# mhpi/hydrodl2

Measured on AMD Instinct MI355X. Metric: basin-ensemble-timesteps/sec fwd+bwd, higher is better.
Workload: dtype f32

## Files before the change

### __graft_entry__.py

```python
from __future__ import annotations

import os
import subprocess
import sys

ROOT = os.path.dirname(os.path.abspath(__file__))
CSRC = os.path.join(ROOT, "hydrodl2_amd", "csrc")
HIP_LIB = os.path.join(CSRC, "libhbvx.so")
ORACLE_DIR = os.path.join(ROOT, "oracle")
ORACLE_LIB = os.path.join(ORACLE_DIR, "liboracle_hbv.so")

HIPCC_FLAGS = ["--offload-arch=gfx950", "-O3", "-std=c++17", "-ffp-contract=off", "-fno-slp-vectorize", "-fPIC"]


def _newer(target: str, *sources: str) -> bool:
    if not os.path.exists(target):
        return False
    t = os.path.getmtime(target)
    return all(os.path.getmtime(s) <= t for s in sources)


def _hipcc() -> str:
    hipcc = os.environ.get("HIPCC", "/opt/rocm/bin/hipcc")
    return hipcc if os.path.exists(hipcc) else "hipcc"


def build_hip(force: bool = False, tag: str = "", flags=()) -> str:
    from concurrent.futures import ThreadPoolExecutor
    units = [os.path.join(CSRC, f) for f in sorted(os.listdir(CSRC)) if f.endswith(".hip")]
    headers = [os.path.join(CSRC, f) for f in sorted(os.listdir(CSRC)) if f.endswith(".h")] + [
        os.path.join(ROOT, "include", "hbvx.h"), os.path.join(ROOT, "include", "hbvx_lstm.h"),
        os.path.join(ROOT, "include", "hbvx_gage_pop.h"), os.path.join(ROOT, "include", "hbvx_route_rows.h"),
        os.path.join(ROOT, "include", "hbvx_pop_fdc.h"), os.path.join(ROOT, "include", "hbvx_gage_events.h"),
        os.path.join(ROOT, "include", "hbvx_pop_events.h"), os.path.join(ROOT, "include", "hbvx_gage_fdc.h")]
    objdir = os.path.join(CSRC, "build_" + tag if tag else "build")
    os.makedirs(objdir, exist_ok=True)
    extra = os.environ.get("HBVX_EXTRA_HIPCC_FLAGS", "").split() + list(flags)
    lib = os.path.join(CSRC, f"libhbvx_{tag}.so") if tag else HIP_LIB

    def compile_one(src):
        obj = os.path.join(objdir, os.path.basename(src)[:-4] + ".o")
        if force or not _newer(obj, src, *headers):
            subprocess.check_call([_hipcc()] + HIPCC_FLAGS + extra + ["-c", src, "-o", obj], cwd=CSRC)
            return obj, True
        return obj, False

    with ThreadPoolExecutor(max_workers=min(len(units), os.cpu_count() or 1)) as pool:
        done = list(pool.map(compile_one, units))
    objs = [o for o, _ in done]
    if force or any(r for _, r in done) or not _newer(lib, *objs):
        subprocess.check_call([_hipcc(), "--offload-arch=gfx950", "-shared", "-fPIC", "-o", lib] + objs, cwd=CSRC)
    return lib


def build_oracle() -> str:
    subprocess.check_call(["make", "-C", ORACLE_DIR], stdout=subprocess.DEVNULL)
    return ORACLE_LIB


def build() -> None:
    build_hip()
    build_oracle()
    if ROOT not in sys.path:
        sys.path.insert(0, ROOT)
    import hydrodl2_amd
    from hydrodl2_amd._abi import Library
    lib = Library(HIP_LIB)
    assert lib.is_device
    assert set(hydrodl2_amd.available_models()["hbv"]) >= {"hbv", "hbv_1_1p", "hbv_2"}


def smoke() -> None:
    if ROOT not in sys.path:
        sys.path.insert(0, ROOT)
    import torch
    assert torch.cuda.is_available(), "smoke() needs a GPU"
    if not os.path.exists(HIP_LIB):
        build_hip()
    if not os.path.exists(ORACLE_LIB):
        build_oracle()
    from tests.abi_util import assert_close, compare_runs, make_problem, run_problem
    prob = make_problem(model="Hbv", T=120, B=9, M=16, dyn=("parBETA", "parBETAET"), seed=3)
    got = run_problem(prob, None, device="cuda:0", x_grad=True)
    want = run_problem(prob, ORACLE_LIB, device="cpu", x_grad=True)
    compare_runs(prob, got, want, keys=("flux", "routed", "state_out", "g_params", "g_x"))
    from tests import seam
    from hydrodl2_amd.lstm import SeqLSTM
    torch.manual_seed(0)
    net = SeqLSTM(5, 64, check=True)
    xs = torch.randn(30, 9, 5)
    outs = []
    for dev, lib in (("cuda:0", None), ("cpu", ORACLE_LIB)):
        seam.use_library(lib)
        m = net.to(dev)
        xd = xs.to(dev).requires_grad_(True)
        o, _ = m(xd)
        o.square().sum().backward()
        outs.append((o.detach().cpu(), xd.grad.cpu(), m.weight_hh_l0.grad.cpu().clone()))
        m.zero_grad()
    seam.use_library(None)
    for name, g, w in zip(("lstm h", "lstm grad_x", "lstm grad_w_hh"), outs[0], outs[1]):
        assert_close(name, g.numpy(), w.numpy())
    print("smoke ok: HIP path matches the CPU oracle "
          f"(flux {got['flux'].shape}, grad {got['g_params'].shape}, lstm {tuple(outs[0][0].shape)})")


if __name__ == "__main__":
    if len(sys.argv) > 2 and sys.argv[1] == "variant":
        print(build_hip(tag=sys.argv[2], flags=sys.argv[3:]))
        sys.exit(0)
    build()
    if len(sys.argv) > 1 and sys.argv[1] == "smoke":
        smoke()
```

### hydrodl2_amd/_abi.py

```python
from __future__ import annotations

import ctypes as C
import os
from typing import NamedTuple, Optional

ABI_VERSION = 10
MAX_PARAM = 20
GAGE_MAXLEN = 72
NSTATE = 5
MAX_FLUX = 12
UH_MAXLEN = 15

MODEL_HBV10, MODEL_HBV11P, MODEL_HBV20, MODEL_HBVADJ, MODEL_HOURLY = 0, 1, 2, 3, 4

TRAJ_ROWS, TRAJ_PACKED, TRAJ_CKPT = 0, 1, 2

(F_QSIM, F_Q0, F_Q1, F_Q2, F_AET, F_SWE, F_RECHARGE, F_EXCS, F_EVAPFACTOR, F_TOSOIL, F_PERC,
 F_CAPILLARY) = range(12)

PARAM_SLOTS = ["parBETA", "parFC", "parK0", "parK1", "parK2", "parLP", "parPERC", "parUZL",
               "parTT", "parCFMAX", "parCFR", "parCWH", "parBETAET", "parC", "parRT", "parAC",
               "parF0", "parFMIN", "parALPHA"]

_fp = C.c_void_p
# ... 153 lines not shown

SIGNATURES = [
    ("hbvx_zero", True, _int, [_vp, _u64, _vp], None),
    ("hbvx_zero_except", True, _int, [_vp, _i64, _i32, _i64, _i64, _i32, C.c_uint32, _vp], None),
    ("hbvx_preferred_traj_layout", True, _int, [_P(Desc)], None),
    ("hbvx_lstm_workspace_bytes", True, _u64, [_P(LstmDesc)], None),
    ("hbvx_lstm_forward", True, _int, [_P(LstmDesc), _fp, _fp, _fp, _fp, _fp, _vp, _u64, _vp], None),
    ("hbvx_lstm_backward", True, _int, [_P(LstmDesc), _fp, _fp, _fp, _fp, _fp, _vp, _u64, _vp], None),
    ("hbvx_lstm_check", True, _int, [_P(LstmDesc), _vp, _vp], None),
    ("hbvx_version", True, _int, [], None),
    ("hbvx_last_error", True, _str, [], None),
    ("hbvx_backend", True, _str, [], None),
    ("hbvx_sizeof", True, _u64, [_int], None),
    ("hbvx_forward", True, _int, [_P(Desc), _P(FwdOut), _vp], None),
    ("hbvx_backward", True, _int, [_P(Desc), _P(BwdIO), _vp], None),
    ("hbvx_backward_workspace_bytes", True, _u64, [_P(Desc)], None),
    ("hbvx_ckpt_workspace_bytes", True, _u64, [_P(Desc), _i32], None),
    ("hbvx_route_forward", True, _int, [_P(RouteDesc), _fp, _fp, _fp, _vp], None),
    ("hbvx_route_workspace_bytes", True, _u64, [_P(RouteDesc)], None),
    ("hbvx_route_backward", True, _int, [_P(RouteDesc), _fp, _fp, _fp, _fp, _fp, _fp, _fp, _u64, _vp], None),
    ("hbvx_adj_forward", True, _int, [_P(Desc), _P(FwdOut), _vp], None),
    ("hbvx_adj_backward", True, _int, [_P(Desc), _P(BwdIO), _vp], None),
    ("hbvx_bfi", True, _int, [_i32, _i32, _fp, _fp, C.c_float, _fp, _vp], None),
    ("hbvx_gage_route_forward", True, _int, [_P(GageDesc), _fp, _fp, _fp, _vp, _u64, _vp], None),
    ("hbvx_gage_route_backward", True, _int, [_P(GageDesc), _fp, _fp, _fp, _fp, _fp, _vp, _u64, _vp], None),
    ("hbvx_gage_route_workspace_bytes", True, _u64, [_P(GageDesc)], None),
    ("hbvx_zero_in_launch", True, _int, [], None),
    ("hbvx_zero_rest", True, _int, [_vp, _u64, _vp, _vp], None),
    ("hbvx_last_dispatch", True, _str, [_int], None),
    ("hbvx_lstm_forward_hx", False, _int, [_P(LstmDesc), _fp, _fp, _fp, _fp, _fp, _fp, _fp, _vp, _u64, _vp], None),
    ("hbvx_lstm_backward_hx", False, _int, [_P(LstmDesc), _fp, _fp, _fp, _fp, _fp, _fp, _fp, _fp, _vp, _u64, _vp], None),
    ("hbvx_forward_tangent", False, _int, [_P(Desc), _P(TanIO), _vp], (7, TanIO)),
    ("hbvx_route_tangent", False, _int, [_P(RouteDesc), _fp, _fp, _fp, _fp, _fp, _fp, _vp], None),
    ("hbvx_bfi_tangent", False, _int, [_i32, _i32, _fp, _fp, _fp, _fp, C.c_float, _fp, _vp], None),
    ("hbvx_lstm_tangent", False, _int,
     [_P(LstmDesc), _fp, _fp, _fp, _fp, _fp, _fp, _fp, _fp, _fp, _vp, _u64, _vp], None),
    ("hbvx_forward_tangent_batch", False, _int, [_P(Desc), _P(TanBatch), _vp], (8, TanBatch)),
    ("hbvx_route_tangent_batch", False, _int,
     [_P(RouteDesc), _i32, _fp, _fp, _fp, _i64, _fp, _fp, _i64, _fp, _vp], None),
    ("hbvx_bfi_tangent_batch", False, _int, [_i32, _i32, _i32, _fp, _fp, _fp, _fp, _i64, C.c_float, _fp, _vp], None),
    ("hbvx_lstm_tangent_batch", False, _int,
     [_P(LstmDesc), _i32, _fp, _fp, _fp, _fp, _fp, _fp, _fp, _fp, _fp, _vp, _u64, _vp], None),
    ("hbvx_lstm_tangent_batch_workspace_bytes", False, _u64, [_P(LstmDesc), _i32], None),
    ("hbvx_hourly_tangent_batch", False, _int, [_P(Desc), _P(TanBatch), _vp], (8, TanBatch)),
    ("hbvx_gage_route_tangent_batch", False, _int,
     [_P(GageDesc), _i32, _fp, _fp, _fp, _i64, _fp, _i64, _fp, _vp, _u64, _vp], None),
    ("hbvx_gage_route_tangent_workspace_bytes", False, _u64, [_P(GageDesc), _i32], None),
    ("hbvx_adj_tangent_batch", False, _int, [_P(Desc), _P(TanBatch), _fp, _vp], (8, TanBatch)),
    ("hbvx_gram", False, _int, [_P(GramDesc), _fp, _fp, _fp, _fp, _fp, _fp, _vp, _u64, _vp], (9, GramDesc)),
    ("hbvx_gram_workspace_bytes", False, _u64, [_P(GramDesc)], None),
    ("hbvx_quadform", False, _int, [_P(GramDesc), _fp, _fp, _fp, _vp, _u64, _vp], (9, GramDesc)),
    ("hbvx_quadform_workspace_bytes", False, _u64, [_P(GramDesc)], None),
] + [(_name, False, _int, [_P(Desc), _P(_e.struct), _vp], (_POP_SIZEOF[_e.struct], _e.struct))
     for _name, _e in POPULATION.items()]

EXPORTS = [row[0] for row in SIGNATURES if row[1]]
OPTIONAL_EXPORTS = [row[0] for row in SIGNATURES if not row[1]]

GAGE_POP_ABI_VERSION = 1


class PopRunoff(C.Structure):
    _fields_ = [("abi_version", C.c_int32), ("n_cand", C.c_int32), ("p", PopSrc * MAX_PARAM), ("runoff", _fp)]


class GagePop(C.Structure):
    _fields_ = [("abi_version", C.c_int32), ("n_cand", C.c_int32), ("runoff", _fp), ("runoff_c_stride", C.c_int64),
                ("dp", _fp), ("uh", _fp), ("transform", C.c_int32), ("n_periods", C.c_int32),
                ("period_end", C.c_void_p),
                ("target", _fp), ("w", _fp), ("shift", _fp), ("eps", _fp),
                ("sse", _fp), ("s1", _fp), ("s2", _fp), ("s3", _fp), ("sim", _fp), ("series", _fp)]


GAGE_POP_SIGNATURES = [
    ("hbvx_gage_pop_sizeof", False, _u64, [_int], None),
    ("hbvx_hourly_population_runoff", False, _int, [_P(Desc), _P(PopRunoff), _vp], (0, PopRunoff)),
    ("hbvx_gage_population_workspace_bytes", False, _u64, [_P(GageDesc), _P(GagePop)], (1, GagePop)),
    ("hbvx_gage_population_stats", False, _int, [_P(GageDesc), _P(GagePop), _vp, _u64, _vp], (1, GagePop)),
]


GAGE_EVENTS_ABI_VERSION = 1


class GageEvents(C.Structure):
    _fields_ = [("abi_version", C.c_int32), ("n_cand", C.c_int32), ("T", C.c_int32), ("G", C.c_int32),
                ("n_events", C.c_int32), ("series", _fp),
                ("start", C.c_void_p), ("end", C.c_void_p),
                ("peak", _fp), ("peak_hour", C.c_void_p), ("volume", _fp)]


GAGE_EVENTS_SIGNATURES = [
    ("hbvx_gage_events_sizeof", False, _u64, [_int], None),
    ("hbvx_gage_population_events", False, _int, [_P(GageEvents), _vp], (0, GageEvents)),
]


POP_FDC_ABI_VERSION = 1
POP_FDC_MAX_THR = 32

GAGE_FDC_ABI_VERSION = 1
GAGE_QUANT_MAX_T = 16384


class GageFdc(C.Structure):
    _fields_ = [("abi_version", C.c_int32), ("n_cand", C.c_int32), ("T", C.c_int32), ("G", C.c_int32),
                ("n_lev", C.c_int32), ("series", _fp),
                ("scored", C.c_void_p),
                ("thr", _fp), ("count", C.c_void_p), ("volume", _fp),
                ("rank", C.c_void_p), ("quantile", _fp)]


GAGE_FDC_SIGNATURES = [
    ("hbvx_gage_fdc_sizeof", False, _u64, [_int], None),
    ("hbvx_gage_population_fdc", False, _int, [_P(GageFdc), _vp], (0, GageFdc)),
    ("hbvx_gage_quantiles_workspace_bytes", False, _u64, [C.c_int32, C.c_int32, C.c_int32], None),
    ("hbvx_gage_population_quantiles", False, _int, [_P(GageFdc), _fp, _u64, _vp], (0, GageFdc)),
]


class PopFdc(C.Structure):
    _fields_ = [("abi_version", C.c_int32), ("n_thr", C.c_int32), ("flow", PopStats), ("thr", _fp),
                ("count", C.c_void_p),
                ("volume", _fp)]


POP_FDC_SIGNATURES = [
    ("hbvx_pop_fdc_sizeof", False, _u64, [_int], None),
    ("hbvx_population_fdc", False, _int, [_P(Desc), _P(PopFdc), _vp], (0, PopFdc)),
]
POP_FDC_ENTRY = PopEntry(PopFdc, False, None)


POP_EVENTS_ABI_VERSION = 1


class PopEvents(C.Structure):
    _fields_ = [("abi_version", C.c_int32), ("n_events", C.c_int32), ("flow", PopStats),
                ("start", C.c_void_p), ("end", C.c_void_p),
                ("peak", _fp), ("peak_day", C.c_void_p), ("volume", _fp)]


POP_EVENTS_SIGNATURES = [
    ("hbvx_pop_events_sizeof", False, _u64, [_int], None),
    ("hbvx_population_events", False, _int, [_P(Desc), _P(PopEvents), _vp], (0, PopEvents)),
]
POP_EVENTS_ENTRY = PopEntry(PopEvents, False, None)


ROUTE_ROWS_SIGNATURES = [
    ("hbvx_route_backward_rows", False, _int, [_P(RouteDesc), _fp, _fp, _fp, _fp, _i32, _fp, _fp, _fp, _u64, _vp], None),
]


class HbvxError(RuntimeError):
    pass


class Library:

    def __init__(self, path: str):
        if not os.path.exists(path):
            raise FileNotFoundError(path)
        self.path = path
        self.dll = C.CDLL(path)
        d = self.dll
        for name in EXPORTS:
            if not hasattr(d, name):
                raise HbvxError(f"{path}: missing export {name}")
        self.missing = [name for name in OPTIONAL_EXPORTS +
                        [row[0] for row in GAGE_POP_SIGNATURES + ROUTE_ROWS_SIGNATURES + POP_FDC_SIGNATURES +
                         GAGE_EVENTS_SIGNATURES + POP_EVENTS_SIGNATURES + GAGE_FDC_SIGNATURES]
                        if not hasattr(d, name)]
        checked = set()
        for name, _, restype, argtypes, layout, sizeof in [row + ("hbvx_sizeof",) for row in SIGNATURES] + \
                [row + ("hbvx_gage_pop_sizeof",) for row in GAGE_POP_SIGNATURES] + \
                [row + ("hbvx_sizeof",) for row in ROUTE_ROWS_SIGNATURES] + \
                [row + ("hbvx_pop_fdc_sizeof",) for row in POP_FDC_SIGNATURES] + \
                [row + ("hbvx_gage_events_sizeof",) for row in GAGE_EVENTS_SIGNATURES] + \
                [row + ("hbvx_pop_events_sizeof",) for row in POP_EVENTS_SIGNATURES] + \
                [row + ("hbvx_gage_fdc_sizeof",) for row in GAGE_FDC_SIGNATURES]:
            if name in self.missing:
                continue
            fn = getattr(d, name)
            fn.restype, fn.argtypes = restype, argtypes
            if layout is not None and (sizeof, layout[0]) not in checked and sizeof not in self.missing:
                checked.add((sizeof, layout[0]))
                which, st = layout
                got = getattr(d, sizeof)(which)
                if got != C.sizeof(st):
                    raise HbvxError(f"{path}: layout mismatch for {st.__name__}: {got} != {C.sizeof(st)}")
        if d.hbvx_version() != ABI_VERSION:
            raise HbvxError(f"{path}: ABI version {d.hbvx_version()} != {ABI_VERSION}")
        for which, st in enumerate([Desc, FwdOut, BwdIO, RouteDesc, ParamSrc, ParamGrad, GageDesc]):
            if d.hbvx_sizeof(which) != C.sizeof(st):
                raise HbvxError(f"{path}: layout mismatch for {st.__name__}: "
                                f"{d.hbvx_sizeof(which)} != {C.sizeof(st)}")
        self.backend = d.hbvx_backend().decode()
        self.saves_pow = "+savepow" in self.backend

    @property
    def is_device(self) -> bool:
        return self.backend.startswith("hip")

    def _check(self, rc: int, what: str):
        if rc != 0:
            msg = self.dll.hbvx_last_error().decode(errors="replace")
            raise HbvxError(f"{what} failed ({rc}): {msg}")

    def forward(self, desc: Desc, out: FwdOut, stream: int):
        self._check(self.dll.hbvx_forward(C.byref(desc), C.byref(out), C.c_void_p(stream)),
                    "hbvx_forward")

    def backward(self, desc: Desc, io: BwdIO, stream: int):
        self._check(self.dll.hbvx_backward(C.byref(desc), C.byref(io), C.c_void_p(stream)),
                    "hbvx_backward")

    def zero_rest(self, ptr: int, nbytes: int, state_ptr: int, stream: int):
        self._check(self.dll.hbvx_zero_rest(C.c_void_p(ptr), nbytes, C.c_void_p(state_ptr), C.c_void_p(stream)), "hbvx_zero_rest")

    def zero_in_launch(self) -> bool:
        return bool(self.dll.hbvx_zero_in_launch())

    def last_dispatch(self, direction: int) -> str:
        return self.dll.hbvx_last_dispatch(direction).decode()

    def preferred_traj_layout(self, desc: Desc) -> int:
        return int(self.dll.hbvx_preferred_traj_layout(C.byref(desc)))

    def ckpt_workspace_bytes(self, desc: Desc, K: int) -> int:
        return int(self.dll.hbvx_ckpt_workspace_bytes(C.byref(desc), K))

    def backward_workspace_bytes(self, desc: Desc) -> int:
        return int(self.dll.hbvx_backward_workspace_bytes(C.byref(desc)))

    def adj_forward(self, desc: Desc, out: FwdOut, stream: int):
        self._check(self.dll.hbvx_adj_forward(C.byref(desc), C.byref(out), C.c_void_p(stream)),
                    "hbvx_adj_forward")

    def adj_backward(self, desc: Desc, io: BwdIO, stream: int):
        self._check(self.dll.hbvx_adj_backward(C.byref(desc), C.byref(io), C.c_void_p(stream)),
                    "hbvx_adj_backward")

    def gage_route_workspace_bytes(self, r: GageDesc) -> int:
        return int(self.dll.hbvx_gage_route_workspace_bytes(C.byref(r)))

    def gage_route_forward(self, r: GageDesc, qs: int, uh: int, out: int, ws, ws_bytes: int, stream: int):
        self._check(self.dll.hbvx_gage_route_forward(C.byref(r), qs, uh, out, ws, C.c_uint64(ws_bytes),
                                                     C.c_void_p(stream)), "hbvx_gage_route_forward")

    def gage_route_backward(self, r: GageDesc, qs: int, uh: int, go: int, gqs: int, gdp: int, ws,
                            ws_bytes: int, stream: int):
        self._check(self.dll.hbvx_gage_route_backward(C.byref(r), qs, uh, go, gqs, gdp, ws,
                                                      C.c_uint64(ws_bytes), C.c_void_p(stream)),
                    "hbvx_gage_route_backward")

    def zero(self, ptr: int, nbytes: int, stream: int):
        self._check(self.dll.hbvx_zero(ptr, C.c_uint64(nbytes), C.c_void_p(stream)), "hbvx_zero")

    def zero_except(self, ptr: int, rows: int, width: int, r0: int, r1: int, group_w: int, keep: int,
                    stream: int):
        self._check(self.dll.hbvx_zero_except(ptr, rows, width, r0, r1, group_w, C.c_uint32(keep),
                                              C.c_void_p(stream)), "hbvx_zero_except")

    def lstm_workspace_bytes(self, r: LstmDesc) -> int:
        return int(self.dll.hbvx_lstm_workspace_bytes(C.byref(r)))

    def lstm_forward(self, r: LstmDesc, w_hh: int, gx: int, gates: int, c_all: int, h_all: int, ws,
                     ws_bytes: int, stream: int):
        self._check(self.dll.hbvx_lstm_forward(C.byref(r), w_hh, gx, gates, c_all, h_all, ws,
                                               C.c_uint64(ws_bytes), C.c_void_p(stream)), "hbvx_lstm_forward")

    def lstm_backward(self, r: LstmDesc, w_hh: int, gates: int, c_all: int, gh: int, gg: int, ws,
                      ws_bytes: int, stream: int):
        self._check(self.dll.hbvx_lstm_backward(C.byref(r), w_hh, gates, c_all, gh, gg, ws,
                                                C.c_uint64(ws_bytes), C.c_void_p(stream)), "hbvx_lstm_backward")

    def require(self, name: str):
        if name in self.missing:
            raise HbvxError(f"{self.path}: missing export {name} (backend {self.backend!r})")

    def lstm_forward_hx(self, r: LstmDesc, w_hh: int, gx: int, h0, c0, gates: int, c_all: int, h_all: int, ws,
                        ws_bytes: int, stream: int):
        self.require("hbvx_lstm_forward_hx")
        self._check(self.dll.hbvx_lstm_forward_hx(C.byref(r), w_hh, gx, h0, c0, gates, c_all, h_all, ws,
                                                  C.c_uint64(ws_bytes), C.c_void_p(stream)), "hbvx_lstm_forward_hx")

    def lstm_backward_hx(self, r: LstmDesc, w_hh: int, gates: int, c0, c_all: int, gh: int, gc_last, gg: int, gc0,
                         ws, ws_bytes: int, stream: int):
        self.require("hbvx_lstm_backward_hx")
        self._check(self.dll.hbvx_lstm_backward_hx(C.byref(r), w_hh, gates, c0, c_all, gh, gc_last, gg, gc0, ws,
                                                   C.c_uint64(ws_bytes), C.c_void_p(stream)), "hbvx_lstm_backward_hx")

    def lstm_tangent(self, r: LstmDesc, w_hh: int, gates: int, c0, c_all: int, gx_t: int, h0_t, c0_t, h_t: int,
                     c_t_last, ws, ws_bytes: int, stream: int):
        self.require("hbvx_lstm_tangent")
        self._check(self.dll.hbvx_lstm_tangent(C.byref(r), w_hh, gates, c0, c_all, gx_t, h0_t, c0_t, h_t, c_t_last, ws,
                                               C.c_uint64(ws_bytes), C.c_void_p(stream)), "hbvx_lstm_tangent")

    def lstm_tangent_batch_workspace_bytes(self, r: LstmDesc, n_dir: int) -> int:
        self.require("hbvx_lstm_tangent_batch_workspace_bytes")
        return int(self.dll.hbvx_lstm_tangent_batch_workspace_bytes(C.byref(r), n_dir))

    def lstm_tangent_batch(self, r: LstmDesc, n_dir: int, w_hh: int, gates: int, c0, c_all: int, gx_t: int, h0_t,
                           c0_t, h_t: int, c_t_last, ws, ws_bytes: int, stream: int):
        self.require("hbvx_lstm_tangent_batch")
        self._check(self.dll.hbvx_lstm_tangent_batch(C.byref(r), n_dir, w_hh, gates, c0, c_all, gx_t, h0_t, c0_t, h_t,
                                                     c_t_last, ws, C.c_uint64(ws_bytes), C.c_void_p(stream)),
                    "hbvx_lstm_tangent_batch")

    def forward_tangent(self, desc: Desc, io: TanIO, stream: int):
        self.require("hbvx_forward_tangent")
        self._check(self.dll.hbvx_forward_tangent(C.byref(desc), C.byref(io), C.c_void_p(stream)), "hbvx_forward_tangent")

    def route_tangent(self, r: RouteDesc, q: int, uh: int, q_dot, ra_dot, rb_dot, q_rout_dot: int, stream: int):
        self.require("hbvx_route_tangent")
        self._check(self.dll.hbvx_route_tangent(C.byref(r), q, uh, q_dot, ra_dot, rb_dot, q_rout_dot,
                                                C.c_void_p(stream)), "hbvx_route_tangent")

    def bfi_tangent(self, T: int, B: int, qs: int, q2: int, qs_dot, q2_dot, nearzero: float, out: int, stream: int):
        self.require("hbvx_bfi_tangent")
        self._check(self.dll.hbvx_bfi_tangent(T, B, qs, q2, qs_dot, q2_dot, C.c_float(nearzero), out,
                                              C.c_void_p(stream)), "hbvx_bfi_tangent")

    def forward_tangent_batch(self, desc: Desc, tb: TanBatch, stream: int):
        self.require("hbvx_forward_tangent_batch")
        self._check(self.dll.hbvx_forward_tangent_batch(C.byref(desc), C.byref(tb), C.c_void_p(stream)),
                    "hbvx_forward_tangent_batch")

    def route_tangent_batch(self, r: RouteDesc, n_dir: int, q: int, uh: int, q_dot, q_dot_ds: int, ra_dot, rb_dot,
                            r_ds: int, q_rout_dot: int, stream: int):
        self.require("hbvx_route_tangent_batch")
        self._check(self.dll.hbvx_route_tangent_batch(C.byref(r), n_dir, q, uh, q_dot, q_dot_ds, ra_dot, rb_dot, r_ds,
                                                      q_rout_dot, C.c_void_p(stream)), "hbvx_route_tangent_batch")

    def bfi_tangent_batch(self, T: int, B: int, n_dir: int, qs: int, q2: int, qs_dot, q2_dot, dot_ds: int,
                          nearzero: float, out: int, stream: int):
        self.require("hbvx_bfi_tangent_batch")
        self._check(self.dll.hbvx_bfi_tangent_batch(T, B, n_dir, qs, q2, qs_dot, q2_dot, dot_ds, C.c_float(nearzero),
                                                    out, C.c_void_p(stream)), "hbvx_bfi_tangent_batch")

    def hourly_tangent_batch(self, desc: Desc, tb: TanBatch, stream: int):
        self.require("hbvx_hourly_tangent_batch")
        self._check(self.dll.hbvx_hourly_tangent_batch(C.byref(desc), C.byref(tb), C.c_void_p(stream)),
                    "hbvx_hourly_tangent_batch")

    def adj_tangent_batch(self, desc: Desc, tb: TanBatch, traj, stream: int):
        self.require("hbvx_adj_tangent_batch")
        self._check(self.dll.hbvx_adj_tangent_batch(C.byref(desc), C.byref(tb), traj, C.c_void_p(stream)),
                    "hbvx_adj_tangent_batch")

    def gram_workspace_bytes(self, g: GramDesc) -> int:
        self.require("hbvx_gram_workspace_bytes")
        return int(self.dll.hbvx_gram_workspace_bytes(C.byref(g)))

    def gram(self, g: GramDesc, s: int, w, r, gram: int, rhs, cost, ws, ws_bytes: int, stream: int):
        self.require("hbvx_gram")
        self._check(self.dll.hbvx_gram(C.byref(g), s, w, r, gram, rhs, cost, ws, C.c_uint64(ws_bytes),
                                       C.c_void_p(stream)), "hbvx_gram")

    def quadform_workspace_bytes(self, g: GramDesc) -> int:
        self.require("hbvx_quadform_workspace_bytes")
        return int(self.dll.hbvx_quadform_workspace_bytes(C.byref(g)))

    def quadform(self, g: GramDesc, s: int, m: int, q: int, ws, ws_bytes: int, stream: int):
        self.require("hbvx_quadform")
        self._check(self.dll.hbvx_quadform(C.byref(g), s, m, q, ws, C.c_uint64(ws_bytes), C.c_void_p(stream)),
                    "hbvx_quadform")

    def gage_route_tangent_workspace_bytes(self, r: GageDesc, n_dir: int) -> int:
# ... 92 lines not shown
```

### hydrodl2_amd/csrc/hbv_chunked.h

```cpp
#pragma once

#include <hip/hip_runtime.h>

#include "../../include/hbvx.h"
#include "hbv_step.h"
#include "hbv_lane.h"
#include "hbv_onepass_compose.h"

namespace hbvx {

struct ChunkArgs {
    hbvx_desc d;
    hbvx_bwd_io io;
    int lgMp;
    int C;
    int nchunk;
    float *phi;
    float *abnd;
    float *gpart;
    int nd;
    int dslot[3];
    int per_xcd;
    int group;
};

struct ChunkBlock {
    int bx, chunk;
};
__host__ __device__ inline int chunk_per_xcd(int B, int lgMp)
{
    const int bpw = 64 >> lgMp;
    return ((B + bpw - 1) / bpw + 7) / 8;
}
__device__ __forceinline__ bool chunk_block(const hbvx_desc &d, int lgMp, int per_xcd, ChunkBlock &b)
{
    const int i = blockIdx.x;
#if defined(HBVX_CHUNK_XCD) && HBVX_CHUNK_XCD == 0
    b.chunk = i / (8 * per_xcd);
    b.bx = i - b.chunk * (8 * per_xcd);
#else
    const int c = i & 7, k = i >> 3;
    b.chunk = k / per_xcd;
    b.bx = c * per_xcd + (k - b.chunk * per_xcd);
#endif
    return b.bx * (64 >> lgMp) < d.B;
}

#define CHUNK_FEW 3

template <int NP>
__device__ __forceinline__ void slot_set(float *p, int slot, float v)
{
#pragma unroll
    for (int i = 0; i < NP; i++)
        if (slot == i) p[i] = v;
}
template <int NP>
__device__ __forceinline__ float slot_get(const float *p, int slot)
{
    float v = 0.0f;
#pragma unroll
    for (int i = 0; i < NP; i++)
        if (slot == i) v = p[i];
    return v;
}

template <int MODEL, bool BETAET>
struct ChunkNP {
    static constexpr int value = MODEL == MODEL_HBV10 ? (BETAET ? 13 : 12)
                               : MODEL == MODEL_HBV11P ? 14 : (MODEL == MODEL_HOURLY ? 19 : 16);
};

template <int NP>
struct ChunkRaw {
    float f[3];
    float st[5];
    float sw0, ef0;
    float gf[HBVX_MAX_FLUX];
    float g4[4];
    float dv[NP];
    float mu;
};

template <int MODEL, bool BETAET, int NP>
struct ChunkDay {
    Step<MODEL, BETAET> s;
    float p[NPARAM_MAX];
    float ud[NP];
    FluxGrad g;
    float gq;
};

template <int NP>
__device__ __forceinline__ void chunk_dma_dyn(const hbvx_desc &d, const LaneId &L, int t, float *lds)
{
#if defined(__HIP_DEVICE_COMPILE__)
    const hbvx_param_src &ps = d.p[0];
    const float *src = ps.dyn + (int64_t)t * ps.dyn_t_stride + (int64_t)L.b * ps.dyn_b_stride + L.j;
    const int M = d.M;
#pragma unroll
    for (int i = 0; i < NP; i++) {
        __builtin_amdgcn_global_load_lds((const __attribute__((address_space(1))) void *)src,
                                         (__attribute__((address_space(3))) void *)(lds + i * 64), 4, 0, 0);
        src += M;
    }
#endif
}
template <int NP>
__device__ __forceinline__ void chunk_pull_dyn(ChunkRaw<NP> &R, const float *lds)
{
#pragma unroll
    for (int i = 0; i < NP; i++) R.dv[i] = lds[i * 64 + (threadIdx.x & 63)];
}

template <int NP, int DYN, bool GFULL, bool LDSDV = false, bool MU = false>
__device__ __forceinline__ void chunk_issue(const hbvx_desc &d, const hbvx_bwd_io &io,
                                            const LaneId &L, int t, int nf, ChunkRaw<NP> &R,
                                            int nd, const int *dslot)
{
    const int T = d.T;
    const int64_t N = (int64_t)d.B * d.M;
    const float *xr = d.x + (int64_t)t * d.x_t_stride + (int64_t)L.b * d.x_b_stride;
    R.f[0] = xr[d.ch_prcp]; R.f[1] = xr[d.ch_tmean]; R.f[2] = xr[d.ch_pet];
    const float *tp = io.traj + (int64_t)t * N + L.n;
    const int64_t ks = (int64_t)(T + 1) * N;
#pragma unroll
    for (int k = 0; k < 5; k++) R.st[k] = tp[k * ks];
    if (SAVE_POW) {
        const float *ap = io.aux + (int64_t)t * N + L.n;
        R.sw0 = ap[0];
        R.ef0 = ap[(int64_t)T * N];
    } else {
        R.sw0 = R.ef0 = 0.0f;
    }
    const int64_t fs = (int64_t)T * d.B, go = (int64_t)t * d.B + L.b;
#pragma unroll
    for (int k = 0; k < HBVX_MAX_FLUX; k++) {
        R.gf[k] = 0.0f;
        if (GFULL && k < nf) R.gf[k] = io.grad_flux[k * fs + go];
        if (k < 4) R.g4[k] = io.grad_flux4 ? io.grad_flux4[k * fs + go] : 0.0f;
    }
    R.mu = 0.0f;
    if (DYN == 1) {
#pragma unroll
        for (int k = 0; k < CHUNK_FEW; k++)
            if (k < nd) {
                const hbvx_param_src &ps = d.p[dslot[k]];
                R.dv[k] = ps.dyn[(int64_t)t * ps.dyn_t_stride + (int64_t)L.b * ps.dyn_b_stride + L.j];
            }
    }
    if (DYN == 3 && !LDSDV) {
        const hbvx_param_src &ps = d.p[0];
        const float *src = ps.dyn + (int64_t)t * ps.dyn_t_stride + (int64_t)L.b * ps.dyn_b_stride + L.j;
#pragma unroll
        for (int i = 0; i < NP; i++) R.dv[i] = src[i * d.M];
    }
    if (DYN == 2) {
#pragma unroll
        for (int i = 0; i < NP; i++) {
            const hbvx_param_src &ps = d.p[i];
            const bool dy = ps.dyn != nullptr;
            const float *base = dy ? ps.dyn : ps.sta;
            const int64_t ts = dy ? ps.dyn_t_stride : 0, bs = dy ? ps.dyn_b_stride : ps.sta_b_stride;
            R.dv[i] = base[(int64_t)t * ts + (int64_t)L.b * bs + L.j];
        }
    }
    if ((MU || DYN == 2) && d.muwts) R.mu = d.muwts[(int64_t)t * d.mu_t_stride + (int64_t)L.b * d.mu_b_stride + L.j];
}

template <int MODEL, bool BETAET, int NP, int DYN, bool GFULL, bool MU = false>
__device__ __forceinline__ void chunk_finish(const hbvx_desc &d, const ChunkRaw<NP> &R, bool raw, float nz,
                                             float ac, float elev, const float *usta, const float *psta,
                                             const bool *use_dyn, int nf, float invM,
                                             ChunkDay<MODEL, BETAET, NP> &D, int nd, const int *dslot, bool has4)
{
    float gf[HBVX_MAX_FLUX];
#pragma unroll
    for (int k = 0; k < HBVX_MAX_FLUX; k++) {
        gf[k] = R.gf[k];
        if (k < 4 && has4) gf[k] += R.g4[k];
    }
    D.s.P = R.f[0]; D.s.Tf = R.f[1]; D.s.PET = R.f[2];
    D.s.SP = R.st[0]; D.s.MW = R.st[1]; D.s.SM = R.st[2]; D.s.SUZ = R.st[3]; D.s.SLZ = R.st[4];
    if (DYN == 1) {
#pragma unroll
        for (int i = 0; i < NP; i++) D.p[i] = psta[i];
#pragma unroll
        for (int k = 0; k < CHUNK_FEW; k++)
            if (k < nd) {
                const hbvx_param_src &ps = d.p[dslot[k]];
                const float v = raw ? sigmoid_dyn_(R.dv[k]) : R.dv[k];
                D.ud[k] = v;
                const float pv = descale_(v, ps.lo, ps.hi);
                const float cur = slot_get<NP>(D.p, dslot[k]);
                slot_set<NP>(D.p, dslot[k], use_dyn[k] ? pv : cur);
            }
    }
    if (DYN == 3) {
#pragma unroll
        for (int i = 0; i < NP; i++) {
            D.ud[i] = raw ? sigmoid_dyn_(R.dv[i]) : R.dv[i];
            D.p[i] = descale_(D.ud[i], d.p[i].lo, d.p[i].hi);
        }
    }
#pragma unroll
    for (int i = 0; i < NP; i++) {
        if (DYN == 1 || DYN == 3) break;
        D.ud[i] = usta[i];
        D.p[i] = psta[i];
        if (DYN == 2) {
            const float v = raw ? sigmoid_dyn_(R.dv[i]) : R.dv[i];
            D.ud[i] = use_dyn[i] ? v : usta[i];
            D.p[i] = use_dyn[i] ? descale_(v, d.p[i].lo, d.p[i].hi) : psta[i];
        }
    }
#pragma unroll
    for (int i = NP; i < NPARAM_MAX; i++) D.p[i] = 0.0f;
    D.s.template fwd<SAVE_POW>(D.p, nz, ac, elev, R.sw0, R.ef0);
    D.gq = gf[HBVX_F_QSIM];
    const float wq = ((MU || DYN == 2) && d.muwts) ? R.mu : invM;
    D.g.gQ = D.gq * wq;
    D.g.gQ0 = gf[HBVX_F_Q0] * invM;
    D.g.gQ1 = gf[HBVX_F_Q1] * invM;
    D.g.gQ2 = gf[HBVX_F_Q2] * invM;
    D.g.gET = GFULL ? gf[HBVX_F_AET] * invM : 0.0f;
    D.g.gSWE = GFULL ? gf[HBVX_F_SWE] * invM : 0.0f;
    D.g.grech = GFULL ? gf[HBVX_F_RECHARGE] * invM : 0.0f;
    D.g.gexc = GFULL ? gf[HBVX_F_EXCS] * invM : 0.0f;
    D.g.gef = GFULL ? gf[HBVX_F_EVAPFACTOR] * invM : 0.0f;
    D.g.gtosoil = GFULL ? gf[HBVX_F_TOSOIL] * invM : 0.0f;
    D.g.gPERC = GFULL ? gf[HBVX_F_PERC] * invM : 0.0f;
    D.g.gcap = (GFULL && nf > HBVX_F_CAPILLARY) ? gf[HBVX_F_CAPILLARY] * invM : 0.0f;
}

template <int NP, int DYN>
__device__ __forceinline__ void chunk_static(const hbvx_desc &d, const LaneId &L, bool raw,
                                             float *usta, float *psta, bool *use_dyn, int nd,
                                             const int *dslot)
{
#pragma unroll
    for (int i = 0; i < NP; i++) {
        if (DYN == 3) {
            usta[i] = psta[i] = 0.0f;
            use_dyn[i] = true;
            continue;
        }
        const hbvx_param_src &s = d.p[i];
        float v = s.sta[(int64_t)L.b * s.sta_b_stride + L.j];
        usta[i] = raw ? sigmoid_(v) : v;
        psta[i] = descale_(usta[i], s.lo, s.hi);
        use_dyn[i] = DYN == 2 && s.dyn && !(s.drop && s.drop[L.b]);
    }
    if (DYN == 1) {
#pragma unroll
        for (int k = 0; k < CHUNK_FEW; k++) {
            use_dyn[k] = false;
            if (k < nd) {
                const hbvx_param_src &s = d.p[dslot[k]];
                use_dyn[k] = !(s.drop && s.drop[L.b]);
            }
        }
    }
}

template <int SC>
struct SlotCombo {
    static constexpr int nd = SC == 1 ? 2 : (SC == 2 ? 3 : 0);
    static constexpr int s0 = P_BETA, s1 = SC == 1 ? P_BETAET : P_K0, s2 = P_BETAET;
};
#define CHUNK_SLOTS(A)                                                                             \
    const int nd_ = SC ? SlotCombo<SC>::nd : (A).nd;                                               \
    const int ds_[3] = {SC ? SlotCombo<SC>::s0 : (A).dslot[0], SC ? SlotCombo<SC>::s1 : (A).dslot[1], \
                        SC ? SlotCombo<SC>::s2 : (A).dslot[2]}

template <int MODEL, bool BETAET, int DYN, bool GFULL, int SC = 0, bool MU = false>
__global__ void __launch_bounds__(64) k_bwd_chunk_phi(const ChunkArgs A)
{
    CHUNK_SLOTS(A);
    constexpr int NP = ChunkNP<MODEL, BETAET>::value;
    const hbvx_desc &d = A.d;
    const hbvx_bwd_io &io = A.io;
    ChunkBlock blk;
    if (!chunk_block(d, A.lgMp, A.per_xcd, blk)) return;
    const LaneId L = lane_id(d, A.lgMp, blk.bx);
    const int chunk = blk.chunk;
    const int t0 = chunk * A.C, t1 = min(d.T, t0 + A.C);
    const int64_t N = (int64_t)d.B * d.M;
    const bool raw = d.raw_sigmoid != 0;
    const float nz = d.nearzero, invM = 1.0f / (float)d.M;
    const float ac = (MODEL == MODEL_HBV20 || MODEL == MODEL_HOURLY) ? d.ac[L.b] : 0.0f;
    const float elev = (MODEL == MODEL_HBV20 || MODEL == MODEL_HOURLY) ? d.elev[L.b] : 0.0f;
    float usta[NP], psta[NP];
    bool use_dyn[NP];
    chunk_static<NP, DYN>(d, L, raw, usta, psta, use_dyn, nd_, ds_);

    float Phi[5][5], phi[5];
#pragma unroll
    for (int k = 0; k < 5; k++) {
        phi[k] = 0.0f;
#pragma unroll
        for (int i = 0; i < 5; i++) Phi[k][i] = (i == k) ? 1.0f : 0.0f;
    }
    FluxGrad g0;
    g0.gQ = g0.gQ0 = g0.gQ1 = g0.gQ2 = g0.gET = g0.gSWE = g0.grech = g0.gexc = g0.gef = g0.gtosoil =
        g0.gPERC = g0.gcap = 0.0f;
    constexpr bool LDSDV = DYN == 3;
    __shared__ float dvbuf[LDSDV ? NP * 64 : 1];
    ChunkRaw<NP> Rn;
    if (LDSDV) chunk_dma_dyn<NP>(d, L, t1 - 1, dvbuf);
    chunk_issue<NP, DYN, GFULL, LDSDV, MU>(d, io, L, t1 - 1, io.n_flux, Rn, nd_, ds_);
    for (int t = t1 - 1; t >= t0; t--) {
        ChunkRaw<NP> Rc = Rn;
        if (LDSDV) {
            asm volatile("s_waitcnt vmcnt(0)" ::: "memory");
            chunk_pull_dyn<NP>(Rc, dvbuf);
            asm volatile("s_waitcnt lgkmcnt(0)" ::: "memory");
        }
        if (t > t0) {
            if (LDSDV) chunk_dma_dyn<NP>(d, L, t - 1, dvbuf);
            chunk_issue<NP, DYN, GFULL, LDSDV, MU>(d, io, L, t - 1, io.n_flux, Rn, nd_, ds_);
        }
        ChunkDay<MODEL, BETAET, NP> D;
        chunk_finish<MODEL, BETAET, NP, DYN, GFULL, MU>(d, Rc, raw, nz, ac, elev, usta, psta, use_dyn,
                                                    io.n_flux, invM, D, nd_, ds_, io.grad_flux4 != nullptr);
        float gp[NPARAM_MAX], gx[3];
#pragma unroll
        for (int i = 0; i < NPARAM_MAX; i++) gp[i] = 0.0f;
        if constexpr (MODEL == MODEL_HBV10) {
            typedef Step<MODEL, BETAET> S;
            const typename S::JT c = D.s.jt_coef(D.p, nz);
            S::template jt_unit<0>(c, Phi[0]);
            S::template jt_unit<0>(c, Phi[1]);
            S::template jt_unit<1>(c, Phi[2]);
            S::template jt_unit<2>(c, Phi[3]);
            S::template jt_unit<2>(c, Phi[4]);
            if constexpr (!GFULL) {
                S::jt_affine(c, phi, D.g.gQ0 + D.g.gQ, D.g.gQ1 + D.g.gQ, D.g.gQ2 + D.g.gQ);
                continue;
            }
        } else if constexpr (MODEL == MODEL_HBV11P || MODEL == MODEL_HBV20) {
            typedef Step<MODEL, BETAET> S;
            const typename S::JTC c = D.s.jt_coef_cap(D.p, nz);
            S::template jt_unit<0>(c, Phi[0]);
            S::template jt_unit<0>(c, Phi[1]);
#pragma unroll
            for (int k = 2; k < 5; k++) S::jt_cap(c, Phi[k], 0.0f, 0.0f, 0.0f);
            if constexpr (!GFULL) {
                S::jt_cap(c, phi, D.g.gQ0 + D.g.gQ, D.g.gQ1 + D.g.gQ, D.g.gQ2 + D.g.gQ);
                continue;
            }
        } else {
#pragma unroll
            for (int k = 0; k < 5; k++) D.s.bwd(D.p, nz, g0, Phi[k], gp, gx);
        }
        D.s.bwd(D.p, nz, D.g, phi, gp, gx);
    }
    if (L.active) {
        float *dst = A.phi + ((int64_t)chunk * 30) * N + L.n;
#pragma unroll
        for (int k = 0; k < 5; k++)
#pragma unroll
            for (int i = 0; i < 5; i++) dst[(int64_t)(k * 5 + i) * N] = Phi[k][i];
#pragma unroll
        for (int i = 0; i < 5; i++) dst[(int64_t)(25 + i) * N] = phi[i];
    }
}

#define ONEPASS_GMAX 4
__host__ __device__ constexpr int onepass_slot_bytes(int NP) { return (30 + onepass_rows(NP)) * 64 * (int)sizeof(float); }

template <int NP>
struct OnepassSlot {
    float *s;
    __device__ __forceinline__ float Phi(int k, int j) const { return s[(k * 5 + j) * 64]; }
    __device__ __forceinline__ float phi(int j) const { return s[(25 + j) * 64]; }
    __device__ __forceinline__ float G(int k, int p) const { return s[(30 + onepass_row(p) + k - onepass_kmin(p)) * 64]; }
    __device__ __forceinline__ void Phi(int k, int i, float v) { s[(k * 5 + i) * 64] = v; }
    __device__ __forceinline__ void phi(int i, float v) { s[(25 + i) * 64] = v; }
    __device__ __forceinline__ void G(int k, int p, float v) { s[(30 + onepass_row(p) + k - onepass_kmin(p)) * 64] = v; }
};
template <int NP>
struct OnepassRows {
    float *m, *g;
    int64_t N;
    bool active;
    __device__ __forceinline__ void Phi(int k, int i, float v) { if (active) m[(int64_t)(k * 5 + i) * N] = v; }
    __device__ __forceinline__ void phi(int i, float v) { if (active) m[(int64_t)(25 + i) * N] = v; }
    __device__ __forceinline__ void G(int k, int p, float v)
    {
        if (active) g[(int64_t)(onepass_row(p) + k - onepass_kmin(p)) * N] = v;
    }
};

template <bool BETAET, bool GFULL>
__global__ void __launch_bounds__(64 * ONEPASS_GMAX) __attribute__((amdgpu_waves_per_eu(GFULL ? 2 : 3)))
k_bwd_chunk_onepass(const ChunkArgs A)
{
    extern __shared__ float onepass_slot[];
    constexpr int MODEL = MODEL_HBV10, DYN = 0;
    constexpr int NP = ChunkNP<MODEL, BETAET>::value;
    typedef Step<MODEL, BETAET> S;
    const int ds_[3] = {0, 0, 0};
    const hbvx_desc &d = A.d;
    const hbvx_bwd_io &io = A.io;
    ChunkBlock blk;
    if (!chunk_block(d, A.lgMp, A.per_xcd, blk)) return;
    const LaneId L = lane_id(d, A.lgMp, blk.bx);
    const int grp = blk.chunk;
    const int w = __builtin_amdgcn_readfirstlane((int)threadIdx.x >> 6);
    const int nw = min(min(A.group, ONEPASS_GMAX), A.nchunk - grp * A.group);
    const int chunk = grp * A.group + w;
    const int t0 = chunk * A.C, t1 = min(d.T, t0 + A.C);
    const int64_t N = (int64_t)d.B * d.M;
    const bool raw = d.raw_sigmoid != 0;
    const float nz = d.nearzero, invM = 1.0f / (float)d.M;
    float usta[NP], psta[NP];
    bool use_dyn[NP];
    chunk_static<NP, DYN>(d, L, raw, usta, psta, use_dyn, 0, ds_);

    float Phi[5][5], phi[5];
    float G[6][NPARAM_MAX];
#pragma unroll
    for (int k = 0; k < 5; k++) {
        phi[k] = 0.0f;
#pragma unroll
        for (int i = 0; i < 5; i++) Phi[k][i] = (i == k) ? 1.0f : 0.0f;
    }
#pragma unroll
    for (int k = 0; k < 6; k++)
#pragma unroll
        for (int i = 0; i < NPARAM_MAX; i++) G[k][i] = 0.0f;
    if (w < nw) {
    ChunkRaw<NP> Rn;
    chunk_issue<NP, DYN, GFULL>(d, io, L, t1 - 1, io.n_flux, Rn, 0, ds_);
    for (int t = t1 - 1; t >= t0; t--) {
        ChunkRaw<NP> Rc = Rn;
        if (t > t0) chunk_issue<NP, DYN, GFULL>(d, io, L, t - 1, io.n_flux, Rn, 0, ds_);
        ChunkDay<MODEL, BETAET, NP> D;
        chunk_finish<MODEL, BETAET, NP, DYN, GFULL>(d, Rc, raw, nz, 0.0f, 0.0f, usta, psta, use_dyn, io.n_flux, invM,
                                                    D, 0, ds_, io.grad_flux4 != nullptr);
        const typename S::JT c = D.s.jt_coef(D.p, nz);
        const typename S::JG k = D.s.jg_coef(D.p, nz);
        S::template jt_gp<0>(c, k, Phi[0], G[0]);
        S::template jt_gp<0>(c, k, Phi[1], G[1]);
        S::template jt_gp<1>(c, k, Phi[2], G[2]);
        S::template jt_gp<2>(c, k, Phi[3], G[3]);
        S::template jt_gp<2>(c, k, Phi[4], G[4]);
        if constexpr (!GFULL) {
            S::template jt_gp<2, true>(c, k, phi, G[5], D.g.gQ0 + D.g.gQ, D.g.gQ1 + D.g.gQ, D.g.gQ2 + D.g.gQ);
        } else {
            float gx[3];
            D.s.bwd(D.p, nz, D.g, phi, G[5], gx);
        }
    }
    }
    OnepassRows<NP> rows{A.phi + ((int64_t)grp * 30) * N + L.n, A.gpart + ((int64_t)grp * onepass_rows(NP)) * N + L.n, N,
                         L.active};
    if (A.group == 1) {
        onepass_put<float, NP>(Phi, phi, G, rows);
        return;
    }
    OnepassSlot<NP> slot{onepass_slot + (threadIdx.x & 63)};
    if (w == nw - 1 && w > 0) onepass_put<float, NP>(Phi, phi, G, slot);
    static_assert(ONEPASS_GMAX == 4, "one stage per wave above wave 0");
    if (nw > 1) {
        if (nw > 2) {
            if (nw > 3) __syncthreads();
            if (w == 2 && nw > 3) onepass_compose<float, NP, false>(slot, Phi, phi, G, slot);
            __syncthreads();
        }
        if (w == 1 && nw > 2) onepass_compose<float, NP, false>(slot, Phi, phi, G, slot);
        __syncthreads();
    }
    if (w == 0) {
        if (nw == 1) onepass_put<float, NP>(Phi, phi, G, rows);
        else onepass_compose<float, NP, true>(slot, Phi, phi, G, rows);
    }
}

#ifndef HBVX_CHUNK_NO_SHARED_KERNELS
__global__ void __launch_bounds__(64) k_bwd_chunk_scan(const ChunkArgs A)
{
    const hbvx_desc &d = A.d;
    const int64_t N = (int64_t)d.B * d.M;
    const int64_t n = (int64_t)blockIdx.x * 64 + threadIdx.x;
    if (n >= N) return;
    float a[5];
#pragma unroll
    for (int k = 0; k < 5; k++) a[k] = A.io.grad_state_out ? A.io.grad_state_out[k * N + n] : 0.0f;
    constexpr int SCAN_DEPTH = 4;
    float buf[SCAN_DEPTH][30];
    auto fetch = [&](int c, float *dst) __attribute__((always_inline)) {
        const float *src = A.phi + ((int64_t)c * 30) * N + n;
#pragma unroll
        for (int i = 0; i < 30; i++) dst[i] = src[(int64_t)i * N];
    };
#pragma unroll
    for (int j = 0; j < SCAN_DEPTH; j++)
        if (A.nchunk - 1 - j >= 0) fetch(A.nchunk - 1 - j, buf[j]);
    for (int c0 = A.nchunk - 1; c0 >= 0; c0 -= SCAN_DEPTH) {
#pragma unroll
        for (int j = 0; j < SCAN_DEPTH; j++) {
            const int c = c0 - j;
            if (c < 0) break;
            float cur[30];
#pragma unroll
            for (int i = 0; i < 30; i++) cur[i] = buf[j][i];
            if (c - SCAN_DEPTH >= 0) fetch(c - SCAN_DEPTH, buf[j]);
#pragma unroll
            for (int k = 0; k < 5; k++) A.abnd[((int64_t)c * 5 + k) * N + n] = a[k];
            float an[5];
#pragma unroll
            for (int i = 0; i < 5; i++) {
                float v = cur[25 + i];
#pragma unroll
                for (int k = 0; k < 5; k++) v += a[k] * cur[k * 5 + i];
                an[i] = v;
            }
#pragma unroll
            for (int i = 0; i < 5; i++) a[i] = an[i];
        }
    }
    if (A.io.grad_state_in) {
#pragma unroll
        for (int k = 0; k < 5; k++) A.io.grad_state_in[k * N + n] = a[k];
    }
}

#endif

template <int MODEL, bool BETAET, int DYN, bool GFULL, int SC = 0, bool ROWST = false, bool MU = false>
__global__ void __launch_bounds__(64) k_bwd_chunk_sweep(const ChunkArgs A)
{
    CHUNK_SLOTS(A);
    constexpr int NP = ChunkNP<MODEL, BETAET>::value;
    __shared__ float rowbuf[ROWST ? 64 * NP : 1];
    const hbvx_desc &d = A.d;
    const hbvx_bwd_io &io = A.io;
    ChunkBlock blk;
    if (!chunk_block(d, A.lgMp, A.per_xcd, blk)) return;
    const LaneId L = lane_id(d, A.lgMp, blk.bx);
    const int chunk = blk.chunk;
    const int t0 = chunk * A.C, t1 = min(d.T, t0 + A.C);
    const int64_t N = (int64_t)d.B * d.M;
    const bool raw = d.raw_sigmoid != 0;
    const float nz = d.nearzero, invM = 1.0f / (float)d.M;
    const float ac = (MODEL == MODEL_HBV20 || MODEL == MODEL_HOURLY) ? d.ac[L.b] : 0.0f;
    const float elev = (MODEL == MODEL_HBV20 || MODEL == MODEL_HOURLY) ? d.elev[L.b] : 0.0f;
    float usta[NP], psta[NP], gsta[NP];
    bool use_dyn[NP];
    chunk_static<NP, DYN>(d, L, raw, usta, psta, use_dyn, nd_, ds_);
#pragma unroll
    for (int i = 0; i < NP; i++) gsta[i] = 0.0f;
    float gused[CHUNK_FEW] = {0.0f, 0.0f, 0.0f};
    float a[5];
#pragma unroll
    for (int k = 0; k < 5; k++) a[k] = A.abnd[((int64_t)chunk * 5 + k) * N + L.n];

    constexpr bool LDSDV = DYN == 3;
    __shared__ float dvbuf[LDSDV ? NP * 64 : 1];
    ChunkRaw<NP> Rn;
    if (LDSDV) chunk_dma_dyn<NP>(d, L, t1 - 1, dvbuf);
    chunk_issue<NP, DYN, GFULL, LDSDV, MU>(d, io, L, t1 - 1, io.n_flux, Rn, nd_, ds_);
    for (int t = t1 - 1; t >= t0; t--) {
        ChunkRaw<NP> Rc = Rn;
        if (LDSDV) {
            asm volatile("s_waitcnt vmcnt(0)" ::: "memory");
            chunk_pull_dyn<NP>(Rc, dvbuf);
            asm volatile("s_waitcnt lgkmcnt(0)" ::: "memory");
        }
        if (t > t0) {
            if (LDSDV) chunk_dma_dyn<NP>(d, L, t - 1, dvbuf);
            chunk_issue<NP, DYN, GFULL, LDSDV, MU>(d, io, L, t - 1, io.n_flux, Rn, nd_, ds_);
        }
        ChunkDay<MODEL, BETAET, NP> D;
        chunk_finish<MODEL, BETAET, NP, DYN, GFULL, MU>(d, Rc, raw, nz, ac, elev, usta, psta, use_dyn,
                                                    io.n_flux, invM, D, nd_, ds_, io.grad_flux4 != nullptr);
        if ((MU || DYN == 2) && io.grad_muwts && L.active) io.grad_muwts[((int64_t)t * d.B + L.b) * d.M + L.j] = D.gq * D.s.Q;
        float gp[NPARAM_MAX], gx[3];
#pragma unroll
        for (int i = 0; i < NPARAM_MAX; i++) gp[i] = 0.0f;
        D.s.bwd(D.p, nz, D.g, a, gp, gx);
        if (DYN == 1) {
#pragma unroll
            for (int i = 0; i < NP; i++) gsta[i] += gp[i] * (d.p[i].hi - d.p[i].lo);
#pragma unroll
            for (int k = 0; k < CHUNK_FEW; k++)
                if (k < nd_) {
                    const int sl = ds_[k];
                    const float gu = slot_get<NP>(gp, sl) * (d.p[sl].hi - d.p[sl].lo);
                    const float gr = raw ? gu * (D.ud[k] * (1.0f - D.ud[k])) : gu;
                    if (io.g[sl].dyn && L.active)
                        io.g[sl].dyn[(int64_t)t * io.g[sl].dyn_t_stride + (int64_t)L.b * io.g[sl].dyn_b_stride + L.j] =
                            use_dyn[k] ? gr : 0.0f;
                    gused[k] += use_dyn[k] ? gu : 0.0f;
                }
        }
        if (DYN == 3 && !ROWST) {
#pragma unroll
            for (int i = 0; i < NP; i++) {
                const float gu = gp[i] * (d.p[i].hi - d.p[i].lo);
                const float gr = raw ? gu * (D.ud[i] * (1.0f - D.ud[i])) : gu;
                if (io.g[i].dyn && L.active)
                    io.g[i].dyn[(int64_t)t * io.g[i].dyn_t_stride + (int64_t)L.b * io.g[i].dyn_b_stride + L.j] = gr;
            }
        }
        if (DYN == 3 && ROWST) {
            const int M = d.M, rowf = NP * M, bl = (threadIdx.x & 63) >> A.lgMp;
            if (L.jm < M) {
#pragma unroll
                for (int i = 0; i < NP; i++) {
                    const float gu = gp[i] * (d.p[i].hi - d.p[i].lo);
                    rowbuf[bl * rowf + i * M + L.jm] = raw ? gu * (D.ud[i] * (1.0f - D.ud[i])) : gu;
                }
            }
            const int b0 = blk.bx * (64 >> A.lgMp);
            const int nb = min(64 >> A.lgMp, d.B - b0);
            const int half = rowf >> 1, total2 = nb * half;
            float *gbase = io.g[0].dyn + (int64_t)t * io.g[0].dyn_t_stride + (int64_t)b0 * io.g[0].dyn_b_stride;
            for (int k = threadIdx.x & 63; k < total2; k += 64) {
                const int rb = k / half, w2 = k - rb * half;
                const float2 v = *reinterpret_cast<const float2 *>(&rowbuf[rb * rowf + 2 * w2]);
                *reinterpret_cast<float2 *>(gbase + (int64_t)rb * io.g[0].dyn_b_stride + 2 * w2) = v;
            }
        }
#pragma unroll
        for (int i = 0; i < NP; i++) {
            if (DYN == 1 || DYN == 3) break;
            const float gu = gp[i] * (d.p[i].hi - d.p[i].lo);
            if (DYN == 2) {
// ... 118 lines not shown
```

### hydrodl2_amd/csrc/hbv_pipe.h

```cpp
#pragma once

#include <hip/hip_runtime.h>

#include "../../include/hbvx.h"
#include "hbv_step.h"
#include "hbv_tiled.h"
#include "hbv_adj_step.h"

namespace hbvx {

#ifndef PIPE_KT
#define PIPE_KT 8
#endif
#ifndef PIPE_KT_STATIC
#define PIPE_KT_STATIC 10
#endif
#define PIPE_KT_MANY 4
#define PIPE_FEWDYN 3
#define PIPE_MAXDYN 18
#ifndef PIPE_REBALANCE
#define PIPE_REBALANCE 1
#endif
#ifndef PIPE_Q1
#define PIPE_Q1 2
#endif

#define PIPE_DAYS(nt, body)                                                                        \
    do {                                                                                           \
        if ((nt) == KT && !PIPE_NO_UNROLL) {                                                       \
            _Pragma("unroll") for (int tt_ = 0; tt_ < KT; tt_++) body(tt_, tt_ + 1 < KT);          \
        } else {                                                                                   \
            for (int tt_ = 0; tt_ < (nt); tt_++) body(tt_, tt_ + 1 < (nt));                        \
        }                                                                                          \
    } while (0)

struct PipeArgs {
    hbvx_desc d;
    hbvx_fwd_out o;
    int lgMp;
    int Kt;
    int ckptK;
    void *fill_ptr;
    unsigned *fill_state;
    unsigned long long fill_n16;
    int nwg;
    int fill_waves;
};

typedef float pipe_f4 __attribute__((ext_vector_type(4)));
constexpr unsigned PIPE_FILL_PIECE16 = HBVX_ZERO_PIECE / 16;

__device__ __forceinline__ void pipe_signal_done(const PipeArgs &A)
{
    if (A.fill_n16 && (threadIdx.x & 63) == 0)
        __hip_atomic_fetch_add(A.fill_state + 1, 1u, __ATOMIC_RELAXED, __HIP_MEMORY_SCOPE_AGENT);
}

__device__ __forceinline__ void pipe_fill_role(const PipeArgs &A)
{
    const unsigned lane = threadIdx.x & 63;
    if ((int)(threadIdx.x >> 6) >= A.fill_waves) return;
    const unsigned long long npiece = (A.fill_n16 + PIPE_FILL_PIECE16 - 1) / PIPE_FILL_PIECE16;
    pipe_f4 *base = static_cast<pipe_f4 *>(A.fill_ptr);
    const pipe_f4 z = {0.0f, 0.0f, 0.0f, 0.0f};
    for (;;) {
        unsigned done = 0, c = 0;
        if (lane == 0) done = __hip_atomic_load(A.fill_state + 1, __ATOMIC_RELAXED, __HIP_MEMORY_SCOPE_AGENT);
        if (__builtin_amdgcn_readfirstlane(done) >= (unsigned)A.nwg) return;
        if (lane == 0) c = __hip_atomic_fetch_add(A.fill_state, 1u, __ATOMIC_RELAXED, __HIP_MEMORY_SCOPE_AGENT);
        c = __builtin_amdgcn_readfirstlane(c);
        if (c >= npiece) return;
        const unsigned long long i0 = (unsigned long long)c * PIPE_FILL_PIECE16;
        const unsigned long long left = A.fill_n16 - i0;
        const unsigned n = left < PIPE_FILL_PIECE16 ? (unsigned)left : PIPE_FILL_PIECE16;
        pipe_f4 *p = base + i0;
#pragma unroll 4
        for (unsigned i = lane; i < n; i += 64) __builtin_nontemporal_store(z, p + i);
    }
}

struct PipeLds {
    int xin, ab, bc, oa, ob, oc, pin, total;
    __host__ __device__ explicit PipeLds(int Kt, int pd = 0, bool cap = false)
    {
        const int obr = cap ? 8 : 7;
        xin = 0;
        ab = xin + 4 * Kt * 256;
        bc = ab + 2 * Kt * 128;
        oa = bc + 2 * Kt * 128;
        ob = oa + 2 * Kt * 256;
        oc = ob + 2 * Kt * obr * 64;
        pin = oc + 2 * Kt * 448;
        total = pin + 5 * Kt * pd * 64;
    }
};

template <int NSER, int NFS, unsigned FMAP>
__device__ __forceinline__ void pipe_reduce_pass(const hbvx_desc &d, const hbvx_fwd_out &o, const float *buf,
                                                 int t0, int items, int pass, int lane, int lgMp, int b0, bool muq = false)
{
    const int T = d.T, B = d.B;
    const float invM = 1.0f / (float)d.M;
    __amdgpu_buffer_rsrc_t r = __builtin_amdgcn_make_buffer_rsrc(o.flux, 0, -1, 0x00020000);
    ens_reduce_pass<NSER, NFS>(buf, items, pass * 64, lane, d.M, lgMp, [&](int tt, int ks, int bl, float acc) {
        const int kk = (int)((FMAP >> (4 * ks)) & 0xFu);
        const unsigned off = b0 + bl < B ? (unsigned)(((kk * T + (t0 + tt)) * B + b0 + bl) * 4) : 0xFFFFFFFFu;
        const float v = (muq && kk == HBVX_F_QSIM) ? acc : acc * invM;
        __builtin_amdgcn_raw_buffer_store_b32(__builtin_bit_cast(unsigned, v), r, off, 0, 0);
    });
}

#ifdef PIPE_PROBE
__device__ unsigned long long g_pipe_probe[32];
__device__ unsigned long long g_pipe_blocks[4096];
#define PIPE_BARRIER()                                                                             \
    do {                                                                                           \
        unsigned long long t_a = __builtin_readcyclecounter();                                     \
        probe_busy += t_a - probe_t;                                                               \
        lds_barrier();                                                                             \
        probe_t = __builtin_readcyclecounter();                                                    \
        probe_wait += probe_t - t_a;                                                               \
    } while (0)
#else
#define PIPE_BARRIER() lds_barrier()
#endif

template <int SC>
__device__ __forceinline__ constexpr int pipe_sc_flag(int X)
{
    return SC == 0 ? -1 : ((X == P_BETA || X == P_BETAET || (SC == 2 && X == P_K0)) ? 1 : 0);
}
#define DY_DECL(X) const bool dy_##X = DYN && (pipe_sc_flag<SC>(X) >= 0 ? pipe_sc_flag<SC>(X) != 0 : (((dmask >> X) & 1u) != 0)); const int ix_##X = dy_##X ? dyn_index(dmask, X) * 64 : 0; float pn_##X = 0.0f
#define DY_LOAD(X, ptr) do { pn_##X = (ptr)[ix_##X]; } while (0)
#define DY_USE(X) do { p[X] = dy_##X ? pn_##X : p[X]; } while (0)

template <int MODEL, bool BETAET, int TRAJ, bool DYN, bool MANY = false, int SC = 0>
__global__ void __launch_bounds__(1024) k_fwd_pipe(const PipeArgs A)
{
    constexpr bool ADJ = MODEL == MODEL_HBVADJ;
    constexpr bool PIPE_NO_UNROLL = ADJ;
    constexpr bool CAP = MODEL != MODEL_HBV10 && !ADJ;
    constexpr int KT = MANY ? PIPE_KT_MANY : (DYN ? PIPE_KT : PIPE_KT_STATIC);
    constexpr int OBR = CAP ? 8 : 7, NFB = CAP ? 5 : 4;
#ifdef PIPE_PROBE
    unsigned long long probe_busy = 0, probe_wait = 0, probe_t = __builtin_readcyclecounter();
    struct ProbeFlush {
        unsigned long long &b, &w;
        __device__ ~ProbeFlush()
        {
            if ((threadIdx.x >> 6) == 1 && (threadIdx.x & 63) == 0 && blockIdx.x < 4096) g_pipe_blocks[blockIdx.x] = b + w;
            if (blockIdx.x == 5 && (threadIdx.x & 63) == 0) {
                g_pipe_probe[(threadIdx.x >> 6) * 2] = b;
                g_pipe_probe[(threadIdx.x >> 6) * 2 + 1] = w;
            }
        }
    } probe_flush{probe_busy, probe_wait};
#endif
    constexpr int NP = NParamT<MODEL, BETAET>::value;
    extern __shared__ __align__(16) float lds[];
    if (A.fill_n16 && (int)blockIdx.x >= A.nwg) {
        pipe_fill_role(A);
        return;
    }
    const hbvx_desc &d = A.d;
    const hbvx_fwd_out &o = A.o;
    const int wave = __builtin_amdgcn_readfirstlane(threadIdx.x >> 6);
    const LaneT L = lane_t(d, A.lgMp);
    const int lane = L.lane;
    const int T = d.T, Kt = A.Kt;
    const int nT = (T + Kt - 1) / Kt;
    const int nIt = nT + 3;
    const int64_t N = (int64_t)d.B * d.M;
    const bool raw = d.raw_sigmoid != 0;
    const unsigned row_bytes = (unsigned)(N * 4);
    const unsigned voff = L.active ? (unsigned)(L.n * 4) : 0xFFFFFFFFu;
    unsigned dmask = 0;
    if (DYN) {
#pragma unroll
        for (int i = 0; i < NP; i++) dmask |= d.p[i].dyn ? (1u << i) : 0u;
    }
    const bool has_mu = DYN && !ADJ && d.muwts != nullptr;
    const int mrow = __builtin_popcount(dmask);
    const int ix_mu = has_mu ? mrow * 64 : 0;
    const int PD = DYN ? (MANY ? mrow + (has_mu ? 1 : 0) : PIPE_FEWDYN) : 0;
    const PipeLds P(Kt, PD, CAP);
    const float nz = d.nearzero;
    const float ac = (MODEL == MODEL_HBV20 || MODEL == MODEL_HOURLY) ? d.ac[L.b] : 0.0f;
    const float elev = (MODEL == MODEL_HBV20 || MODEL == MODEL_HOURLY) ? d.elev[L.b] : 0.0f;
    auto pin_of = [&](int tile) { return lds + P.pin + (tile % 5) * Kt * PD * 64 + lane; };

    float p[NPARAM_MAX];
#pragma unroll
    for (int i = 0; i < NPARAM_MAX; i++) p[i] = 0.0f;
#pragma unroll
    for (int i = 0; i < NP; i++) {
        const hbvx_param_src &s = d.p[i];
        float v = s.sta[(int64_t)L.b * s.sta_b_stride + L.j];
        v = raw ? sigmoid_(v) : v;
        p[i] = descale_(v, s.lo, s.hi);
    }
    auto tile_nt = [&](int tile) { return min(Kt, T - tile * Kt); };

    constexpr bool DIRECT = TRAJ == 2 && !SAVE_POW;
    const int64_t SRt = (int64_t)(T + 1) * N;
    auto trj_rsrc = [&](int k, int tile) {
        return A.ckptK ? __builtin_amdgcn_make_buffer_rsrc(o.traj, 0, -1, 0x00020000)
                       : __builtin_amdgcn_make_buffer_rsrc(o.traj + k * SRt + (int64_t)tile * Kt * N, 0, (int)(row_bytes * KT),
                                                           0x00020000);
    };
    auto trj_put = [&](__amdgpu_buffer_rsrc_t r, int tile, int tt, int k, float v) __attribute__((always_inline)) {
        if (A.ckptK) {
            const int day = tile * Kt + tt;
            if (day % A.ckptK == 0)
                __builtin_amdgcn_raw_buffer_store_b32(__builtin_bit_cast(unsigned, v), r, voff,
                                                      (unsigned)(((int64_t)(day / A.ckptK) * 5 + k) * row_bytes), 0);
        } else {
            __builtin_amdgcn_raw_buffer_store_b32(__builtin_bit_cast(unsigned, v), r, voff, (unsigned)tt * row_bytes, 0);
        }
    };

    if (wave == 0) {
        __builtin_amdgcn_s_setprio(3);
        constexpr float S0 = ADJ ? 0.0f : 0.001f;
        float SP = d.state_in ? d.state_in[0 * N + L.n] : S0;
        float MW = d.state_in ? d.state_in[1 * N + L.n] : S0;
        PIPE_BARRIER();
        for (int it = 0; it < nIt; it++) {
            const int tile = it;
            if (tile < nT) {
                const int nt = tile_nt(tile);
                const float4 *in4 = reinterpret_cast<const float4 *>(lds + P.xin + (tile & 3) * Kt * 256);
                float *ab = lds + P.ab + (tile & 1) * Kt * 128 + lane;
                float *oa = lds + P.oa + (tile & 1) * Kt * 256 + lane;
                float4 fn = in4[lane];
                const float *pin = pin_of(tile);
                const auto rSP = trj_rsrc(0, tile), rMW = trj_rsrc(1, tile);
                DY_DECL(P_TT); DY_DECL(P_CFMAX); DY_DECL(P_CFR); DY_DECL(P_CWH);
                if (DYN) { DY_LOAD(P_TT, pin); DY_LOAD(P_CFMAX, pin); DY_LOAD(P_CFR, pin); DY_LOAD(P_CWH, pin); }
                auto day = [&](int tt, bool more) __attribute__((always_inline)) {
                    const float4 f = fn;
                    if (DYN) { DY_USE(P_TT); DY_USE(P_CFMAX); DY_USE(P_CFR); DY_USE(P_CWH); }
                    if (more) {
                        fn = in4[(tt + 1) * 64 + lane];
                        if (DYN) {
                            const float *pt = pin + (tt + 1) * PD * 64;
                            DY_LOAD(P_TT, pt); DY_LOAD(P_CFMAX, pt); DY_LOAD(P_CFR, pt); DY_LOAD(P_CWH, pt);
                        }
                    }
                    float *q = oa + tt * 256;
                    if constexpr (ADJ) {
                        float y0, y1, rfv, isn;
                        AdjStaged<BETAET>::snow(p, f.x, f.y, 1.0f, SP, MW, y0, y1, rfv, isn);
                        ab[tt * 128] = rfv;
                        ab[tt * 128 + 64] = isn;
                        if (TRAJ) {
                            if (DIRECT) { trj_put(rSP, tile, tt, 0, SP); trj_put(rMW, tile, tt, 1, MW); }
                            else { q[128] = SP; q[192] = MW; }
                        }
                        SP = y0; MW = y1;
                    } else {
                        Step<MODEL, BETAET> s;
                        s.P = f.x; s.Tf = f.y;
                        s.SP = SP; s.MW = MW;
                        s.fwd_snow(p, elev);
                        ab[tt * 128] = s.RAIN;
                        ab[tt * 128 + 64] = s.tosoil;
                        q[0] = s.SP3; q[64] = s.tosoil;
                        if (TRAJ) {
                            if (DIRECT) { trj_put(rSP, tile, tt, 0, SP); trj_put(rMW, tile, tt, 1, MW); }
                            else { q[128] = SP; q[192] = MW; }
                        }
                        SP = s.SP3; MW = s.MW3;
                    }
                };
                PIPE_DAYS(nt, day);
            }
            PIPE_BARRIER();
        }
        if (L.active) {
            o.state_out[0 * N + L.n] = SP;
            o.state_out[1 * N + L.n] = MW;
            if (TRAJ && !A.ckptK) {
                o.traj[((int64_t)0 * (T + 1) + T) * N + L.n] = SP;
                o.traj[((int64_t)1 * (T + 1) + T) * N + L.n] = MW;
            }
        }
    } else if (wave == 1) {
      if constexpr (CAP) {
        __builtin_amdgcn_s_setprio(3);
        float SM = d.state_in ? d.state_in[2 * N + L.n] : 0.001f;
        float SUZ = d.state_in ? d.state_in[3 * N + L.n] : 0.001f;
        float SLZ = d.state_in ? d.state_in[4 * N + L.n] : 0.001f;
        PIPE_BARRIER();
        for (int it = 0; it < nIt; it++) {
            const int tile = it - 1;
            if (tile >= 0 && tile < nT) {
// ... 456 lines not shown
```

### hydrodl2_amd/csrc/hbvx.hip

```cpp
#include "hbvx_host.h"
#include "../../include/hbvx_route_rows.h"
#include "hbv_step.h"
#include "hbv_lane.h"
#include "hbv_gage.h"
#include "hbv_pop.h"

using namespace hbvx;
using namespace hbvx_host;

static thread_local char g_err[512] = "";

int hbvx_host::fail(int code, const char *msg)
{
    snprintf(g_err, sizeof g_err, "%s", msg);
    return code;
}

int hbvx_host::hip_fail(hipError_t e, const char *what)
{
    snprintf(g_err, sizeof g_err, "%s: %s", what, hipGetErrorString(e));
    return HBVX_E_DEVICE;
}

static std::mutex g_disp_mu;
static char g_disp[2][48] = {"", ""};
void hbvx_host::note_dispatch(int dir, const char *family)
{
    std::lock_guard<std::mutex> lock(g_disp_mu);
    snprintf(g_disp[dir & 1], sizeof g_disp[0], "%s", family);
}
extern "C" int hbvx_zero_in_launch(void) { return hbvx_host::zero_taken() ? 1 : 0; }

extern "C" const char *hbvx_last_dispatch(int direction)
{
    static thread_local char out[48];
    std::lock_guard<std::mutex> lock(g_disp_mu);
    snprintf(out, sizeof out, "%s", g_disp[direction & 1]);
    return out;
}

extern "C" int hbvx_version(void) { return HBVX_ABI_VERSION; }
extern "C" const char *hbvx_last_error(void) { return g_err; }
extern "C" const char *hbvx_backend(void) { return hbvx::SAVE_POW ? "hip:gfx950+savepow" : "hip:gfx950"; }
extern "C" uint64_t hbvx_sizeof(int which)
{
    switch (which) {
    case 0: return sizeof(hbvx_desc);
    case 1: return sizeof(hbvx_fwd_out);
    case 2: return sizeof(hbvx_bwd_io);
    case 3: return sizeof(hbvx_route_desc);
    case 6: return sizeof(hbvx_gage_desc);
    case 4: return sizeof(hbvx_param_src);
    case 5: return sizeof(hbvx_param_grad);
    case 7: return sizeof(hbvx_tan_io);
    case 8: return sizeof(hbvx_tan_batch);
    case 9: return sizeof(hbvx_gram_desc);
    case 10: return sizeof(hbvx_pop);
    case 11: return sizeof(hbvx_pop_stats);
    case 12: return sizeof(hbvx_pop_joint);
    case 13: return sizeof(hbvx_pop_period);
    default: return 0;
    }
}

struct FwdArgs {
    hbvx_desc d;
    hbvx_fwd_out o;
    int lgMp;
};

template <int MODEL, bool BETAET>
__global__ void __launch_bounds__(64) k_fwd(const FwdArgs A)
{
    constexpr int NP = NParam<MODEL, BETAET>::value;
    const hbvx_desc &d = A.d;
    const hbvx_fwd_out &o = A.o;
    const int lgMp = A.lgMp;
    const LaneId L = lane_id(d, lgMp);
    const int T = d.T;
    const int64_t N = (int64_t)d.B * d.M;
    const bool raw = d.raw_sigmoid != 0;
    const float nz = d.nearzero;
    const float ac = (MODEL == MODEL_HBV20 || MODEL == MODEL_HOURLY) ? d.ac[L.b] : 0.0f;
    const float elev = (MODEL == MODEL_HBV20 || MODEL == MODEL_HOURLY) ? d.elev[L.b] : 0.0f;

    float p[NPARAM_MAX];
    const float *dynp[NP];
    bool use_dyn[NP];
    unsigned dmask = 0;
#pragma unroll
    for (int i = 0; i < NP; i++) {
        const hbvx_param_src &s = d.p[i];
        float v = s.sta[(int64_t)L.b * s.sta_b_stride + L.j];
        v = raw ? sigmoid_(v) : v;
        p[i] = descale_(v, s.lo, s.hi);
        dynp[i] = s.dyn ? s.dyn + (int64_t)L.b * s.dyn_b_stride + L.j : s.sta;
        use_dyn[i] = s.dyn && !(s.drop && s.drop[L.b]);
        if (s.dyn) dmask |= 1u << i;
    }
#pragma unroll
    for (int i = NP; i < NPARAM_MAX; i++) p[i] = 0.0f;

    float st[5];
#pragma unroll
    for (int k = 0; k < 5; k++) st[k] = d.state_in ? d.state_in[k * N + L.n] : 0.001f;

    const float *xb = d.x + (int64_t)L.b * d.x_b_stride;
    const float *mu = d.muwts ? d.muwts + (int64_t)L.b * d.mu_b_stride + L.j : nullptr;
    const float invM = 1.0f / (float)d.M;
    const int nf = o.n_flux;
    const int ckpt_k = (o.traj && HBVX_TRAJ_KIND(o.traj_layout) == HBVX_TRAJ_CKPT) ? HBVX_TRAJ_CKPT_DAYS(o.traj_layout) : 0;

    float nxf[3], nxd[NP];
    {
        const float *xr = xb;
        nxf[0] = T > 0 ? xr[d.ch_prcp] : 0.f;
        nxf[1] = T > 0 ? xr[d.ch_tmean] : 0.f;
        nxf[2] = T > 0 ? xr[d.ch_pet] : 0.f;
#pragma unroll
        for (int i = 0; i < NP; i++) nxd[i] = ((dmask >> i) & 1) && T > 0 ? dynp[i][0] : 0.f;
    }

    for (int t = 0; t < T; t++) {
        Step<MODEL, BETAET> s;
        s.P = nxf[0]; s.Tf = nxf[1]; s.PET = nxf[2];
        float cur[NP];
#pragma unroll
        for (int i = 0; i < NP; i++) cur[i] = nxd[i];
        {
            const int tn = t + 1 < T ? t + 1 : t;
            const float *xr = xb + (int64_t)tn * d.x_t_stride;
            nxf[0] = xr[d.ch_prcp]; nxf[1] = xr[d.ch_tmean]; nxf[2] = xr[d.ch_pet];
#pragma unroll
            for (int i = 0; i < NP; i++)
                if ((dmask >> i) & 1) nxd[i] = dynp[i][(int64_t)tn * d.p[i].dyn_t_stride];
        }
#pragma unroll
        for (int i = 0; i < NP; i++)
            if ((dmask >> i) & 1) {
                float v = raw ? sigmoid_dyn_(cur[i]) : cur[i];
                float pv = descale_(v, d.p[i].lo, d.p[i].hi);
                if (use_dyn[i]) p[i] = pv;
            }
        s.SP = st[0]; s.MW = st[1]; s.SM = st[2]; s.SUZ = st[3]; s.SLZ = st[4];
        s.template fwd<false, true>(p, nz, ac, elev, 0.f, 0.f);

        if (ckpt_k) {
            if (t % ckpt_k == 0 && L.active) {
#pragma unroll
                for (int k = 0; k < 5; k++) o.traj[((int64_t)(t / ckpt_k) * 5 + k) * N + L.n] = st[k];
            }
        } else if (o.traj && L.active) {
#pragma unroll
            for (int k = 0; k < 5; k++) o.traj[((int64_t)k * (T + 1) + t) * N + L.n] = st[k];
// ... 514 lines not shown
    else if (d->model == HBVX_MODEL_HBV20) ok = (d->n_param == 16);
    else if (d->model == HBVX_MODEL_HBVADJ) ok = (d->n_param == 12 || d->n_param == 13);
    else if (d->model == HBVX_MODEL_HOURLY) ok = (d->n_param == 19);
    else return fail(HBVX_E_UNSUPPORTED, "unknown model");
    if (!ok) return fail(HBVX_E_SHAPE, "n_param does not match model");
    if (!d->x && d->T > 0) return fail(HBVX_E_NULL, "forcing pointer is NULL");
    if (d->ch_prcp < 0 || d->ch_tmean < 0 || d->ch_pet < 0)
        return fail(HBVX_E_SHAPE, "negative forcing channel");
    if (!(d->nearzero >= 0.0f)) return fail(HBVX_E_SHAPE, "nearzero must be >= 0 (the storages' lower clamp, hbv.py:54)");
    if ((d->model == HBVX_MODEL_HBV20 || d->model == HBVX_MODEL_HOURLY) && (!d->ac || !d->elev))
        return fail(HBVX_E_NULL, "HBV 2.0 needs ac and elev");
    for (int i = 0; i < d->n_param; i++)
        if (!d->p[i].sta) return fail(HBVX_E_NULL, "static parameter pointer is NULL");
    if (d->model != HBVX_MODEL_HBVADJ) {
        if (!(d->p[P_LP].hi <= 1.0f && d->p[P_LP].lo <= 1.0f))
            return fail(HBVX_E_UNSUPPORTED, "parLP bounds above 1 are not supported (evaporation factor on an excess day, hbv.py:474-477)");
        if (!(d->p[P_BETA].lo > 0.0f && d->p[P_BETA].hi > 0.0f))
            return fail(HBVX_E_UNSUPPORTED, "parBETA bounds must be positive (soil wetness power, hbv.py:462)");
        if (d->n_param > P_BETAET && !(d->p[P_BETAET].lo > 0.0f && d->p[P_BETAET].hi > 0.0f))
            return fail(HBVX_E_UNSUPPORTED, "parBETAET bounds must be positive (evaporation factor power, hbv.py:476)");
        if (d->model == HBVX_MODEL_HOURLY && !(d->p[P_ALPHA].lo > 0.0f && d->p[P_ALPHA].hi > 0.0f))
            return fail(HBVX_E_UNSUPPORTED, "parALPHA bounds must be positive (infiltration power, hbv_2_hourly.py:590-600)");
    }
    return HBVX_OK;
}

int hbvx_host::lg_members(int M)
{
    int lg = 0;
    while ((1 << lg) < M) lg++;
    return lg;
}

int hbvx_host::env_int(const char *name, int dflt)
{
    const char *v = getenv(name);
    return (v && *v) ? atoi(v) : dflt;
}

bool hbvx_host::use_tiled(const hbvx_desc *d)
{
    const char *v = getenv("HBVX_KERNEL");
    if (v && !strcmp(v, "simple")) return false;
    return d->T > 0;
}

hipError_t hbvx_host::set_dynamic_lds(const void *kern, int lds)
{
    struct Entry { const void *k; int dev, lds; };
    static std::mutex mu;
    static Entry seen[256];
    static int n_seen = 0;
    int dev = 0;
    (void)hipGetDevice(&dev);
    std::lock_guard<std::mutex> lock(mu);
    Entry *e = nullptr;
    for (int i = 0; i < n_seen && !e; i++)
        if (seen[i].k == kern && seen[i].dev == dev) e = &seen[i];
    if (e && lds <= e->lds) return hipSuccess;
    const hipError_t rc = hipFuncSetAttribute(kern, hipFuncAttributeMaxDynamicSharedMemorySize, lds);
    if (rc != hipSuccess) return rc;
    if (e) e->lds = lds;
    else if (n_seen < 256) seen[n_seen++] = Entry{kern, dev, lds};
    return hipSuccess;
}

int hbvx_host::count_dyn(const hbvx_desc *d)
{
    int nd = 0;
    for (int i = 0; i < d->n_param; i++) nd += d->p[i].dyn ? 1 : 0;
    return nd;
}

int hbvx_host::device_cu_count()
{
    static int n_cu[64] = {0};
    int dev = 0;
    if (hipGetDevice(&dev) != hipSuccess || dev < 0 || dev >= 64) return 256;
    if (n_cu[dev] == 0) {
        int v = 0;
        if (hipDeviceGetAttribute(&v, hipDeviceAttributeMultiprocessorCount, dev) != hipSuccess || v <= 0) v = 256;
        n_cu[dev] = v;
    }
    return n_cu[dev];
}

bool &hbvx_host::zero_taken()
{
    static thread_local bool taken = false;
    return taken;
}

static int forward_dispatch(const hbvx_desc *d, const hbvx_fwd_out *out, void *stream);

extern "C" int hbvx_forward(const hbvx_desc *d, const hbvx_fwd_out *out, void *stream)
{
    zero_taken() = false;
    if (out && out->zero_ptr && !out->zero_state) return fail(HBVX_E_NULL, "zero_ptr needs zero_state");
    return forward_dispatch(d, out, stream);
}

static int forward_dispatch(const hbvx_desc *d, const hbvx_fwd_out *out, void *stream)
{
    int rc = check_desc(d);
    if (rc) return rc;
    if (d->model == HBVX_MODEL_HBVADJ) return fail(HBVX_E_UNSUPPORTED, "use hbvx_adj_forward for HBVADJ");
    if (!out || !out->state_out) return fail(HBVX_E_NULL, "state_out is NULL");
    const int want_nf = (d->model == HBVX_MODEL_HBV10) ? 11 : 12;
    if (out->flux && out->n_flux != want_nf) return fail(HBVX_E_SHAPE, "n_flux does not match model");
    if (out->traj && out->traj_layout != HBVX_TRAJ_ROWS) {
        const int kind = HBVX_TRAJ_KIND(out->traj_layout);
        if (kind == HBVX_TRAJ_CKPT) {
            const int K = HBVX_TRAJ_CKPT_DAYS(out->traj_layout);
            if (K != 4 && K != 8 && K != 16) return fail(HBVX_E_SHAPE, "checkpoint interval must be 4, 8 or 16");
            if (out->aux) return fail(HBVX_E_SHAPE, "checkpoints: aux must be NULL");
            if (try_fwd_stream(d, out, stream, &rc)) return rc;
            if (try_fwd_pipe(d, out, stream, &rc)) return rc;
            if (try_fwd_stream(d, out, stream, &rc, true)) return rc;
            FwdArgs ca;
            ca.d = *d;
            ca.o = *out;
            ca.lgMp = lg_members(d->M);
            const int bpw_c = 64 >> ca.lgMp;
            note_dispatch(0, "simple");
            const dim3 grid_c((d->B + bpw_c - 1) / bpw_c);
            hipError_t ec = with_model(d, [&](auto m, auto be) {
                hipLaunchKernelGGL((k_fwd<m, be>), grid_c, dim3(64), 0, (hipStream_t)stream, ca);
                return hipGetLastError();
            });
            return ec == hipSuccess ? HBVX_OK : hip_fail(ec, "hbvx_forward (checkpoints) launch");
        }
        if (out->traj_layout != HBVX_TRAJ_PACKED) return fail(HBVX_E_SHAPE, "unknown traj_layout");
        if (try_fwd_stream(d, out, stream, &rc, true)) return rc;
        return fail(HBVX_E_UNSUPPORTED, "packed trajectory: no forward kernel for this call");
    }
    if (try_fwd_stream(d, out, stream, &rc)) return rc;
    if (try_fwd_pipe(d, out, stream, &rc)) return rc;
    if (try_fwd_tiled(d, out, stream, &rc)) return rc;
    FwdArgs a;
    a.d = *d;
    a.o = *out;
    a.lgMp = lg_members(d->M);
    const int bpw = 64 >> a.lgMp;
    dim3 grid((d->B + bpw - 1) / bpw);
    note_dispatch(0, "simple");
    hipError_t e = with_model(d, [&](auto m, auto be) {
        hipLaunchKernelGGL((k_fwd<m, be>), grid, dim3(64), 0, (hipStream_t)stream, a);
        return hipGetLastError();
    });
    if (e != hipSuccess) return hip_fail(e, "hbvx_forward launch");
    return HBVX_OK;
}

extern "C" int hbvx_backward(const hbvx_desc *d, const hbvx_bwd_io *io, void *stream)
{
    int rc = check_desc(d);
    if (rc) return rc;
    if (d->model == HBVX_MODEL_HBVADJ) return fail(HBVX_E_UNSUPPORTED, "use hbvx_adj_backward for HBVADJ");
    if (!io || !io->traj) return fail(HBVX_E_NULL, "traj is NULL");
    if (SAVE_POW && !io->aux && HBVX_TRAJ_KIND(io->traj_layout) != HBVX_TRAJ_CKPT) return fail(HBVX_E_NULL, "aux is NULL");
    const int want_nf = (d->model == HBVX_MODEL_HBV10) ? 11 : 12;
    if (io->n_flux != want_nf) return fail(HBVX_E_SHAPE, "n_flux does not match model");
    if (d->T == 0) return HBVX_OK;
    if (io->traj_layout != HBVX_TRAJ_ROWS) {
        if (HBVX_TRAJ_KIND(io->traj_layout) == HBVX_TRAJ_CKPT) {
            if (try_bwd_stream_ckpt(d, io, stream, &rc)) return rc;
            if (try_bwd_ckpt(d, io, stream, &rc)) return rc;
            return fail(HBVX_E_UNSUPPORTED, "checkpoints: no adjoint kernel for this call");
        }
        if (io->traj_layout != HBVX_TRAJ_PACKED) return fail(HBVX_E_SHAPE, "unknown traj_layout");
        if (try_bwd_stream(d, io, stream, &rc)) return rc;
        return fail(HBVX_E_UNSUPPORTED, "packed trajectory: no adjoint kernel for this call");
    }
    if (try_bwd_stream(d, io, stream, &rc)) return rc;
    if (try_bwd_chunked(d, io, stream, &rc)) return rc;
    if (try_bwd_tiled(d, io, stream, &rc)) return rc;
    BwdArgs a;
    a.d = *d;
    a.io = *io;
    a.lgMp = lg_members(d->M);
    const int bpw = 64 >> a.lgMp;
    dim3 grid((d->B + bpw - 1) / bpw);
    store_gate(io, (hipStream_t)stream);
    note_dispatch(1, "simple");
    hipError_t e = with_model(d, [&](auto m, auto be) {
        hipLaunchKernelGGL((k_bwd<m, be>), grid, dim3(64), 0, (hipStream_t)stream, a);
        return hipGetLastError();
    });
    if (e != hipSuccess) return hip_fail(e, "hbvx_backward launch");
    return HBVX_OK;
}

static int check_route(const hbvx_route_desc *r)
{
    if (!r) return fail(HBVX_E_NULL, "route desc is NULL");
    if (r->abi_version != HBVX_ABI_VERSION) return fail(HBVX_E_ABI, "abi_version mismatch");
    if (r->T <= 0 || r->B <= 0 || r->S <= 0) return fail(HBVX_E_SHAPE, "bad T/B/S");
    const int L = r->T < HBVX_UH_MAXLEN ? r->T : HBVX_UH_MAXLEN;
    if (r->L != L) return fail(HBVX_E_SHAPE, "L must be min(T, 15)");
    if (!r->ra || !r->rb) return fail(HBVX_E_NULL, "routing parameter pointer is NULL");
    return HBVX_OK;
}

extern "C" int hbvx_route_forward(const hbvx_route_desc *r, const float *q, float *uh,
                                  float *q_rout, void *stream)
{
    int rc = check_route(r);
    if (rc) return rc;
    if (!q || !uh || !q_rout) return fail(HBVX_E_NULL, "route buffer is NULL");
    hipStream_t st = (hipStream_t)stream;
    hipLaunchKernelGGL(k_uh_gamma, dim3((r->B + UH_PB - 1) / UH_PB), dim3(16 * UH_PB), 0, st, *r, uh);
    const int64_t nblk = (int64_t)((r->B + 63) / 64) * ((r->T + ROUTE_FWD_TILE - 1) / ROUTE_FWD_TILE) * r->S;
    if (nblk > INT32_MAX - 8) return fail(HBVX_E_SHAPE, "routing: too many (basin, day, series) tiles for one launch");
    hipLaunchKernelGGL(k_route_fwd, dim3(xcd_grid(nblk)), dim3(256), 0, st, r->T, r->B, r->S, r->L, q, uh, q_rout);
    hipError_t e = hipGetLastError();
    if (e != hipSuccess) return hip_fail(e, "hbvx_route_forward launch");
    return HBVX_OK;
}

static int route_chunks(const hbvx_route_desc *r) { return (r->T + ROUTE_CHUNK_BWD - 1) / ROUTE_CHUNK_BWD; }

extern "C" uint64_t hbvx_route_workspace_bytes(const hbvx_route_desc *r)
{
    if (!r || r->T <= 0 || r->B <= 0) return 0;
    return (uint64_t)route_chunks(r) * (uint64_t)r->L * (uint64_t)r->B * sizeof(double);
}

static int launch_route_bwd(const hbvx_route_desc *r, const float *q, const float *uh, const float *grad_q_rout,
                            float *grad_q, int n_rows, float *grad_ra, float *grad_rb, void *workspace,
                            uint64_t workspace_bytes, void *stream, const char *what)
{
    int rc = check_route(r);
    if (rc) return rc;
    if (!q || !uh || !grad_q_rout || !grad_q) return fail(HBVX_E_NULL, "route buffer is NULL");
    if (n_rows < r->S) return fail(HBVX_E_SHAPE, "grad_q has fewer rows than series");
    hipStream_t st = (hipStream_t)stream;
    const bool want_p = grad_ra || grad_rb;
    if (want_p && (!workspace || workspace_bytes < hbvx_route_workspace_bytes(r)))
        return fail(HBVX_E_NULL, "route workspace missing or too small");
    const int nchunk = route_chunks(r);
    const int64_t nblk = (int64_t)((r->B + 63) / 64) * nchunk;
    if (nblk > INT32_MAX - 8) return fail(HBVX_E_SHAPE, "routing adjoint: too many (basin, chunk) tiles for one launch");
    hipLaunchKernelGGL(k_route_bwd, dim3(xcd_grid(nblk)), dim3(256), 0, st, r->T, r->B, r->S, r->L, n_rows, q, uh,
                       grad_q_rout, grad_q, want_p ? (double *)workspace : nullptr);
    if (want_p)
        hipLaunchKernelGGL(k_route_bwd_params, dim3((r->B + ROUTE_PB - 1) / ROUTE_PB), dim3(1024), 0, st, *r, nchunk,
                           uh, (const double *)workspace, grad_ra, grad_rb);
    hipError_t e = hipGetLastError();
    if (e != hipSuccess) return hip_fail(e, what);
    return HBVX_OK;
}

extern "C" int hbvx_route_backward(const hbvx_route_desc *r, const float *q, const float *uh,
                                   const float *grad_q_rout, float *grad_q, float *grad_ra,
                                   float *grad_rb, void *workspace, uint64_t workspace_bytes,
                                   void *stream)
{
    return launch_route_bwd(r, q, uh, grad_q_rout, grad_q, r ? r->S : 0, grad_ra, grad_rb, workspace, workspace_bytes,
                            stream, "hbvx_route_backward launch");
}

extern "C" int hbvx_route_backward_rows(const hbvx_route_desc *r, const float *q, const float *uh,
                                        const float *grad_q_rout, float *grad_q, int32_t grad_q_rows, float *grad_ra,
                                        float *grad_rb, void *workspace, uint64_t workspace_bytes, void *stream)
{
    return launch_route_bwd(r, q, uh, grad_q_rout, grad_q, grad_q_rows, grad_ra, grad_rb, workspace, workspace_bytes,
                            stream, "hbvx_route_backward_rows launch");
}

__global__ void k_selftest_pow(const float *x, const float *y, float *out, int n)
{
    int i = blockIdx.x * blockDim.x + threadIdx.x;
    if (i < n) out[i] = pow_pos_(x[i], y[i]);
}

extern "C" int hbvx_selftest_pow(const float *x, const float *y, float *out, int n, void *stream)
{
    if (!x || !y || !out || n <= 0) return fail(HBVX_E_NULL, "selftest_pow: bad arguments");
    hipLaunchKernelGGL(k_selftest_pow, dim3((n + 255) / 256), dim3(256), 0, (hipStream_t)stream, x, y,
                       out, n);
    hipError_t e = hipGetLastError();
    if (e != hipSuccess) return hip_fail(e, "selftest_pow launch");
    return HBVX_OK;
}

__global__ void k_selftest_div(const float *x, const float *y, float *out, int n)
{
    int i = blockIdx.x * blockDim.x + threadIdx.x;
    if (i < n) out[i] = div_(x[i], y[i]);
}

extern "C" int hbvx_selftest_div(const float *x, const float *y, float *out, int n, void *stream)
{
    if (!x || !y || !out || n <= 0) return fail(HBVX_E_NULL, "selftest_div: bad arguments");
    hipLaunchKernelGGL(k_selftest_div, dim3((n + 255) / 256), dim3(256), 0, (hipStream_t)stream, x, y,
                       out, n);
    hipError_t e = hipGetLastError();
    if (e != hipSuccess) return hip_fail(e, "selftest_div launch");
    return HBVX_OK;
}

#define BFI_ROWS 8
template <int PB, int NH>
__global__ void __launch_bounds__(PB * 64 * NH) k_bfi(int T, int B, const float *__restrict__ qs,
                                                      const float *__restrict__ q2, float nz,
                                                      float *__restrict__ bfi)
{
    constexpr int NC = 2 / NH, NR = BFI_ROWS / NC;
    __shared__ float r0[2][64][PB], r2[2][64][PB];
    const int bl = threadIdx.x % PB, sl = (threadIdx.x / PB) & 63, half = threadIdx.x / (PB * 64);
    const int b = xcd_block() * PB + bl;
    float a0[NC], a2[NC];
#pragma unroll
    for (int i = 0; i < NC; i++) a0[i] = a2[i] = 0.0f;
    if (b < B) {
        const int h0 = half * NC;
        int t = sl;
        for (; t + 64 * (h0 + NC - 1) + 128 * (NR - 1) < T; t += 128 * NR) {
            float v0[NC][NR], v2[NC][NR];
#pragma unroll
            for (int j = 0; j < NR; j++)
#pragma unroll
                for (int i = 0; i < NC; i++) {
                    v0[i][j] = qs[(int64_t)(t + 64 * (h0 + i) + 128 * j) * B + b];
                    v2[i][j] = q2[(int64_t)(t + 64 * (h0 + i) + 128 * j) * B + b];
                }
#pragma unroll
            for (int j = 0; j < NR; j++)
#pragma unroll
                for (int i = 0; i < NC; i++) {
                    a0[i] += v0[i][j];
                    a2[i] += v2[i][j];
                }
        }
#pragma unroll
        for (int i = 0; i < NC; i++)
            for (int tt = t + 64 * (h0 + i); tt < T; tt += 128) {
                a0[i] += qs[(int64_t)tt * B + b];
                a2[i] += q2[(int64_t)tt * B + b];
            }
    }
#pragma unroll
    for (int i = 0; i < NC; i++) {
// ... 400 lines not shown
```

### hydrodl2_amd/csrc/hbvx_host.h

```cpp
#pragma once

#include <hip/hip_runtime.h>

#include <cstdint>
#include <cstdio>
#include <cstdlib>
#include <cstring>
#include <mutex>
#include <type_traits>

#include "../../include/hbvx.h"
#include "hbv_step.h"

namespace hbvx_host {

int fail(int code, const char *msg);
int hip_fail(hipError_t e, const char *what);
void note_dispatch(int dir, const char *family);
int env_int(const char *name, int dflt);
int device_cu_count();
bool &zero_taken();
int lg_members(int M);
int count_dyn(const hbvx_desc *d);
bool use_tiled(const hbvx_desc *d);
int check_desc(const hbvx_desc *d);
inline bool aux_matches_traj(const hbvx_fwd_out *out) { return !hbvx::SAVE_POW || ((out->traj != nullptr) == (out->aux != nullptr)); }

static const int LDS_BUDGET = 160 * 1024 - 512;

template <typename F>
auto with_model(const hbvx_desc *d, F &&f)
{
    using namespace hbvx;
    switch (d->model) {
    case HBVX_MODEL_HBV10:
        if (d->n_param == 13) return f(std::integral_constant<int, MODEL_HBV10>{}, std::true_type{});
        return f(std::integral_constant<int, MODEL_HBV10>{}, std::false_type{});
    case HBVX_MODEL_HBV11P: return f(std::integral_constant<int, MODEL_HBV11P>{}, std::true_type{});
    case HBVX_MODEL_HOURLY: return f(std::integral_constant<int, MODEL_HOURLY>{}, std::true_type{});
    default: return f(std::integral_constant<int, MODEL_HBV20>{}, std::true_type{});
    }
}

template <typename F>
auto with_adj(const hbvx_desc *d, bool few, F &&f)
{
    if (d->n_param == 13) return few ? f(std::true_type{}, std::true_type{}) : f(std::true_type{}, std::false_type{});
    return few ? f(std::false_type{}, std::true_type{}) : f(std::false_type{}, std::false_type{});
}

inline int check_tan_params(const hbvx_desc *d, const hbvx_param_tan *p)
{
    for (int i = d->n_param; i < HBVX_MAX_PARAM; i++)
        if (p[i].dyn || p[i].sta) return fail(HBVX_E_SHAPE, "tangent for a parameter slot the model lacks");
    for (int i = 0; i < d->n_param; i++)
        if (p[i].dyn && !d->p[i].dyn) return fail(HBVX_E_SHAPE, "dynamic tangent for a static parameter");
    return HBVX_OK;
}
inline void zero_stride_tangents(hbvx_tan_batch &tb, int n_param)
{
    if (!tb.x_d_stride) tb.x = nullptr;
    if (!tb.mu_d_stride) tb.muwts = nullptr;
    if (!tb.state_d_stride) tb.state_in = nullptr;
    for (int i = 0; i < n_param; i++) {
        if (!tb.dyn_d_stride[i]) tb.p[i].dyn = nullptr;
        if (!tb.sta_d_stride[i]) tb.p[i].sta = nullptr;
    }
}

bool try_fwd_pipe(const hbvx_desc *d, const hbvx_fwd_out *out, void *stream, int *rc);
bool try_fwd_stream(const hbvx_desc *d, const hbvx_fwd_out *out, void *stream, int *rc, bool any_size = false);
hipError_t set_dynamic_lds(const void *kern, int lds);
template <typename Args, typename K>
hipError_t launch_tiled_one(K kern, const Args &a, dim3 grid, int threads, size_t lds, hipStream_t st)
{
    hipError_t e = set_dynamic_lds(reinterpret_cast<const void *>(kern), (int)lds);
    if (e != hipSuccess) return e;
    hipLaunchKernelGGL(kern, grid, dim3(threads), lds, st, a);
    return hipGetLastError();
}
inline void store_gate(const hbvx_bwd_io *io, hipStream_t st)
{
    if (io->store_gate) (void)hipStreamWaitEvent(st, (hipEvent_t)io->store_gate, 0);
}
bool try_bwd_stream(const hbvx_desc *d, const hbvx_bwd_io *io, void *stream, int *rc);
bool stream_ckpt_applicable(const hbvx_desc *d, int K);
bool try_bwd_stream_ckpt(const hbvx_desc *d, const hbvx_bwd_io *io, void *stream, int *rc);
bool try_fwd_tiled(const hbvx_desc *d, const hbvx_fwd_out *out, void *stream, int *rc);
bool try_bwd_tiled(const hbvx_desc *d, const hbvx_bwd_io *io, void *stream, int *rc);
bool chunked_applicable(const hbvx_desc *d);
int chunk_days();
bool try_bwd_chunked(const hbvx_desc *d, const hbvx_bwd_io *io, void *stream, int *rc);

bool try_bwd_ckpt(const hbvx_desc *d, const hbvx_bwd_io *io, void *stream, int *rc);

}
```

### hydrodl2_amd/csrc/launch_chunked.hip

```cpp
#include "hbvx_host.h"
#include "hbv_chunked.h"

#include <algorithm>
#include <atomic>

using namespace hbvx;
using namespace hbvx_host;

namespace hbvx_host {
void launch_chunk_scan(const hbvx::ChunkArgs &a, hipStream_t st)
{
    const int64_t N = (int64_t)a.d.B * a.d.M;
    hipLaunchKernelGGL(k_bwd_chunk_scan, dim3((unsigned)((N + 63) / 64)), dim3(64), 0, st, a);
}
void launch_chunk_reduce(const hbvx::ChunkArgs &a, int n_param, hipStream_t st)
{
    const int64_t N = (int64_t)a.d.B * a.d.M;
    hipLaunchKernelGGL(k_bwd_chunk_reduce, dim3((unsigned)((N + 255) / 256), n_param), dim3(256), 0, st, a, n_param);
}
}

int hbvx_host::chunk_days() { int c = env_int("HBVX_CHUNK", 64); return c < 2 ? 2 : c; }

bool hbvx_host::chunked_applicable(const hbvx_desc *d)
{
    const char *v = getenv("HBVX_BWD");
    if (v && !strcmp(v, "tiled")) return false;
    return d->T >= 2 * chunk_days();
}

static int np_of(const hbvx_desc *d) { return d->n_param; }

static bool onepass_admitted(const hbvx_desc *d)
{
    return d->model == HBVX_MODEL_HBV10 && (d->n_param == 12 || d->n_param == 13) && count_dyn(d) == 0;
}

static int gpart_rows(const hbvx_desc *d)
{
    const int np = np_of(d);
    return onepass_admitted(d) ? std::max(np, onepass_rows(np)) : np;
}

extern "C" uint64_t hbvx_backward_workspace_bytes(const hbvx_desc *d)
{
    if (!d || d->T <= 0 || d->B <= 0 || d->M <= 0 || !chunked_applicable(d)) return 0;
    const int C = chunk_days();
    const uint64_t nchunk = (uint64_t)(d->T + C - 1) / C;
    return nchunk * (uint64_t)d->B * (uint64_t)d->M * (uint64_t)(35 + gpart_rows(d)) * sizeof(float);
}

static std::atomic<int> g_chunk_form{0};
extern "C" int hbvx_chunk_form(void) { return g_chunk_form.load(); }

#define ONEPASS_GROUP_DEFAULT 4
static int onepass_group() { return std::min(std::max(env_int("HBVX_ONEPASS_GROUP", ONEPASS_GROUP_DEFAULT), 1), ONEPASS_GMAX); }
static std::atomic<int> g_onepass_group{0};
extern "C" int hbvx_onepass_group(void) { return g_onepass_group.load(); }
extern "C" int hbvx_onepass_slot_bytes(int n_param) { return onepass_slot_bytes(n_param); }

template <int MODEL, bool BETAET, int DYN, bool GFULL>
static hipError_t launch_chunked_t(const ChunkArgs &a, hipStream_t st, bool onepass)
{
    const hbvx_desc &d = a.d;
    const int bpw = 64 >> a.lgMp;
    const int64_t N = (int64_t)d.B * d.M;
    (void)bpw;
    dim3 g2((unsigned)(8 * a.per_xcd * a.nchunk));
    if constexpr (MODEL == MODEL_HBV10 && DYN == 0) {
        if (onepass) {
            constexpr int NP = ChunkNP<MODEL, BETAET>::value;
            g_chunk_form = 1;
            ChunkArgs o = a;
            o.group = onepass_group();
            g_onepass_group = o.group;
            const int ngrp = (a.nchunk + o.group - 1) / o.group;
            hipLaunchKernelGGL((k_bwd_chunk_onepass<BETAET, GFULL>), dim3((unsigned)(8 * a.per_xcd * ngrp)),
                               dim3(64 * o.group), o.group > 1 ? onepass_slot_bytes(NP) : 0, st, o);
            ChunkArgs s = a;
            s.nchunk = ngrp;
            hipLaunchKernelGGL(k_bwd_chunk_scan, dim3((unsigned)((N + 63) / 64)), dim3(64), 0, st, s);
            store_gate(&a.io, st);
            const int ngroup = (ngrp + ONEPASS_FOLD_GROUP - 1) / ONEPASS_FOLD_GROUP;
            hipLaunchKernelGGL((k_bwd_chunk_fold<NP>), dim3((unsigned)((N + 255) / 256), (unsigned)ngroup), dim3(256), 0,
                               st, s);
            ChunkArgs r = a;
            r.gpart = a.phi;
            r.nchunk = ngroup;
            hipLaunchKernelGGL(k_bwd_chunk_reduce, dim3((unsigned)((N + 255) / 256), d.n_param), dim3(256), 0, st,
                               r, d.n_param);
            return hipGetLastError();
        }
    }
    g_chunk_form = 2;
    int sc = 0;
    const bool mu = d.muwts != nullptr;
    if (!mu && DYN == 1 && MODEL == MODEL_HBV10 && BETAET && a.nd == 2 && a.dslot[0] == P_BETA && a.dslot[1] == P_BETAET) sc = 1;
    if (!mu && DYN == 1 && (MODEL == MODEL_HBV20 || MODEL == MODEL_HOURLY) && a.nd == 3 && a.dslot[0] == P_BETA &&
        a.dslot[1] == P_K0 && a.dslot[2] == P_BETAET)
        sc = 2;
    if constexpr (DYN == 1 && MODEL == MODEL_HBV10 && BETAET) {
        if (sc == 1) {
            hipLaunchKernelGGL((k_bwd_chunk_phi<MODEL, BETAET, DYN, GFULL, 1>), g2, dim3(64), 0, st, a);
            hipLaunchKernelGGL(k_bwd_chunk_scan, dim3((unsigned)((N + 63) / 64)), dim3(64), 0, st, a);
            store_gate(&a.io, st);
            hipLaunchKernelGGL((k_bwd_chunk_sweep<MODEL, BETAET, DYN, GFULL, 1>), g2, dim3(64), 0, st, a);
        }
    }
    if constexpr (DYN == 1 && (MODEL == MODEL_HBV20 || MODEL == MODEL_HOURLY)) {
        if (sc == 2) {
            hipLaunchKernelGGL((k_bwd_chunk_phi<MODEL, BETAET, DYN, GFULL, 2>), g2, dim3(64), 0, st, a);
            hipLaunchKernelGGL(k_bwd_chunk_scan, dim3((unsigned)((N + 63) / 64)), dim3(64), 0, st, a);
            store_gate(&a.io, st);
            hipLaunchKernelGGL((k_bwd_chunk_sweep<MODEL, BETAET, DYN, GFULL, 2>), g2, dim3(64), 0, st, a);
        }
    }
    if (sc != 0) {
        hipLaunchKernelGGL(k_bwd_chunk_reduce, dim3((unsigned)((N + 255) / 256), d.n_param), dim3(256), 0, st,
                           a, d.n_param);
        return hipGetLastError();
    }
    if constexpr (DYN == 0 || DYN == 1) {
        if (d.muwts) {
            hipLaunchKernelGGL((k_bwd_chunk_phi<MODEL, BETAET, DYN, GFULL, 0, true>), g2, dim3(64), 0, st, a);
            hipLaunchKernelGGL(k_bwd_chunk_scan, dim3((unsigned)((N + 63) / 64)), dim3(64), 0, st, a);
            store_gate(&a.io, st);
            hipLaunchKernelGGL((k_bwd_chunk_sweep<MODEL, BETAET, DYN, GFULL, 0, false, true>), g2, dim3(64), 0, st, a);
            hipLaunchKernelGGL(k_bwd_chunk_reduce, dim3((unsigned)((N + 255) / 256), d.n_param), dim3(256), 0, st,
                               a, d.n_param);
            return hipGetLastError();
        }
    }
    hipLaunchKernelGGL((k_bwd_chunk_phi<MODEL, BETAET, DYN, GFULL>), g2, dim3(64), 0, st, a);
    hipLaunchKernelGGL(k_bwd_chunk_scan, dim3((unsigned)((N + 63) / 64)), dim3(64), 0, st, a);
    store_gate(&a.io, st);
    if constexpr (DYN == 3) {
        const hbvx_param_grad &g0 = a.io.g[0];
        bool rows = g0.dyn && ((uintptr_t)g0.dyn & 7) == 0 &&
                    (g0.dyn_b_stride & 1) == 0 && (g0.dyn_t_stride & 1) == 0 && ((d.n_param * d.M) & 1) == 0;
        for (int i = 1; i < d.n_param && rows; i++)
            rows = a.io.g[i].dyn == g0.dyn + (int64_t)i * d.M && a.io.g[i].dyn_b_stride == g0.dyn_b_stride &&
                   a.io.g[i].dyn_t_stride == g0.dyn_t_stride;
        if (rows) hipLaunchKernelGGL((k_bwd_chunk_sweep<MODEL, BETAET, DYN, GFULL, 0, true>), g2, dim3(64), 0, st, a);
        else hipLaunchKernelGGL((k_bwd_chunk_sweep<MODEL, BETAET, DYN, GFULL>), g2, dim3(64), 0, st, a);
        return hipGetLastError();
    }
    hipLaunchKernelGGL((k_bwd_chunk_sweep<MODEL, BETAET, DYN, GFULL>), g2, dim3(64), 0, st, a);
    if (DYN == 3) return hipGetLastError();
    hipLaunchKernelGGL(k_bwd_chunk_reduce, dim3((unsigned)((N + 255) / 256), d.n_param), dim3(256), 0, st,
                       a, d.n_param);
    return hipGetLastError();
}

template <int DYN, bool GFULL>
static hipError_t launch_chunked_v(const hbvx_desc *d, const ChunkArgs &a, hipStream_t st, bool onepass = false)
{
    return with_model(d, [&](auto m, auto be) { return launch_chunked_t<m, be, DYN, GFULL>(a, st, onepass); });
}

static hipError_t launch_chunked(const hbvx_desc *d, const hbvx_bwd_io *io, hipStream_t st)
{
    ChunkArgs a;
    a.d = *d;
    a.io = *io;
    a.lgMp = lg_members(d->M);
    a.C = chunk_days();
    a.nchunk = (d->T + a.C - 1) / a.C;
    a.per_xcd = chunk_per_xcd(d->B, a.lgMp);
    a.group = 1;
    const int64_t N = (int64_t)d->B * d->M;
    a.phi = (float *)io->workspace;
    a.abnd = a.phi + (int64_t)a.nchunk * 30 * N;
    a.gpart = a.abnd + (int64_t)a.nchunk * 5 * N;
    const bool gfull = io->grad_flux != nullptr;
    a.nd = 0;
    a.dslot[0] = a.dslot[1] = a.dslot[2] = 0;
    const int ndyn = count_dyn(d);
    if (ndyn > 0 && ndyn <= CHUNK_FEW) {
        for (int i = 0; i < d->n_param; i++)
            if (d->p[i].dyn) a.dslot[a.nd++] = i;
        return gfull ? launch_chunked_v<1, true>(d, a, st) : launch_chunked_v<1, false>(d, a, st);
    }
    bool alldyn = ndyn == d->n_param && !d->muwts;
    for (int i = 0; i < d->n_param && alldyn; i++)
        alldyn = d->p[i].drop == nullptr && d->p[i].dyn == d->p[0].dyn + (int64_t)i * d->M &&
                 d->p[i].dyn_t_stride == d->p[0].dyn_t_stride && d->p[i].dyn_b_stride == d->p[0].dyn_b_stride;
    if (alldyn) return gfull ? launch_chunked_v<3, true>(d, a, st) : launch_chunked_v<3, false>(d, a, st);
    if (ndyn > 0) return gfull ? launch_chunked_v<2, true>(d, a, st) : launch_chunked_v<2, false>(d, a, st);
    const bool onepass = onepass_admitted(d) && !d->muwts && !io->grad_x && env_int("HBVX_CHUNK_ONEPASS", 1) != 0;
    return gfull ? launch_chunked_v<0, true>(d, a, st, onepass) : launch_chunked_v<0, false>(d, a, st, onepass);
}

bool hbvx_host::try_bwd_chunked(const hbvx_desc *d, const hbvx_bwd_io *io, void *stream, int *rc)
{
    if (io->workspace && chunked_applicable(d) && io->workspace_bytes >= hbvx_backward_workspace_bytes(d)) {
        hipError_t e = launch_chunked(d, io, (hipStream_t)stream);
        note_dispatch(1, "chunked");
        *rc = e != hipSuccess ? hip_fail(e, "hbvx_backward (chunked) launch") : HBVX_OK;
        return true;
    }
    return false;
}
```

### hydrodl2_amd/csrc/launch_pipe.hip

```cpp
#include "hbvx_host.h"
#include "hbv_pipe.h"

using namespace hbvx;
using namespace hbvx_host;

bool hbvx_host::try_fwd_pipe(const hbvx_desc *d, const hbvx_fwd_out *out, void *stream, int *rc)
{
        const char *fv = getenv("HBVX_FWD");
        const bool adj = d->model == HBVX_MODEL_HBVADJ;
        const bool mu = d->muwts != nullptr && !adj;
        const int nd = count_dyn(d) + (mu ? 1 : 0);
        const bool many = nd > PIPE_FEWDYN;
        const int Kt = many ? PIPE_KT_MANY : (nd > 0 ? PIPE_KT : PIPE_KT_STATIC);
        const bool cap = d->model != HBVX_MODEL_HBV10 && !adj;
        const int nfl = adj ? 1 : (cap ? 12 : 11);
        bool off32 = ((int64_t)d->B * d->x_b_stride + (int64_t)Kt * d->x_t_stride) * 4 < (int64_t)1 << 31;
        for (int i = 0; i < d->n_param; i++)
            if (d->p[i].dyn)
                off32 = off32 && ((int64_t)d->B * d->p[i].dyn_b_stride + (int64_t)Kt * d->p[i].dyn_t_stride) * 4 <
                                     (int64_t)1 << 31;
        if (mu) off32 = off32 && ((int64_t)d->B * d->mu_b_stride + (int64_t)Kt * d->mu_t_stride) * 4 < (int64_t)1 << 31 &&
                        d->mu_t_stride >= 0;
        const int chmax = std::max(d->ch_prcp, std::max(d->ch_tmean, d->ch_pet));
        bool day_outer = (int64_t)(d->B - 1) * d->x_b_stride + chmax + 1 <= d->x_t_stride;
        for (int i = 0; i < d->n_param; i++)
            if (d->p[i].dyn)
                day_outer = day_outer && (int64_t)(d->B - 1) * d->p[i].dyn_b_stride + d->M <= d->p[i].dyn_t_stride;
        if (mu) day_outer = day_outer && (int64_t)(d->B - 1) * d->mu_b_stride + d->M <= d->mu_t_stride;
        const int64_t wgs_p = ((int64_t)d->B + (64 >> lg_members(d->M)) - 1) / (64 >> lg_members(d->M));
        const bool pmodel = d->model == HBVX_MODEL_HBV10 || d->model == HBVX_MODEL_HBV11P ||
                            d->model == HBVX_MODEL_HBV20 || d->model == HBVX_MODEL_HOURLY ||
                            (adj && d->adj_stop == 2 && !many);
        const size_t lds = (size_t)PipeLds(Kt, nd > 0 ? (many ? nd : PIPE_FEWDYN) : 0, cap).total * 4;
        const int ckpt_k = (out->traj && HBVX_TRAJ_KIND(out->traj_layout) == HBVX_TRAJ_CKPT)
                               ? HBVX_TRAJ_CKPT_DAYS(out->traj_layout) : 0;
        const bool ckpt_fits = !ckpt_k || ((int64_t)((d->T + ckpt_k - 1) / ckpt_k) * 5 * d->B * d->M * 4 < (int64_t)1 << 32);
        if (ckpt_fits && use_tiled(d) && !(fv && !strcmp(fv, "tiled")) && pmodel && off32 && day_outer &&
            nd <= PIPE_MAXDYN && (int)lds <= LDS_BUDGET && wgs_p < 4096 && !(adj && d->muwts) && (out->flux || adj) && d->T >= 4 * Kt &&
            (adj ? !ckpt_k : (ckpt_k ? true : aux_matches_traj(out))) &&
            (int64_t)d->B * d->M * 4 * Kt < (int64_t)1 << 31 &&
            (int64_t)nfl * d->T * d->B * 4 < (int64_t)1 << 31) {
            PipeArgs pa;
            pa.d = *d;
            pa.o = *out;
            pa.lgMp = lg_members(d->M);
            pa.Kt = Kt;
            pa.ckptK = ckpt_k;
            const int bpw_p = 64 >> pa.lgMp;
            dim3 grid_p((d->B + bpw_p - 1) / bpw_p);
            pa.fill_ptr = nullptr;
            pa.fill_state = nullptr;
            pa.fill_n16 = 0;
            pa.nwg = (int)grid_p.x;
            pa.fill_waves = env_int("HBVX_PIPE_FILL_WAVES", 16);
            if (out->zero_ptr && out->zero_state && out->zero_bytes >= 16 && ((uintptr_t)out->zero_ptr & 15) == 0) {
                const int n_cu = device_cu_count();
                const int spare = n_cu - (int)grid_p.x;
                const int nfill = env_int("HBVX_PIPE_FILL_WGS", spare >= n_cu / 8 ? spare : 0);
                if (nfill > 0) {
                    pa.fill_ptr = out->zero_ptr;
                    pa.fill_state = (unsigned *)out->zero_state;
                    pa.fill_n16 = out->zero_bytes / 16;
                    grid_p.x += (unsigned)nfill;
                    zero_taken() = true;
                }
            }
            int pthreads = env_int("HBVX_PIPE_THREADS", 1024);
            pthreads = pthreads < 512 ? 512 : (pthreads > 1024 ? 1024 : (pthreads / 64) * 64);
            if (nd > 0) pthreads = 1024;
            const bool be = d->n_param == 13, tr = out->traj != nullptr, dy = nd > 0;
            const int dflag = env_int("HBVX_PIPE_DIRECT", -1);
            const bool direct = !SAVE_POW && (dflag >= 0 ? dflag != 0 : bpw_p >= 8);
            hipStream_t st = (hipStream_t)stream;
            unsigned dmask = 0;
            for (int i = 0; i < d->n_param; i++) dmask |= d->p[i].dyn ? (1u << i) : 0u;
            const int sc = dmask == ((1u << P_BETA) | (1u << P_BETAET)) ? 1
                         : dmask == ((1u << P_BETA) | (1u << P_K0) | (1u << P_BETAET)) ? 2 : 0;
            auto go = [&](auto m, auto be_c, auto trm) -> hipError_t {
                constexpr int MODEL = decltype(m)::value, TR = decltype(trm)::value;
                constexpr bool BE = decltype(be_c)::value;
                constexpr bool S1 = BE && (MODEL == MODEL_HBV10 || MODEL == MODEL_HBV11P);
                constexpr bool S2 = BE && (MODEL == MODEL_HBV10 || MODEL == MODEL_HBV20 || MODEL == MODEL_HOURLY);
                auto launch = [&](auto kern) { return launch_tiled_one(kern, pa, grid_p, pthreads, lds, st); };
                if constexpr (MODEL != MODEL_HBVADJ)
                    if (many) return launch(k_fwd_pipe<MODEL, BE, TR, true, true, 0>);
                if constexpr (S1)
                    if (dy && sc == 1) return launch(k_fwd_pipe<MODEL, BE, TR, true, false, 1>);
                if constexpr (S2)
                    if (dy && sc == 2) return launch(k_fwd_pipe<MODEL, BE, TR, true, false, 2>);
                if (dy) return launch(k_fwd_pipe<MODEL, BE, TR, true, false, 0>);
                return launch(k_fwd_pipe<MODEL, BE, TR, false, false, 0>);
            };
            constexpr std::integral_constant<int, 0> tr0{};
            constexpr std::integral_constant<int, 1> tr1{};
            constexpr std::integral_constant<int, 2> tr2{};
            hipError_t e;
            if (adj) {
                constexpr std::integral_constant<int, MODEL_HBVADJ> ma{};
                if (be) e = tr ? go(ma, std::true_type{}, tr1) : go(ma, std::true_type{}, tr0);
                else e = tr ? go(ma, std::false_type{}, tr1) : go(ma, std::false_type{}, tr0);
            } else {
                e = with_model(d, [&](auto m, auto be_c) {
                    return tr && direct ? go(m, be_c, tr2) : (tr ? go(m, be_c, tr1) : go(m, be_c, tr0));
                });
            }
            note_dispatch(0, "pipe");
            *rc = e != hipSuccess ? hip_fail(e, "hbvx_forward (pipelined) launch") : HBVX_OK;
            return true;
        }
    return false;
}

#ifdef PIPE_PROBE
extern "C" int hbvx_debug_pipe_blocks(unsigned long long *out, int n)
{
    hipError_t e = hipMemcpyFromSymbol(out, HIP_SYMBOL(hbvx::g_pipe_blocks), (size_t)(n > 4096 ? 4096 : n) * sizeof(unsigned long long));
    return e == hipSuccess ? 0 : -1;
}
extern "C" int hbvx_debug_pipe_probe(unsigned long long *out32)
{
    hipError_t e = hipMemcpyFromSymbol(out32, HIP_SYMBOL(hbvx::g_pipe_probe), 32 * sizeof(unsigned long long));
    return e == hipSuccess ? 0 : -1;
}
#endif
```

### hydrodl2_amd/csrc/launch_stream_bwd.hip

```cpp
#include "launch_stream_plan.h"
#include "hbv_stream2_ckpt.h"

using namespace hbvx;
using namespace hbvx_host;
using namespace hbvx_host::stream_plan;

namespace {

bool four_waves_pay(int64_t wgs)
{
    const int n_cu = device_cu_count();
    const int64_t s3 = (int64_t)n_cu * 4 * 3, s4 = (int64_t)n_cu * 4 * 4;
    return (wgs + s4 - 1) / s4 < (wgs + s3 - 1) / s3;
}

template <int MODEL, bool BE, int SC>
void go_bwd2(int trj, bool gfull, const StreamBwdArgs &sa, dim3 grid, hipStream_t st)
{
    if constexpr (SC != 4) {
        if (trj == 2 && !gfull && MODEL != MODEL_HOURLY && four_waves_pay((int64_t)sa.per_xcd * 8)) {
            hipLaunchKernelGGL((k_bwd_stream2<MODEL, BE, 2, SC, false, true, MODEL != MODEL_HOURLY>), grid, dim3(64), 0, st, sa);
            return;
        }
    }
    if (trj == 2) {
        if (gfull) hipLaunchKernelGGL((k_bwd_stream2<MODEL, BE, 2, SC, true, true>), grid, dim3(64), 0, st, sa);
        else hipLaunchKernelGGL((k_bwd_stream2<MODEL, BE, 2, SC, false, true>), grid, dim3(64), 0, st, sa);
    } else {
        if (gfull) hipLaunchKernelGGL((k_bwd_stream2<MODEL, BE, 1, SC, true, true>), grid, dim3(64), 0, st, sa);
        else hipLaunchKernelGGL((k_bwd_stream2<MODEL, BE, 1, SC, false, true>), grid, dim3(64), 0, st, sa);
    }
}

template <int MODEL, bool BE, int SC>
void go_bwd2c(bool gfull, int K, const StreamBwdArgs &sa, dim3 grid, hipStream_t st, hipError_t *err)
{
    constexpr int NP = NParamT<MODEL, BE>::value;
    if constexpr (SC == 4) {
        *err = hipErrorInvalidValue;
    } else {
        const int lds = s2c_lds_floats<NP, StreamDyn<SC>::nd>(K) * (int)sizeof(float);
        if (gfull) {
            *err = set_dynamic_lds((const void *)k_bwd_stream2_ckpt<MODEL, BE, SC, true>, lds);
            if (*err == hipSuccess) hipLaunchKernelGGL((k_bwd_stream2_ckpt<MODEL, BE, SC, true>), grid, dim3(64), lds, st, sa, K);
        } else {
            *err = set_dynamic_lds((const void *)k_bwd_stream2_ckpt<MODEL, BE, SC, false>, lds);
            if (*err == hipSuccess) hipLaunchKernelGGL((k_bwd_stream2_ckpt<MODEL, BE, SC, false>), grid, dim3(64), lds, st, sa, K);
        }
    }
}

}

bool hbvx_host::try_bwd_stream(const hbvx_desc *d, const hbvx_bwd_io *io, void *stream, int *rc)
{
    StreamPlan P = plan_stream(d);
    const int64_t lim = (int64_t)1 << 32;
    const bool packed = io->traj_layout == HBVX_TRAJ_PACKED;
    bool ok = P.ok && (io->grad_flux || io->grad_flux4) && (packed || P.rows_ok);
    for (int i = 0; i < d->n_param && ok; i++)
        if (d->p[i].dyn && io->g[i].dyn)
            ok = io->g[i].dyn_t_stride >= 0 && (int64_t)d->B * io->g[i].dyn_b_stride * 4 < lim;
    if (packed) {
        if (!(ok && P.packed_ok)) {
            *rc = fail(HBVX_E_UNSUPPORTED, "packed trajectory: no adjoint kernel for this call");
            return true;
        }
    } else if (!(ok && !adjoint_pinned_elsewhere() && P.wgs >= stream_min(true))) {
        return false;
    }
    StreamBwdArgs sa;
    sa.d = *d;
    sa.io = *io;
    sa.lgMp = P.lg;
    sa.nd = P.nd;
    for (int k = 0; k < 6; k++) sa.dslot[k] = k < P.nd ? P.dslot[k] : 0;
    sa.per_xcd = (int)((P.wgs + 7) / 8);
    const dim3 grid2((unsigned)(8 * sa.per_xcd));
    const bool gfull = io->grad_flux != nullptr;
    const int trj = packed ? 2 : 1;
    hipStream_t st = (hipStream_t)stream;
    store_gate(io, st);
    with_stream2(d, P.sc, [&](auto m, auto be, auto sc) { go_bwd2<m, be, sc>(trj, gfull, sa, grid2, st); });
    hipError_t e = hipGetLastError();
    note_dispatch(1, "stream2");
    *rc = e != hipSuccess ? hip_fail(e, "hbvx_backward (stream) launch") : HBVX_OK;
    return true;
}

bool hbvx_host::stream_ckpt_applicable(const hbvx_desc *d, int K)
{
    if (K != 4 && K != 8 && K != 16) return false;
    const int want = env_int("HBVX_CKPT_ONCHIP", -1);
    if (want == 0) return false;
    const StreamPlan P = plan_stream(d);
    if (!(P.ok && P.sc != 4 && P.packed_ok)) return false;
    if (want == 1) return true;
    return !adjoint_pinned_elsewhere() && P.wgs >= stream_min(true);
}

bool hbvx_host::try_bwd_stream_ckpt(const hbvx_desc *d, const hbvx_bwd_io *io, void *stream, int *rc)
{
    const int K = HBVX_TRAJ_CKPT_DAYS(io->traj_layout);
    if (!stream_ckpt_applicable(d, K) || !(io->grad_flux || io->grad_flux4)) return false;
    const StreamPlan P = plan_stream(d);
    const int64_t lim = (int64_t)1 << 32;
    for (int i = 0; i < d->n_param; i++)
        if (d->p[i].dyn && io->g[i].dyn &&
            !(io->g[i].dyn_t_stride >= 0 && (int64_t)d->B * io->g[i].dyn_b_stride * 4 < lim))
            return false;
    StreamBwdArgs sa;
    sa.d = *d;
    sa.io = *io;
    sa.lgMp = P.lg;
    sa.nd = P.nd;
    for (int k = 0; k < 6; k++) sa.dslot[k] = k < P.nd ? P.dslot[k] : 0;
    sa.per_xcd = (int)((P.wgs + 7) / 8);
    const dim3 grid2((unsigned)(8 * sa.per_xcd));
    hipStream_t st = (hipStream_t)stream;
    store_gate(io, st);
    hipError_t e = hipSuccess;
    const bool gfull = io->grad_flux != nullptr;
    with_stream2(d, P.sc, [&](auto m, auto be, auto sc) { go_bwd2c<m, be, sc>(gfull, K, sa, grid2, st, &e); });
    if (e == hipSuccess) e = hipGetLastError();
    note_dispatch(1, "ckpt-stream2");
    *rc = e != hipSuccess ? hip_fail(e, "hbvx_backward (on-chip checkpoints) launch") : HBVX_OK;
    return true;
}
```

### hydrodl2_amd/ops.py

```python
from __future__ import annotations

import contextlib
import ctypes as _C
from dataclasses import dataclass, field
import functools
import os
import struct
import threading
from typing import List, NamedTuple, Optional, Sequence

import torch
import torch.autograd.forward_ad as _fwAD

from . import _abi
from ._lib import get_library


@dataclass
class ParamSource:
    slot: int
    lo: float
    hi: float
    tensor_idx: int
    sta_off: int
# ... 204 lines not shown
        todo.append((big, None))
        gated = gated or cols[0] != 0

    def start():
        if not todo:
            return None
        main = torch.cuda.current_stream(dev)
        side = _side_stream(dev)
        side.wait_stream(main)
        with torch.cuda.stream(side):
            for big, state in todo:
                if state is None:
                    _call(lib, 'hbvx_zero', lib.zero, big.data_ptr(), big.numel() * big.element_size(), _stream_of(lib, big))
                else:
                    _call(lib, 'hbvx_zero', lib.zero_rest, big.data_ptr(), big.numel() * big.element_size(), state.data_ptr(),
                          _stream_of(lib, big))
            done = torch.cuda.Event()
            done.record(side)
        return done
    start.gated = gated
    return gp, rows, bases, start


def _ptr(t: Optional[torch.Tensor], off: int = 0) -> Optional[int]:
    if t is None:
        return None
    return t.data_ptr() + 4 * off


def _stream_of(lib, t: torch.Tensor) -> int:
    if lib.is_device:
        return torch.cuda.current_stream(t.device).cuda_stream
    return 0


def _check_tensor(lib, t: torch.Tensor, name: str):
    if t.dtype != torch.float32:
        raise TypeError(f"{name} must be float32, got {t.dtype}")
    if lib.is_device and not t.is_cuda:
        raise RuntimeError(f"{name} must live on the GPU (got {t.device}); "
                           "hydrodl2_amd has no CPU path")
    if not lib.is_device and t.is_cuda:
        raise RuntimeError(f"{name}: test library expects host tensors")


def has_tangent(*ts) -> bool:
    if _fwAD._current_level < 0:
        return False
    for t in ts:
        if isinstance(t, (tuple, list)):
            if has_tangent(*t):
                return True
        elif torch.is_tensor(t) and _fwAD.unpack_dual(t).tangent is not None:
            return True
    return False


def _mu_t0(cfg: StepConfig) -> int:
    return cfg.t0 if cfg.mu_t0 is None else cfg.mu_t0


_PTR = struct.Struct("<Q")
_D = _abi.Desc
_PS_SIZE = _C.sizeof(_abi.ParamSrc)
_OFF_P = _D.p.offset
_OFF_DYN, _OFF_STA, _OFF_DROP = _abi.ParamSrc.dyn.offset, _abi.ParamSrc.sta.offset, _abi.ParamSrc.drop.offset


class _DescPlan:
    __slots__ = ("key", "template", "sta", "dyn", "drop")


def _desc_plan(cfg: StepConfig, x, has_mu: bool) -> _DescPlan:
    key = (x.stride(0), x.stride(1), has_mu, len(cfg.params), cfg.T, cfg.t0, cfg.B, cfg.M)
    plan = getattr(cfg, "_plan", None)
    if plan is not None and plan.key == key:
        return plan
    d = _abi.Desc()
    d.abi_version = _abi.ABI_VERSION
    d.model = cfg.model
    d.T, d.B, d.M = cfg.T, cfg.B, cfg.M
    d.n_param = cfg.n_param
    d.raw_sigmoid = 1 if cfg.raw_sigmoid else 0
    d.ch_prcp, d.ch_tmean, d.ch_pet = cfg.channels
    d.nearzero = cfg.nearzero
    d.x_t_stride, d.x_b_stride = x.stride(0), x.stride(1)
    if has_mu:
        d.mu_t_stride, d.mu_b_stride = cfg.B * cfg.M, cfg.M
    plan = _DescPlan()
    plan.key, plan.sta, plan.dyn, plan.drop = key, [], [], []
    for i, ps in enumerate(cfg.params):
        s = d.p[ps.slot]
        base = _OFF_P + ps.slot * _PS_SIZE
        s.sta_b_stride = ps.sta_bs
        plan.sta.append((base + _OFF_STA, ps.tensor_idx, 4 * ps.sta_off))
        if ps.dyn_off >= 0:
            s.dyn_t_stride, s.dyn_b_stride = ps.dyn_ts, ps.dyn_bs
            plan.dyn.append((base + _OFF_DYN, ps.dyn_tensor_idx, 4 * ps.dyn_off))
            plan.drop.append((base + _OFF_DROP, i))
        s.lo, s.hi = ps.lo, ps.hi
    d.adj_gtol, d.adj_max_iter, d.adj_stop = cfg.adj_gtol, cfg.adj_max_iter, cfg.adj_stop
    plan.template = bytes(d)
    cfg._plan = plan
    return plan


def _fill_desc(cfg: StepConfig, x, state_in, muwts, ac, elev, ptensors) -> _abi.Desc:
    plan = _desc_plan(cfg, x, muwts is not None)
    buf = bytearray(plan.template)
    pk = _PTR.pack_into
    pk(buf, _D.x.offset, x.data_ptr() + 4 * cfg.t0 * x.stride(0))
    if ac is not None:
        pk(buf, _D.ac.offset, ac.data_ptr())
    if elev is not None:
        pk(buf, _D.elev.offset, elev.data_ptr())
    if muwts is not None:
        pk(buf, _D.muwts.offset, muwts.data_ptr() + 4 * _mu_t0(cfg) * cfg.B * cfg.M)
    if state_in is not None:
        pk(buf, _D.state_in.offset, state_in.data_ptr())
    bases = [t.data_ptr() for t in ptensors]
    for off, ti, boff in plan.sta:
        pk(buf, off, bases[ti] + boff)
    for off, ti, boff in plan.dyn:
        pk(buf, off, bases[ti] + boff)
    params = cfg.params
    for off, i in plan.drop:
        m = params[i].drop
        if m is not None:
            pk(buf, off, m.data_ptr())
    return _abi.Desc.from_buffer(buf)


_MEMO_ENV = ("HBVX_KERNEL", "HBVX_FWD", "HBVX_BWD", "HBVX_STREAM", "HBVX_STREAM_MIN", "HBVX_STREAM_MW_MIN", "HBVX_CHUNK",
             "HBVX_CKPT_BLOCK", "HBVX_CKPT_SCRATCH_MB", "HBVX_CKPT_BLOCKWISE", "HBVX_CKPT_ONCHIP")
_ENV_DATA = getattr(os.environ, "_data", None)
_MEMO_ENV_B = tuple(os.fsencode(k) for k in _MEMO_ENV)


def _env_key() -> tuple:
    if isinstance(_ENV_DATA, dict):
        return tuple(map(_ENV_DATA.get, _MEMO_ENV_B))
    return tuple(os.environ.get(k) for k in _MEMO_ENV)


def _cached(cfg: StepConfig, key, fn):
    memo = cfg.__dict__.setdefault("_memo", {})
    key = (key, _env_key())
    v = memo.get(key)
    if v is None:
        v = memo[key] = fn()
    return v


def _route_desc(cfg: StepConfig, ptensors, S: int = 4) -> _abi.RouteDesc:
    r = _abi.RouteDesc()
    rs = cfg.route
    r.abi_version = _abi.ABI_VERSION
    r.T, r.B, r.S = cfg.T, cfg.B, S
    r.L = min(cfg.T, _abi.UH_MAXLEN)
    r.raw_sigmoid = 1 if cfg.raw_sigmoid else 0
    r.ra = _ptr(ptensors[rs.tensor_idx], rs.a_off)
    r.rb = _ptr(ptensors[rs.tensor_idx], rs.b_off)
    r.r_stride = rs.stride
    r.a_lo, r.a_hi = rs.a_bounds
    r.b_lo, r.b_hi = rs.b_bounds
    return r


class _NoCtx:
    needs_input_grad = ()

    def save_for_backward(self, *a):
        pass

    def mark_non_differentiable(self, *a):
        pass

    def set_materialize_grads(self, v):
        pass


class PathRecord(NamedTuple):
    cfg: StepConfig
    x: torch.Tensor
    state_in: Optional[torch.Tensor]
    muwts: Optional[torch.Tensor]
    ac: Optional[torch.Tensor]
    elev: Optional[torch.Tensor]
    ptensors: tuple
    flux: Optional[torch.Tensor]
    uh: Optional[torch.Tensor]
    routed: Optional[torch.Tensor]
    state_out: torch.Tensor
    traj: Optional[torch.Tensor] = None


_TAP = threading.local()


@contextlib.contextmanager
def record_paths(want_traj: bool = True):
    outer = getattr(_TAP, "records", None), getattr(_TAP, "want_traj", True)
    _TAP.records = records = []
    _TAP.want_traj = want_traj
    try:
        yield records
    finally:
        _TAP.records, _TAP.want_traj = outer


def _hbv_forward(ctx, cfg: StepConfig, x, state_in, muwts, ac, elev, ptensors):
    lib = get_library()
    _check_tensor(lib, x, "x_phy")
    for i, p in enumerate(ptensors):
        _check_tensor(lib, p, f"parameters[{i}]")
        if not p.is_contiguous():
            raise ValueError("parameter tensors must be contiguous")
    if x.stride(2) != 1:
        raise ValueError("x_phy must have unit stride on the forcing axis")
    if muwts is not None:
        _check_tensor(lib, muwts, "muwts")
        if not muwts.is_contiguous() or tuple(muwts.shape[1:]) != (cfg.B, cfg.M):
            raise ValueError("muwts must be a contiguous [T,B,nmul] tensor")
    dev = x.device
    T, B, M = cfg.T, cfg.B, cfg.M
    needs_grad = any(ctx.needs_input_grad)
    keep = needs_grad or cfg.want_traj
    stream = _stream_of(lib, x)

    desc = _fill_desc(cfg, x, state_in, muwts, ac, elev, ptensors)
    out = _abi.FwdOut()
    flux = _out((cfg.n_flux, T, B), dev) \
        if cfg.want_flux else None
    state_out = _out((5, B, M), dev)
    ckpt = cfg.ckpt_days if (needs_grad and cfg.want_flux and not cfg.want_traj) else 0
    if ckpt:
        traj = _out(((T + ckpt - 1) // ckpt * 5, B * M), dev)
        aux = None
        layout = _abi.TRAJ_CKPT | (ckpt << 8)
    else:
        traj = _out((5, T + 1, B * M), dev) if keep else None
        aux = _out((2, T, B * M), dev) if (needs_grad and lib.saves_pow) else None
        layout = (_cached(cfg, ("layout", x.stride(0), x.stride(1)), lambda: lib.preferred_traj_layout(desc))
                  if (keep and cfg.want_flux) else _abi.TRAJ_ROWS)
    out.flux, out.state_out = _ptr(flux), _ptr(state_out)
    out.traj, out.aux = _ptr(traj), _ptr(aux)
    out.n_flux, out.traj_layout = cfg.n_flux, layout
    ctx.early_gp = None
    if needs_grad and cfg.want_flux and any(ctx.needs_input_grad[6:]):
        ctx.early_gp = _early_zero_request(lib, cfg, ptensors, ctx.needs_input_grad[6:], out)
    _call(lib, 'hbvx_forward', lib.forward, desc, out, stream)
    _early_zero_result(lib, cfg, ctx.early_gp)

    routed = uh = None
    if cfg.route is not None and cfg.want_flux:
        r = _route_desc(cfg, ptensors)
        routed = _out((4, T, B), dev)
        uh = _out((B, r.L), dev)
        _call(lib, 'hbvx_route_forward', lib.route_forward, r, _ptr(flux), _ptr(uh), _ptr(routed), stream)

    bfi = None
    if cfg.want_bfi and cfg.want_flux:
        src = routed if routed is not None else flux
        k2 = 3 if routed is not None else _abi.F_Q2
        bfi = _out((B,), dev)
        _call(lib, 'hbvx_bfi', lib.bfi, T, B, _ptr(src), _ptr(src, k2 * T * B), float(cfg.nearzero), _ptr(bfi), stream)

    ctx.cfg = cfg
    ctx.traj_layout = layout
    ctx.desc = desc if needs_grad else None
    ctx.has_bfi = bfi is not None
    ctx.set_materialize_grads(False)
    if needs_grad:
        ctx.save_for_backward(x, state_in, muwts, ac, elev, traj, aux, flux, uh, routed, *ptensors)
    fwd_ad = _fwAD._current_level >= 0 and not isinstance(ctx, _NoCtx)
    if fwd_ad:
        ctx.save_for_forward(x, state_in, muwts, ac, elev, flux, uh, routed, *ptensors)
    ctx.state_tangent = fwd_ad
    nondiff = [] if fwd_ad else [state_out]
    if traj is not None:
        nondiff.append(traj)
    if nondiff:
        ctx.mark_non_differentiable(*nondiff)
    rrows = tuple(routed.unsqueeze(-1).unbind(0)) if routed is not None else ()
    rows = tuple(flux.unsqueeze(-1).unbind(0)) if flux is not None else ()
    ctx.n_routed = len(rrows)
    tap = getattr(_TAP, "records", None)
    if tap is not None:
        tap.append(PathRecord(cfg, x, state_in, muwts, ac, elev, tuple(ptensors), flux, uh, routed, state_out))
    return (state_out, traj, layout, bfi) + rrows + rows


class HbvPath(torch.autograd.Function):

    @staticmethod
    @_device_guard
    def forward(ctx, cfg: StepConfig, x, state_in, muwts, ac, elev, *ptensors):
        return _hbv_forward(ctx, cfg, x, state_in, muwts, ac, elev, ptensors)

    @staticmethod
    @_device_guard
    def backward(ctx, _g_state, _g_traj, _g_layout, g_bfi, *g_all):
        g_rr, g_rows = list(g_all[:ctx.n_routed]), list(g_all[ctx.n_routed:])
        if g_bfi is not None:
            saved_ = ctx.saved_tensors
            flux_, routed_ = saved_[7], saved_[9]
            src = routed_ if routed_ is not None else flux_
            qs, q2 = src[0], src[3 if routed_ is not None else _abi.F_Q2]
            den = qs.sum(0) + ctx.cfg.nearzero
            g_q2 = (100.0 * g_bfi / den).unsqueeze(0).expand_as(q2).unsqueeze(-1)
            g_qs = (-100.0 * g_bfi * q2.sum(0) / (den * den)).unsqueeze(0).expand_as(qs).unsqueeze(-1)
            tgt = g_rr if routed_ is not None else g_rows
            for k, g in ((0, g_qs), (3 if routed_ is not None else _abi.F_Q2, g_q2)):
                tgt[k] = g if tgt[k] is None else tgt[k] + g
        g_routed, n_live = None, 0
        live = [k for k, g in enumerate(g_rr) if g is not None]
        if live:
            n_live = max(live) + 1
            first = g_rr[live[0]]
            if n_live == 1:
                g_routed = first[..., 0].unsqueeze(0)
            else:
                g_routed = torch.zeros((n_live,) + tuple(first.shape[:2]), dtype=torch.float32, device=first.device)
                for k in live:
                    g_routed[k] = g_rr[k][..., 0]
        g_rows = tuple(None if g is None else g[..., 0] for g in g_rows)
        lib = get_library()
        cfg: StepConfig = ctx.cfg
        saved = ctx.saved_tensors
        x, state_in, muwts, ac, elev, traj, aux, flux, uh = saved[:9]
        ptensors = saved[10:]
        dev = x.device
        T, B, M = cfg.T, cfg.B, cfg.M
        stream = _stream_of(lib, x)

        early, ctx.early_gp = ctx.early_gp, None
        rows = [None] * len(ptensors)
        bases = [0] * len(ptensors)
        fill_done, start_fill = None, None
        if _FILL_OVERLAP and lib.is_device:
            gp, rows, bases, start_fill = _overlapped_grad_buffers(lib, cfg, ptensors, ctx.needs_input_grad[6:], early)
        else:
            gp = [_grad_like(lib, p, cfg, i) if ctx.needs_input_grad[6 + i] else None
                  for i, p in enumerate(ptensors)]

        def sta_ptr(idx, off):
            return _ptr(rows[idx], off - bases[idx]) if rows[idx] is not None else _ptr(gp[idx], off)

        def join():
            nonlocal fill_done
            if start_fill is not None and fill_done is None:
                fill_done = start_fill()
            if fill_done is not None:
                torch.cuda.current_stream(dev).wait_event(fill_done)
            for big, row in zip(gp, rows):
                if row is not None:
                    big[-1] += row

        gq = None
        if g_routed is not None and cfg.route is not None:
            r = _route_desc(cfg, ptensors, S=n_live)
            gq = _out((4, T, B), dev)
            in_launch = n_live < 4 and "hbvx_route_backward_rows" not in lib.missing
            if n_live < 4 and not in_launch:
                gq[n_live:].zero_()
            rs = cfg.route
            gt = gp[rs.tensor_idx]
            ws_bytes = _cached(cfg, ("route_ws", n_live), lambda: lib.route_workspace_bytes(r))
            ws = torch.empty((max(ws_bytes, 4) + 3) // 4, dtype=torch.float32, device=dev)
            g_routed = g_routed.contiguous()
            g_ab = (sta_ptr(rs.tensor_idx, rs.a_off) if gt is not None else None,
                    sta_ptr(rs.tensor_idx, rs.b_off) if gt is not None else None)
            if in_launch:
                _call(lib, 'hbvx_route_backward', lib.route_backward_rows, r, _ptr(flux), _ptr(uh),
                      _ptr(g_routed), _ptr(gq), 4, *g_ab, _ptr(ws), ws_bytes, stream)
            else:
                _call(lib, 'hbvx_route_backward', lib.route_backward, r, _ptr(flux), _ptr(uh),
                      _ptr(g_routed), _ptr(gq), *g_ab, _ptr(ws), ws_bytes, stream)
        have = [k for k, g in enumerate(g_rows) if g is not None]
        g_flux = None
        if have and max(have) < 4:
            if gq is None:
                gq = torch.zeros((4, T, B), dtype=torch.float32, device=dev)
            for k in have:
                gq[k] += g_rows[k]
        elif have:
            g_flux = torch.zeros((cfg.n_flux, T, B), dtype=torch.float32, device=dev)
            for k in have:
                g_flux[k] = g_rows[k]

        io = _abi.BwdIO()
        io.traj, io.aux = _ptr(traj), _ptr(aux)
        io.grad_flux, io.grad_flux4 = _ptr(g_flux), _ptr(gq)
        io.n_flux, io.traj_layout = cfg.n_flux, ctx.traj_layout
        gx = gmu = None
        if ctx.needs_input_grad[1]:
            gx = _zeros_like(lib, x)
            if gx.stride() != x.stride():
                raise ValueError("x_phy must be dense for a forcing gradient")
            io.grad_x = _ptr(gx, cfg.t0 * x.stride(0))
        if muwts is not None and ctx.needs_input_grad[3]:
            gmu = torch.zeros_like(muwts)
            io.grad_muwts = _ptr(gmu, _mu_t0(cfg) * B * M)
        for ps in cfg.params:
            g = io.g[ps.slot]
            gs = gp[ps.tensor_idx]
            if gs is not None:
                g.sta = sta_ptr(ps.tensor_idx, ps.sta_off)
                g.sta_b_stride = ps.sta_bs
            if ps.dyn_off >= 0 and gp[ps.dyn_tensor_idx] is not None:
                g.dyn = _ptr(gp[ps.dyn_tensor_idx], ps.dyn_off)
                g.dyn_t_stride, g.dyn_b_stride = ps.dyn_ts, ps.dyn_bs
        desc = ctx.desc if ctx.desc is not None else _fill_desc(cfg, x, state_in, muwts, ac, elev, ptensors)
        if g_flux is None and gq is None:
            join()
            for ps in cfg.params:
                if ps.dyn_off >= 0 and gp[ps.dyn_tensor_idx] is not None:
                    gp[ps.dyn_tensor_idx].zero_()
            return (None, gx, None, gmu, None, None, *gp)
        if (ctx.traj_layout & 0xFF) == _abi.TRAJ_CKPT:
            ws_bytes = _cached(cfg, ("ckpt_ws", ctx.traj_layout), lambda: lib.ckpt_workspace_bytes(desc, ctx.traj_layout >> 8))
        elif ctx.traj_layout == _abi.TRAJ_ROWS:
            ws_bytes = _cached(cfg, "bwd_ws", lambda: lib.backward_workspace_bytes(desc))
        else:
            ws_bytes = 0
        if ws_bytes:
            ws = torch.empty((ws_bytes + 3) // 4, dtype=torch.float32, device=dev)
            io.workspace, io.workspace_bytes = _ptr(ws), ws_bytes
        if start_fill is not None:
            fill_done = start_fill()
            if fill_done is not None and start_fill.gated:
                io.store_gate = fill_done.cuda_event
        _call(lib, 'hbvx_backward', lib.backward, desc, io, stream)
        join()

        return (None, gx, None, gmu, None, None, *gp)

    @staticmethod
    @_device_guard
    def jvp(ctx, _cfg_t, x_t, s_t, mu_t, ac_t, elev_t, *p_t):
        return _hbv_tangent(ctx, x_t, s_t, mu_t, ac_t, elev_t, p_t)


def _hbv_tangent(ctx, x_t, s_t, mu_t, ac_t, elev_t, p_t):
    if ac_t is not None or elev_t is not None:
        raise ValueError("forward-mode AD: tangents of ac_all / elev_all are not supported")
    lib = get_library()
    cfg: StepConfig = ctx.cfg
    x, state_in, muwts, ac, elev, flux, uh, routed, *ptensors = ctx.saved_tensors
    dev = x.device
    T, B, M = cfg.T, cfg.B, cfg.M
    stream = _stream_of(lib, x)
    io = _abi.TanIO()
    keep = []
    if x_t is not None:
        xt = x_t
        if xt.stride() != x.stride():
            xt = torch.empty_strided(x.shape, x.stride(), dtype=x.dtype, device=dev).copy_(x_t)
        keep.append(xt)
        io.x = _ptr(xt, cfg.t0 * x.stride(0))
    if mu_t is not None and muwts is not None:
        mt = mu_t.contiguous()
        keep.append(mt)
        io.muwts = _ptr(mt, _mu_t0(cfg) * B * M)
    if s_t is not None and state_in is not None:
        stt = s_t.contiguous()
        keep.append(stt)
        io.state_in = _ptr(stt)
    pts = [None if t is None else t.contiguous() for t in p_t]
    for ps in cfg.params:
        g = io.p[ps.slot]
        if pts[ps.tensor_idx] is not None:
            g.sta, g.sta_b_stride = _ptr(pts[ps.tensor_idx], ps.sta_off), ps.sta_bs
        if ps.dyn_off >= 0 and pts[ps.dyn_tensor_idx] is not None:
            g.dyn = _ptr(pts[ps.dyn_tensor_idx], ps.dyn_off)
            g.dyn_t_stride, g.dyn_b_stride = ps.dyn_ts, ps.dyn_bs
    tflux = _out((cfg.n_flux, T, B), dev) if cfg.want_flux else None
    tstate = _out((5, B, M), dev)
    io.tan_flux, io.tan_state_out, io.n_flux = _ptr(tflux), _ptr(tstate), cfg.n_flux
    desc = _fill_desc(cfg, x, state_in, muwts, ac, elev, ptensors)
    _call(lib, 'hbvx_forward_tangent', lib.forward_tangent, desc, io, stream)

    troute = None
    if routed is not None:
        r = _route_desc(cfg, ptensors)
        rs = cfg.route
        rt = pts[rs.tensor_idx]
        troute = _out((4, T, B), dev)
        _call(lib, 'hbvx_route_tangent', lib.route_tangent, r, _ptr(flux), _ptr(uh), _ptr(tflux),
              _ptr(rt, rs.a_off), _ptr(rt, rs.b_off), _ptr(troute), stream)
    tbfi = None
    if ctx.has_bfi:
        src, tsrc = (routed, troute) if routed is not None else (flux, tflux)
        k2 = 3 if routed is not None else _abi.F_Q2
        tbfi = _out((B,), dev)
        _call(lib, 'hbvx_bfi_tangent', lib.bfi_tangent, T, B, _ptr(src), _ptr(src, k2 * T * B), _ptr(tsrc),
              _ptr(tsrc, k2 * T * B), float(cfg.nearzero), _ptr(tbfi), stream)
    rrows = tuple(troute.unsqueeze(-1).unbind(0)) if troute is not None else ()
    rows = tuple(tflux.unsqueeze(-1).unbind(0)) if tflux is not None else ()
    return (tstate if ctx.state_tangent else None, None, None, tbfi) + rrows + rows


class BatchOut(NamedTuple):
    flux: Optional[torch.Tensor]
    routed: Optional[torch.Tensor]
    bfi: Optional[torch.Tensor]
    state_out: Optional[torch.Tensor]


def _batch_source(p: torch.Tensor, t: torch.Tensor, off: int):
    if tuple(t.shape[1:]) == tuple(p.shape):
        return off, p.numel()
    row = p[0].numel()
    r, rem = divmod(off, row)
    return (rem, row) if r == p.shape[0] - 1 else None


def hbv_tangent_batch(rec: PathRecord, D: int, x_t=None, mu_t=None, s_t=None, p_t=(), flux_mask: int = 0,
                      n_routed: int = 0, want_bfi: bool = False) -> BatchOut:
    lib = get_library()
    cfg = rec.cfg
    x, ptensors = rec.x, rec.ptensors
    dev = x.device
    T, B, M = cfg.T, cfg.B, cfg.M
    stream = _stream_of(lib, x)
    tb = _abi.TanBatch()
    tb.n_dir, tb.n_flux, tb.flux_mask = D, cfg.n_flux, flux_mask
    keep = []
    if x_t is not None:
        xt = x_t
        if tuple(xt.stride()[1:]) != tuple(x.stride()):
            span = sum((n - 1) * st for n, st in zip(x.shape, x.stride())) + 1
            xt = torch.empty(D * span, dtype=x.dtype, device=dev).as_strided((D,) + tuple(x.shape),
                                                                              (span,) + tuple(x.stride()))
            xt.copy_(x_t)
        keep.append(xt)
        tb.x, tb.x_d_stride = _ptr(xt, cfg.t0 * x.stride(0)), xt.stride(0)
    if mu_t is not None and rec.muwts is not None:
        mt = mu_t.contiguous()
        keep.append(mt)
        tb.muwts, tb.mu_d_stride = _ptr(mt, _mu_t0(cfg) * B * M), mt.stride(0)
    if s_t is not None and rec.state_in is not None:
        stt = s_t.contiguous()
        keep.append(stt)
        tb.state_in, tb.state_d_stride = _ptr(stt), 5 * B * M
    pts = [None if t is None else t.contiguous() for t in p_t]
    pts += [None] * (len(ptensors) - len(pts))
    keep += pts
    dyn_t0 = None
    for ps in cfg.params:
        g = tb.p[ps.slot]
        t = pts[ps.tensor_idx]
        src = None if t is None else _batch_source(ptensors[ps.tensor_idx], t, ps.sta_off)
        if src is not None:
            g.sta, g.sta_b_stride, tb.sta_d_stride[ps.slot] = _ptr(t, src[0]), ps.sta_bs, src[1]
        t = pts[ps.dyn_tensor_idx] if ps.dyn_off >= 0 else None
        if t is None:
            continue
        p = ptensors[ps.dyn_tensor_idx]
        if tuple(t.shape[1:]) == tuple(p.shape):
            off, ds, t0 = ps.dyn_off, p.numel(), 0
        else:
            row = p[0].numel()
            first, col = divmod(ps.dyn_off, row)
            t0 = p.shape[0] - 1 - first
            if t0 != T - 1:
                raise ValueError("compact parameter tangents need a call that ends at the tensor's last row")
            off, ds = col, row
        if dyn_t0 is not None and dyn_t0 != t0:
            raise ValueError("full and compact tangents cannot be mixed over dynamic parameter tensors")
        dyn_t0 = t0
        g.dyn, tb.dyn_d_stride[ps.slot] = _ptr(t, off), ds
        g.dyn_t_stride, g.dyn_b_stride = ps.dyn_ts, ps.dyn_bs
    tb.dyn_t0 = dyn_t0 or 0
    have_any = bool(tb.x or tb.muwts or tb.state_in or any(tb.p[ps.slot].sta or tb.p[ps.slot].dyn for ps in cfg.params))
    rs = cfg.route if n_routed else None
    rt = pts[rs.tensor_idx] if rs is not None else None
    if not flux_mask and not have_any:
        return BatchOut(None, None, None, None)
    nsel = bin(flux_mask).count("1")
    tflux = _out((D, nsel, T, B), dev) if flux_mask else None
    tstate = _out((D, 5, B, M), dev)
    tb.tan_flux, tb.tan_state_out = _ptr(tflux), _ptr(tstate)
    desc = _fill_desc(cfg, x, rec.state_in, rec.muwts, rec.ac, rec.elev, ptensors)
    if cfg.model == _abi.MODEL_HOURLY:
        _call(lib, 'hbvx_hourly_tangent_batch', lib.hourly_tangent_batch, desc, tb, stream)
# ... 817 lines not shown
```

Measured before the change: 36.02 billion.

## Add live-row backward variant that skips dead routed-flux rows in one-pass adjoint

Adds a backward entry point that takes the number of live routed flux rows, so the one-pass static adjoint kernel can be compiled to read only those gradient rows and treat the rest as zero. The Python op no longer zero-fills the unused rows, and the route backward no longer writes them, when this path applies. It also raises the static pipeline tile size when power rows are not saved. Falling back after a refused call adds complexity and a cached refusal flag.

```diff
diff --git a/__graft_entry__.py b/__graft_entry__.py
--- a/__graft_entry__.py
+++ b/__graft_entry__.py
@@ -32,7 +32,8 @@
         os.path.join(ROOT, "include", "hbvx.h"), os.path.join(ROOT, "include", "hbvx_lstm.h"),
         os.path.join(ROOT, "include", "hbvx_gage_pop.h"), os.path.join(ROOT, "include", "hbvx_route_rows.h"),
         os.path.join(ROOT, "include", "hbvx_pop_fdc.h"), os.path.join(ROOT, "include", "hbvx_gage_events.h"),
-        os.path.join(ROOT, "include", "hbvx_pop_events.h"), os.path.join(ROOT, "include", "hbvx_gage_fdc.h")]
+        os.path.join(ROOT, "include", "hbvx_pop_events.h"), os.path.join(ROOT, "include", "hbvx_gage_fdc.h"),
+        os.path.join(ROOT, "include", "hbvx_live_rows.h")]
     objdir = os.path.join(CSRC, "build_" + tag if tag else "build")
     os.makedirs(objdir, exist_ok=True)
     extra = os.environ.get("HBVX_EXTRA_HIPCC_FLAGS", "").split() + list(flags)
diff --git a/hydrodl2_amd/_abi.py b/hydrodl2_amd/_abi.py
--- a/hydrodl2_amd/_abi.py
+++ b/hydrodl2_amd/_abi.py
@@ -329,6 +329,11 @@
     ("hbvx_route_backward_rows", False, _int, [_P(RouteDesc), _fp, _fp, _fp, _fp, _i32, _fp, _fp, _fp, _u64, _vp], None),
 ]
 
+E_UNSUPPORTED = -3
+LIVE_ROWS_SIGNATURES = [
+    ("hbvx_backward_live", False, _int, [_P(Desc), _P(BwdIO), _i32, _vp], None),
+]
+
 
 class HbvxError(RuntimeError):
     pass
@@ -346,13 +351,13 @@
             if not hasattr(d, name):
                 raise HbvxError(f"{path}: missing export {name}")
         self.missing = [name for name in OPTIONAL_EXPORTS +
-                        [row[0] for row in GAGE_POP_SIGNATURES + ROUTE_ROWS_SIGNATURES + POP_FDC_SIGNATURES +
-                         GAGE_EVENTS_SIGNATURES + POP_EVENTS_SIGNATURES + GAGE_FDC_SIGNATURES]
+                        [row[0] for row in GAGE_POP_SIGNATURES + ROUTE_ROWS_SIGNATURES + LIVE_ROWS_SIGNATURES +
+                         POP_FDC_SIGNATURES + GAGE_EVENTS_SIGNATURES + POP_EVENTS_SIGNATURES + GAGE_FDC_SIGNATURES]
                         if not hasattr(d, name)]
         checked = set()
         for name, _, restype, argtypes, layout, sizeof in [row + ("hbvx_sizeof",) for row in SIGNATURES] + \
                 [row + ("hbvx_gage_pop_sizeof",) for row in GAGE_POP_SIGNATURES] + \
-                [row + ("hbvx_sizeof",) for row in ROUTE_ROWS_SIGNATURES] + \
+                [row + ("hbvx_sizeof",) for row in ROUTE_ROWS_SIGNATURES + LIVE_ROWS_SIGNATURES] + \
                 [row + ("hbvx_pop_fdc_sizeof",) for row in POP_FDC_SIGNATURES] + \
                 [row + ("hbvx_gage_events_sizeof",) for row in GAGE_EVENTS_SIGNATURES] + \
                 [row + ("hbvx_pop_events_sizeof",) for row in POP_EVENTS_SIGNATURES] + \
@@ -393,6 +398,16 @@
         self._check(self.dll.hbvx_backward(C.byref(desc), C.byref(io), C.c_void_p(stream)),
                     "hbvx_backward")
 
+    def backward_live(self, desc: Desc, io: BwdIO, n_live4: int, stream: int) -> bool:
+        self.require("hbvx_backward_live")
+        if not 1 <= n_live4 <= 4:
+            raise ValueError(f"n_live4 must be 1 .. 4, got {n_live4}")
+        rc = self.dll.hbvx_backward_live(C.byref(desc), C.byref(io), n_live4, C.c_void_p(stream))
+        if rc == E_UNSUPPORTED:
+            return False
+        self._check(rc, "hbvx_backward_live")
+        return True
+
     def zero_rest(self, ptr: int, nbytes: int, state_ptr: int, stream: int):
         self._check(self.dll.hbvx_zero_rest(C.c_void_p(ptr), nbytes, C.c_void_p(state_ptr), C.c_void_p(stream)), "hbvx_zero_rest")
 
diff --git a/hydrodl2_amd/csrc/hbv_chunked.h b/hydrodl2_amd/csrc/hbv_chunked.h
--- a/hydrodl2_amd/csrc/hbv_chunked.h
+++ b/hydrodl2_amd/csrc/hbv_chunked.h
@@ -113,7 +113,7 @@
     for (int i = 0; i < NP; i++) R.dv[i] = lds[i * 64 + (threadIdx.x & 63)];
 }
 
-template <int NP, int DYN, bool GFULL, bool LDSDV = false, bool MU = false>
+template <int NP, int DYN, bool GFULL, bool LDSDV = false, bool MU = false, int LIVE = 4>
 __device__ __forceinline__ void chunk_issue(const hbvx_desc &d, const hbvx_bwd_io &io,
                                             const LaneId &L, int t, int nf, ChunkRaw<NP> &R,
                                             int nd, const int *dslot)
@@ -138,7 +138,10 @@
     for (int k = 0; k < HBVX_MAX_FLUX; k++) {
         R.gf[k] = 0.0f;
         if (GFULL && k < nf) R.gf[k] = io.grad_flux[k * fs + go];
-        if (k < 4) R.g4[k] = io.grad_flux4 ? io.grad_flux4[k * fs + go] : 0.0f;
+        if (k < 4) {
+            if (LIVE < 4) R.g4[k] = k < LIVE ? io.grad_flux4[k * fs + go] : 0.0f;
+            else R.g4[k] = io.grad_flux4 ? io.grad_flux4[k * fs + go] : 0.0f;
+        }
     }
     R.mu = 0.0f;
     if (DYN == 1) {
@@ -396,86 +399,16 @@
 __global__ void __launch_bounds__(64 * ONEPASS_GMAX) __attribute__((amdgpu_waves_per_eu(GFULL ? 2 : 3)))
 k_bwd_chunk_onepass(const ChunkArgs A)
 {
-    extern __shared__ float onepass_slot[];
-    constexpr int MODEL = MODEL_HBV10, DYN = 0;
-    constexpr int NP = ChunkNP<MODEL, BETAET>::value;
-    typedef Step<MODEL, BETAET> S;
-    const int ds_[3] = {0, 0, 0};
-    const hbvx_desc &d = A.d;
-    const hbvx_bwd_io &io = A.io;
-    ChunkBlock blk;
-    if (!chunk_block(d, A.lgMp, A.per_xcd, blk)) return;
-    const LaneId L = lane_id(d, A.lgMp, blk.bx);
-    const int grp = blk.chunk;
-    const int w = __builtin_amdgcn_readfirstlane((int)threadIdx.x >> 6);
-    const int nw = min(min(A.group, ONEPASS_GMAX), A.nchunk - grp * A.group);
-    const int chunk = grp * A.group + w;
-    const int t0 = chunk * A.C, t1 = min(d.T, t0 + A.C);
-    const int64_t N = (int64_t)d.B * d.M;
-    const bool raw = d.raw_sigmoid != 0;
-    const float nz = d.nearzero, invM = 1.0f / (float)d.M;
-    float usta[NP], psta[NP];
-    bool use_dyn[NP];
-    chunk_static<NP, DYN>(d, L, raw, usta, psta, use_dyn, 0, ds_);
-
-    float Phi[5][5], phi[5];
-    float G[6][NPARAM_MAX];
-#pragma unroll
-    for (int k = 0; k < 5; k++) {
-        phi[k] = 0.0f;
-#pragma unroll
-        for (int i = 0; i < 5; i++) Phi[k][i] = (i == k) ? 1.0f : 0.0f;
-    }
-#pragma unroll
-    for (int k = 0; k < 6; k++)
-#pragma unroll
-        for (int i = 0; i < NPARAM_MAX; i++) G[k][i] = 0.0f;
-    if (w < nw) {
-    ChunkRaw<NP> Rn;
-    chunk_issue<NP, DYN, GFULL>(d, io, L, t1 - 1, io.n_flux, Rn, 0, ds_);
-    for (int t = t1 - 1; t >= t0; t--) {
-        ChunkRaw<NP> Rc = Rn;
-        if (t > t0) chunk_issue<NP, DYN, GFULL>(d, io, L, t - 1, io.n_flux, Rn, 0, ds_);
-        ChunkDay<MODEL, BETAET, NP> D;
-        chunk_finish<MODEL, BETAET, NP, DYN, GFULL>(d, Rc, raw, nz, 0.0f, 0.0f, usta, psta, use_dyn, io.n_flux, invM,
-                                                    D, 0, ds_, io.grad_flux4 != nullptr);
-        const typename S::JT c = D.s.jt_coef(D.p, nz);
-        const typename S::JG k = D.s.jg_coef(D.p, nz);
-        S::template jt_gp<0>(c, k, Phi[0], G[0]);
-        S::template jt_gp<0>(c, k, Phi[1], G[1]);
-        S::template jt_gp<1>(c, k, Phi[2], G[2]);
-        S::template jt_gp<2>(c, k, Phi[3], G[3]);
-        S::template jt_gp<2>(c, k, Phi[4], G[4]);
-        if constexpr (!GFULL) {
-            S::template jt_gp<2, true>(c, k, phi, G[5], D.g.gQ0 + D.g.gQ, D.g.gQ1 + D.g.gQ, D.g.gQ2 + D.g.gQ);
-        } else {
-            float gx[3];
-            D.s.bwd(D.p, nz, D.g, phi, G[5], gx);
-        }
-    }
-    }
-    OnepassRows<NP> rows{A.phi + ((int64_t)grp * 30) * N + L.n, A.gpart + ((int64_t)grp * onepass_rows(NP)) * N + L.n, N,
-                         L.active};
-    if (A.group == 1) {
-        onepass_put<float, NP>(Phi, phi, G, rows);
-        return;
-    }
-    OnepassSlot<NP> slot{onepass_slot + (threadIdx.x & 63)};
-    if (w == nw - 1 && w > 0) onepass_put<float, NP>(Phi, phi, G, slot);
-    static_assert(ONEPASS_GMAX == 4, "one stage per wave above wave 0");
-    if (nw > 1) {
-        if (nw > 2) {
-            if (nw > 3) __syncthreads();
-            if (w == 2 && nw > 3) onepass_compose<float, NP, false>(slot, Phi, phi, G, slot);
-            __syncthreads();
-        }
-        if (w == 1 && nw > 2) onepass_compose<float, NP, false>(slot, Phi, phi, G, slot);
-        __syncthreads();
-    }
-    if (w == 0) {
-        if (nw == 1) onepass_put<float, NP>(Phi, phi, G, rows);
-        else onepass_compose<float, NP, true>(slot, Phi, phi, G, rows);
-    }
+    constexpr int LIVE = 4;
+#include "hbv_onepass_body.h"
+}
+
+template <bool BETAET, int LIVE>
+__global__ void __launch_bounds__(64 * ONEPASS_GMAX) __attribute__((amdgpu_waves_per_eu(3)))
+k_bwd_chunk_onepass_live(const ChunkArgs A)
+{
+    constexpr bool GFULL = false;
+#include "hbv_onepass_body.h"
 }
 
 #ifndef HBVX_CHUNK_NO_SHARED_KERNELS
diff --git a/hydrodl2_amd/csrc/hbv_onepass_body.h b/hydrodl2_amd/csrc/hbv_onepass_body.h
--- /dev/null
+++ b/hydrodl2_amd/csrc/hbv_onepass_body.h
@@ -0,0 +1,81 @@
+    static_assert(LIVE >= 1 && LIVE <= 4 && (LIVE == 4 || !GFULL), "fewer live rows: the runoff-only loss");
+    extern __shared__ float onepass_slot[];
+    constexpr int MODEL = MODEL_HBV10, DYN = 0;
+    constexpr int NP = ChunkNP<MODEL, BETAET>::value;
+    typedef Step<MODEL, BETAET> S;
+    const int ds_[3] = {0, 0, 0};
+    const hbvx_desc &d = A.d;
+    const hbvx_bwd_io &io = A.io;
+    ChunkBlock blk;
+    if (!chunk_block(d, A.lgMp, A.per_xcd, blk)) return;
+    const LaneId L = lane_id(d, A.lgMp, blk.bx);
+    const int grp = blk.chunk;
+    const int w = __builtin_amdgcn_readfirstlane((int)threadIdx.x >> 6);
+    const int nw = min(min(A.group, ONEPASS_GMAX), A.nchunk - grp * A.group);
+    const int chunk = grp * A.group + w;
+    const int t0 = chunk * A.C, t1 = min(d.T, t0 + A.C);
+    const int64_t N = (int64_t)d.B * d.M;
+    const bool raw = d.raw_sigmoid != 0;
+    const float nz = d.nearzero, invM = 1.0f / (float)d.M;
+    float usta[NP], psta[NP];
+    bool use_dyn[NP];
+    chunk_static<NP, DYN>(d, L, raw, usta, psta, use_dyn, 0, ds_);
+
+    float Phi[5][5], phi[5];
+    float G[6][NPARAM_MAX];
+#pragma unroll
+    for (int k = 0; k < 5; k++) {
+        phi[k] = 0.0f;
+#pragma unroll
+        for (int i = 0; i < 5; i++) Phi[k][i] = (i == k) ? 1.0f : 0.0f;
+    }
+#pragma unroll
+    for (int k = 0; k < 6; k++)
+#pragma unroll
+        for (int i = 0; i < NPARAM_MAX; i++) G[k][i] = 0.0f;
+    if (w < nw) {
+    ChunkRaw<NP> Rn;
+    chunk_issue<NP, DYN, GFULL, false, false, LIVE>(d, io, L, t1 - 1, io.n_flux, Rn, 0, ds_);
+    for (int t = t1 - 1; t >= t0; t--) {
+        ChunkRaw<NP> Rc = Rn;
+        if (t > t0) chunk_issue<NP, DYN, GFULL, false, false, LIVE>(d, io, L, t - 1, io.n_flux, Rn, 0, ds_);
+        ChunkDay<MODEL, BETAET, NP> D;
+        chunk_finish<MODEL, BETAET, NP, DYN, GFULL>(d, Rc, raw, nz, 0.0f, 0.0f, usta, psta, use_dyn, io.n_flux, invM,
+                                                    D, 0, ds_, LIVE < 4 || io.grad_flux4 != nullptr);
+        const typename S::JT c = D.s.jt_coef(D.p, nz);
+        const typename S::JG k = D.s.jg_coef(D.p, nz);
+        S::template jt_gp<0>(c, k, Phi[0], G[0]);
+        S::template jt_gp<0>(c, k, Phi[1], G[1]);
+        S::template jt_gp<1>(c, k, Phi[2], G[2]);
+        S::template jt_gp<2>(c, k, Phi[3], G[3]);
+        S::template jt_gp<2>(c, k, Phi[4], G[4]);
+        if constexpr (!GFULL) {
+            S::template jt_gp<2, true>(c, k, phi, G[5], D.g.gQ0 + D.g.gQ, D.g.gQ1 + D.g.gQ, D.g.gQ2 + D.g.gQ);
+        } else {
+            float gx[3];
+            D.s.bwd(D.p, nz, D.g, phi, G[5], gx);
+        }
+    }
+    }
+    OnepassRows<NP> rows{A.phi + ((int64_t)grp * 30) * N + L.n, A.gpart + ((int64_t)grp * onepass_rows(NP)) * N + L.n, N,
+                         L.active};
+    if (A.group == 1) {
+        onepass_put<float, NP>(Phi, phi, G, rows);
+        return;
+    }
+    OnepassSlot<NP> slot{onepass_slot + (threadIdx.x & 63)};
+    if (w == nw - 1 && w > 0) onepass_put<float, NP>(Phi, phi, G, slot);
+    static_assert(ONEPASS_GMAX == 4, "one stage per wave above wave 0");
+    if (nw > 1) {
+        if (nw > 2) {
+            if (nw > 3) __syncthreads();
+            if (w == 2 && nw > 3) onepass_compose<float, NP, false>(slot, Phi, phi, G, slot);
+            __syncthreads();
+        }
+        if (w == 1 && nw > 2) onepass_compose<float, NP, false>(slot, Phi, phi, G, slot);
+        __syncthreads();
+    }
+    if (w == 0) {
+        if (nw == 1) onepass_put<float, NP>(Phi, phi, G, rows);
+        else onepass_compose<float, NP, true>(slot, Phi, phi, G, rows);
+    }
diff --git a/hydrodl2_amd/csrc/hbv_pipe.h b/hydrodl2_amd/csrc/hbv_pipe.h
--- a/hydrodl2_amd/csrc/hbv_pipe.h
+++ b/hydrodl2_amd/csrc/hbv_pipe.h
@@ -13,8 +13,9 @@
 #define PIPE_KT 8
 #endif
 #ifndef PIPE_KT_STATIC
-#define PIPE_KT_STATIC 10
+#define PIPE_KT_STATIC (HBVX_SAVE_POW ? 10 : 11)
 #endif
+#define PIPE_KT_STATIC_ADJ 10
 #define PIPE_KT_MANY 4
 #define PIPE_FEWDYN 3
 #define PIPE_MAXDYN 18
@@ -79,11 +80,14 @@
     }
 }
 
+__host__ __device__ constexpr int pipe_soil_rows(bool cap) { return (cap ? 6 : 5) + (SAVE_POW ? 2 : 0); }
+
 struct PipeLds {
     int xin, ab, bc, oa, ob, oc, pin, total;
-    __host__ __device__ explicit PipeLds(int Kt, int pd = 0, bool cap = false)
+    __host__ __device__ constexpr explicit PipeLds(int Kt, int pd = 0, bool cap = false)
+        : xin(0), ab(0), bc(0), oa(0), ob(0), oc(0), pin(0), total(0)
     {
-        const int obr = cap ? 8 : 7;
+        const int obr = pipe_soil_rows(cap);
         xin = 0;
         ab = xin + 4 * Kt * 256;
         bc = ab + 2 * Kt * 128;
@@ -94,6 +98,7 @@
         total = pin + 5 * Kt * pd * 64;
     }
 };
+static_assert(PipeLds(PIPE_KT_STATIC).total * 4 <= 160 * 1024, "a static three-stage tile must fit the 160 KB of a CU");
 
 template <int NSER, int NFS, unsigned FMAP>
 __device__ __forceinline__ void pipe_reduce_pass(const hbvx_desc &d, const hbvx_fwd_out &o, const float *buf,
@@ -140,8 +145,8 @@
     constexpr bool ADJ = MODEL == MODEL_HBVADJ;
     constexpr bool PIPE_NO_UNROLL = ADJ;
     constexpr bool CAP = MODEL != MODEL_HBV10 && !ADJ;
-    constexpr int KT = MANY ? PIPE_KT_MANY : (DYN ? PIPE_KT : PIPE_KT_STATIC);
-    constexpr int OBR = CAP ? 8 : 7, NFB = CAP ? 5 : 4;
+    constexpr int KT = MANY ? PIPE_KT_MANY : (DYN ? PIPE_KT : (ADJ ? PIPE_KT_STATIC_ADJ : PIPE_KT_STATIC));
+    constexpr int OBR = pipe_soil_rows(CAP), NFB = CAP ? 5 : 4;
 #ifdef PIPE_PROBE
     unsigned long long probe_busy = 0, probe_wait = 0, probe_t = __builtin_readcyclecounter();
     struct ProbeFlush {
diff --git a/hydrodl2_amd/csrc/hbvx.hip b/hydrodl2_amd/csrc/hbvx.hip
--- a/hydrodl2_amd/csrc/hbvx.hip
+++ b/hydrodl2_amd/csrc/hbvx.hip
@@ -1,5 +1,6 @@
 #include "hbvx_host.h"
 #include "../../include/hbvx_route_rows.h"
+#include "../../include/hbvx_live_rows.h"
 #include "hbv_step.h"
 #include "hbv_lane.h"
 #include "hbv_gage.h"
@@ -820,7 +821,7 @@
     return HBVX_OK;
 }
 
-extern "C" int hbvx_backward(const hbvx_desc *d, const hbvx_bwd_io *io, void *stream)
+static int backward_impl(const hbvx_desc *d, const hbvx_bwd_io *io, void *stream, int n_live)
 {
     int rc = check_desc(d);
     if (rc) return rc;
@@ -830,6 +831,9 @@
     const int want_nf = (d->model == HBVX_MODEL_HBV10) ? 11 : 12;
     if (io->n_flux != want_nf) return fail(HBVX_E_SHAPE, "n_flux does not match model");
     if (d->T == 0) return HBVX_OK;
+    const bool live = n_live < 4;
+    if (live && (io->traj_layout != HBVX_TRAJ_ROWS || !io->grad_flux4))
+        return fail(HBVX_E_UNSUPPORTED, "live rows: row trajectory and grad_flux4 only");
     if (io->traj_layout != HBVX_TRAJ_ROWS) {
         if (HBVX_TRAJ_KIND(io->traj_layout) == HBVX_TRAJ_CKPT) {
             if (try_bwd_stream_ckpt(d, io, stream, &rc)) return rc;
@@ -840,8 +844,9 @@
         if (try_bwd_stream(d, io, stream, &rc)) return rc;
         return fail(HBVX_E_UNSUPPORTED, "packed trajectory: no adjoint kernel for this call");
     }
-    if (try_bwd_stream(d, io, stream, &rc)) return rc;
-    if (try_bwd_chunked(d, io, stream, &rc)) return rc;
+    if (try_bwd_stream(d, io, stream, &rc, n_live)) return rc;
+    if (try_bwd_chunked(d, io, stream, &rc, n_live)) return rc;
+    if (live) return fail(HBVX_E_UNSUPPORTED, "live rows: the one-pass static adjoint does not take this call");
     if (try_bwd_tiled(d, io, stream, &rc)) return rc;
     BwdArgs a;
     a.d = *d;
@@ -857,6 +862,17 @@
     });
     if (e != hipSuccess) return hip_fail(e, "hbvx_backward launch");
     return HBVX_OK;
+}
+
+extern "C" int hbvx_backward(const hbvx_desc *d, const hbvx_bwd_io *io, void *stream)
+{
+    return backward_impl(d, io, stream, 4);
+}
+
+extern "C" int hbvx_backward_live(const hbvx_desc *d, const hbvx_bwd_io *io, int32_t n_live4, void *stream)
+{
+    if (n_live4 < 1 || n_live4 > 4) return fail(HBVX_E_SHAPE, "n_live4 must be 1 .. 4");
+    return backward_impl(d, io, stream, n_live4);
 }
 
 static int check_route(const hbvx_route_desc *r)
diff --git a/hydrodl2_amd/csrc/hbvx_host.h b/hydrodl2_amd/csrc/hbvx_host.h
--- a/hydrodl2_amd/csrc/hbvx_host.h
+++ b/hydrodl2_amd/csrc/hbvx_host.h
@@ -83,14 +83,14 @@
 {
     if (io->store_gate) (void)hipStreamWaitEvent(st, (hipEvent_t)io->store_gate, 0);
 }
-bool try_bwd_stream(const hbvx_desc *d, const hbvx_bwd_io *io, void *stream, int *rc);
+bool try_bwd_stream(const hbvx_desc *d, const hbvx_bwd_io *io, void *stream, int *rc, int n_live = 4);
 bool stream_ckpt_applicable(const hbvx_desc *d, int K);
 bool try_bwd_stream_ckpt(const hbvx_desc *d, const hbvx_bwd_io *io, void *stream, int *rc);
 bool try_fwd_tiled(const hbvx_desc *d, const hbvx_fwd_out *out, void *stream, int *rc);
 bool try_bwd_tiled(const hbvx_desc *d, const hbvx_bwd_io *io, void *stream, int *rc);
 bool chunked_applicable(const hbvx_desc *d);
 int chunk_days();
-bool try_bwd_chunked(const hbvx_desc *d, const hbvx_bwd_io *io, void *stream, int *rc);
+bool try_bwd_chunked(const hbvx_desc *d, const hbvx_bwd_io *io, void *stream, int *rc, int n_live = 4);
 
 bool try_bwd_ckpt(const hbvx_desc *d, const hbvx_bwd_io *io, void *stream, int *rc);
 
diff --git a/hydrodl2_amd/csrc/launch_chunked.hip b/hydrodl2_amd/csrc/launch_chunked.hip
--- a/hydrodl2_amd/csrc/launch_chunked.hip
+++ b/hydrodl2_amd/csrc/launch_chunked.hip
@@ -58,9 +58,11 @@
 static std::atomic<int> g_onepass_group{0};
 extern "C" int hbvx_onepass_group(void) { return g_onepass_group.load(); }
 extern "C" int hbvx_onepass_slot_bytes(int n_param) { return onepass_slot_bytes(n_param); }
+static std::atomic<int> g_onepass_live{0};
+extern "C" int hbvx_onepass_live_rows(void) { return g_onepass_live.load(); }
 
 template <int MODEL, bool BETAET, int DYN, bool GFULL>
-static hipError_t launch_chunked_t(const ChunkArgs &a, hipStream_t st, bool onepass)
+static hipError_t launch_chunked_t(const ChunkArgs &a, hipStream_t st, bool onepass, int n_live)
 {
     const hbvx_desc &d = a.d;
     const int bpw = 64 >> a.lgMp;
@@ -75,8 +77,16 @@
             o.group = onepass_group();
             g_onepass_group = o.group;
             const int ngrp = (a.nchunk + o.group - 1) / o.group;
-            hipLaunchKernelGGL((k_bwd_chunk_onepass<BETAET, GFULL>), dim3((unsigned)(8 * a.per_xcd * ngrp)),
-                               dim3(64 * o.group), o.group > 1 ? onepass_slot_bytes(NP) : 0, st, o);
+            const dim3 og((unsigned)(8 * a.per_xcd * ngrp)), ob(64 * o.group);
+            const int olds = o.group > 1 ? onepass_slot_bytes(NP) : 0;
+            const int live = GFULL ? 4 : n_live;
+            g_onepass_live = live;
+            if constexpr (!GFULL) {
+                if (live == 1) hipLaunchKernelGGL((k_bwd_chunk_onepass_live<BETAET, 1>), og, ob, olds, st, o);
+                if (live == 2) hipLaunchKernelGGL((k_bwd_chunk_onepass_live<BETAET, 2>), og, ob, olds, st, o);
+                if (live == 3) hipLaunchKernelGGL((k_bwd_chunk_onepass_live<BETAET, 3>), og, ob, olds, st, o);
+            }
+            if (live >= 4) hipLaunchKernelGGL((k_bwd_chunk_onepass<BETAET, GFULL>), og, ob, olds, st, o);
             ChunkArgs s = a;
             s.nchunk = ngrp;
             hipLaunchKernelGGL(k_bwd_chunk_scan, dim3((unsigned)((N + 63) / 64)), dim3(64), 0, st, s);
@@ -153,12 +163,18 @@
 }
 
 template <int DYN, bool GFULL>
-static hipError_t launch_chunked_v(const hbvx_desc *d, const ChunkArgs &a, hipStream_t st, bool onepass = false)
-{
-    return with_model(d, [&](auto m, auto be) { return launch_chunked_t<m, be, DYN, GFULL>(a, st, onepass); });
-}
-
-static hipError_t launch_chunked(const hbvx_desc *d, const hbvx_bwd_io *io, hipStream_t st)
+static hipError_t launch_chunked_v(const hbvx_desc *d, const ChunkArgs &a, hipStream_t st, bool onepass = false,
+                                   int n_live = 4)
+{
+    return with_model(d, [&](auto m, auto be) { return launch_chunked_t<m, be, DYN, GFULL>(a, st, onepass, n_live); });
+}
+
+static bool onepass_takes(const hbvx_desc *d, const hbvx_bwd_io *io)
+{
+    return onepass_admitted(d) && !d->muwts && !io->grad_x && env_int("HBVX_CHUNK_ONEPASS", 1) != 0;
+}
+
+static hipError_t launch_chunked(const hbvx_desc *d, const hbvx_bwd_io *io, hipStream_t st, int n_live)
 {
     ChunkArgs a;
     a.d = *d;
@@ -187,14 +203,18 @@
                  d->p[i].dyn_t_stride == d->p[0].dyn_t_stride && d->p[i].dyn_b_stride == d->p[0].dyn_b_stride;
     if (alldyn) return gfull ? launch_chunked_v<3, true>(d, a, st) : launch_chunked_v<3, false>(d, a, st);
     if (ndyn > 0) return gfull ? launch_chunked_v<2, true>(d, a, st) : launch_chunked_v<2, false>(d, a, st);
-    const bool onepass = onepass_admitted(d) && !d->muwts && !io->grad_x && env_int("HBVX_CHUNK_ONEPASS", 1) != 0;
-    return gfull ? launch_chunked_v<0, true>(d, a, st, onepass) : launch_chunked_v<0, false>(d, a, st, onepass);
-}
-
-bool hbvx_host::try_bwd_chunked(const hbvx_desc *d, const hbvx_bwd_io *io, void *stream, int *rc)
+    const bool onepass = onepass_takes(d, io);
+    return gfull ? launch_chunked_v<0, true>(d, a, st, onepass) : launch_chunked_v<0, false>(d, a, st, onepass, n_live);
+}
+
+bool hbvx_host::try_bwd_chunked(const hbvx_desc *d, const hbvx_bwd_io *io, void *stream, int *rc, int n_live)
 {
     if (io->workspace && chunked_applicable(d) && io->workspace_bytes >= hbvx_backward_workspace_bytes(d)) {
-        hipError_t e = launch_chunked(d, io, (hipStream_t)stream);
+        if (n_live < 4 && !(onepass_takes(d, io) && !io->grad_flux)) {
+            *rc = fail(HBVX_E_UNSUPPORTED, "live rows: the one-pass static adjoint does not take this call");
+            return true;
+        }
+        hipError_t e = launch_chunked(d, io, (hipStream_t)stream, n_live);
         note_dispatch(1, "chunked");
         *rc = e != hipSuccess ? hip_fail(e, "hbvx_backward (chunked) launch") : HBVX_OK;
         return true;
diff --git a/hydrodl2_amd/csrc/launch_pipe.hip b/hydrodl2_amd/csrc/launch_pipe.hip
--- a/hydrodl2_amd/csrc/launch_pipe.hip
+++ b/hydrodl2_amd/csrc/launch_pipe.hip
@@ -3,6 +3,9 @@
 
 using namespace hbvx;
 using namespace hbvx_host;
+
+static_assert(PipeLds(PIPE_KT_STATIC).total * 4 <= LDS_BUDGET && PipeLds(PIPE_KT_STATIC, 0, true).total * 4 <= LDS_BUDGET,
+              "static pipelined tiles must fit LDS_BUDGET with and without the capillary row");
 
 bool hbvx_host::try_fwd_pipe(const hbvx_desc *d, const hbvx_fwd_out *out, void *stream, int *rc)
 {
@@ -11,7 +14,7 @@
         const bool mu = d->muwts != nullptr && !adj;
         const int nd = count_dyn(d) + (mu ? 1 : 0);
         const bool many = nd > PIPE_FEWDYN;
-        const int Kt = many ? PIPE_KT_MANY : (nd > 0 ? PIPE_KT : PIPE_KT_STATIC);
+        const int Kt = many ? PIPE_KT_MANY : (nd > 0 ? PIPE_KT : (adj ? PIPE_KT_STATIC_ADJ : PIPE_KT_STATIC));
         const bool cap = d->model != HBVX_MODEL_HBV10 && !adj;
         const int nfl = adj ? 1 : (cap ? 12 : 11);
         bool off32 = ((int64_t)d->B * d->x_b_stride + (int64_t)Kt * d->x_t_stride) * 4 < (int64_t)1 << 31;
diff --git a/hydrodl2_amd/csrc/launch_stream_bwd.hip b/hydrodl2_amd/csrc/launch_stream_bwd.hip
--- a/hydrodl2_amd/csrc/launch_stream_bwd.hip
+++ b/hydrodl2_amd/csrc/launch_stream_bwd.hip
@@ -52,7 +52,7 @@
 
 }
 
-bool hbvx_host::try_bwd_stream(const hbvx_desc *d, const hbvx_bwd_io *io, void *stream, int *rc)
+bool hbvx_host::try_bwd_stream(const hbvx_desc *d, const hbvx_bwd_io *io, void *stream, int *rc, int n_live)
 {
     StreamPlan P = plan_stream(d);
     const int64_t lim = (int64_t)1 << 32;
@@ -68,6 +68,10 @@
         }
     } else if (!(ok && !adjoint_pinned_elsewhere() && P.wgs >= stream_min(true))) {
         return false;
+    }
+    if (n_live < 4) {
+        *rc = fail(HBVX_E_UNSUPPORTED, "live rows: the streaming adjoint takes this call");
+        return true;
     }
     StreamBwdArgs sa;
     sa.d = *d;
diff --git a/hydrodl2_amd/ops.py b/hydrodl2_amd/ops.py
--- a/hydrodl2_amd/ops.py
+++ b/hydrodl2_amd/ops.py
@@ -380,6 +380,12 @@
     return v
 
 
+def _live_rows(n_live4: int) -> int:
+    if not isinstance(n_live4, int) or not 1 <= n_live4 <= 4:
+        raise ValueError(f"n_live4 must be an integer in 1 .. 4, got {n_live4!r}")
+    return n_live4
+
+
 def _route_desc(cfg: StepConfig, ptensors, S: int = 4) -> _abi.RouteDesc:
     r = _abi.RouteDesc()
     rs = cfg.route
@@ -586,11 +592,18 @@
                     big[-1] += row
 
         gq = None
+        have = [k for k, g in enumerate(g_rows) if g is not None]
+        live4 = 4
         if g_routed is not None and cfg.route is not None:
             r = _route_desc(cfg, ptensors, S=n_live)
             gq = _out((4, T, B), dev)
-            in_launch = n_live < 4 and "hbvx_route_backward_rows" not in lib.missing
-            if n_live < 4 and not in_launch:
+            if (n_live < 4 and "hbvx_backward_live" not in lib.missing and not have and muwts is None
+                    and cfg.model == _abi.MODEL_HBV10 and ctx.traj_layout == _abi.TRAJ_ROWS
+                    and not ctx.needs_input_grad[1] and all(ps.dyn_off < 0 for ps in cfg.params)
+                    and not _cached(cfg, "live_rows_refused", list)):
+                live4 = n_live
+            in_launch = live4 == 4 and n_live < 4 and "hbvx_route_backward_rows" not in lib.missing
+            if live4 == 4 and n_live < 4 and not in_launch:
                 gq[n_live:].zero_()
             rs = cfg.route
             gt = gp[rs.tensor_idx]
@@ -605,7 +618,6 @@
             else:
                 _call(lib, 'hbvx_route_backward', lib.route_backward, r, _ptr(flux), _ptr(uh),
                       _ptr(g_routed), _ptr(gq), *g_ab, _ptr(ws), ws_bytes, stream)
-        have = [k for k, g in enumerate(g_rows) if g is not None]
         g_flux = None
         if have and max(have) < 4:
             if gq is None:
@@ -659,7 +671,16 @@
             fill_done = start_fill()
             if fill_done is not None and start_fill.gated:
                 io.store_gate = fill_done.cuda_event
-        _call(lib, 'hbvx_backward', lib.backward, desc, io, stream)
+        if live4 < 4:
+            took = []
+            _call(lib, 'hbvx_backward', lambda *a: took.append(lib.backward_live(*a)),
+                  desc, io, _live_rows(live4), stream)
+            if not took[0]:
+                _cached(cfg, "live_rows_refused", list).append(True)
+                gq[live4:].zero_()
+                live4 = 4
+        if live4 == 4:
+            _call(lib, 'hbvx_backward', lib.backward, desc, io, stream)
         join()
 
         return (None, gx, None, gmu, None, None, *gp)
diff --git a/include/hbvx_live_rows.h b/include/hbvx_live_rows.h
--- /dev/null
+++ b/include/hbvx_live_rows.h
@@ -0,0 +1,16 @@
+#ifndef HBVX_LIVE_ROWS_H
+#define HBVX_LIVE_ROWS_H
+
+#include "hbvx.h"
+
+#ifdef __cplusplus
+extern "C" {
+#endif
+
+int hbvx_backward_live(const hbvx_desc *d, const hbvx_bwd_io *io, int32_t n_live4, void *stream);
+
+#ifdef __cplusplus
+}
+#endif
+
+#endif
```

New measurement: 37.77 billion, median of 6. 1.05x the previous value.
